# NERSC/swin_v2_weather

Hardware: AMD Instinct MI355X
Metric: ERA5 samples/sec (73x721x1440) swin_73var depth12 (higher is better)
Workload: dtype bf16

## Files before the change

include/swv2.h:

```cpp
#ifndef SWV2_H
#define SWV2_H
#include <stddef.h>
#include <stdint.h>

#ifdef __cplusplus
extern "C" {
#endif

#define SWV2_VERSION 112

enum {
    SWV2_OK = 0,
    SWV2_ERR_INVALID = -1,
    SWV2_ERR_UNSUPPORTED = -2,
    SWV2_ERR_LAUNCH = -3
};

int swv2_version(void);
const char* swv2_last_error(void);

int swv2_attn_geometry(int L, int head_dim, int* Lp, int* DP);

int swv2_attn_fwd_regime(int L, int head_dim, int has_bias, int dbg);

// ... 155 lines not shown
    void* out;
    int out_f32;
} swv2_prep_item;
int swv2_prep_chunk(void);
int swv2_prep_item_chunks(int out_rows, int out_cols, int transpose);
int swv2_prep_multi(const swv2_prep_item* items_dev, const int* chunks_dev, int n_chunks, void* stream);

#define SWV2_LN_BWD_MAX_BLOCKS 512
typedef struct swv2_ln_args {
    const void* a;
    const float* res;
    const float* gamma;
    const float* beta;
    const float* scale;
    const int32_t* rowidx;
    float* y;
    float* mean;
    float* rstd;
    const float* dy;
    void* da;
    float* dgamma;
    float* dbeta;
    float* ws;
    int M, C, res_mod, rows_per_sample;
    float eps;
} swv2_ln_args;

int swv2_ln_residual_fwd(const swv2_ln_args* a, void* stream);
int swv2_ln_residual_bwd(const swv2_ln_args* a, void* stream);

int swv2_batch_sum(const float* in, float* out, int B, long n, int accumulate, void* stream);

int swv2_merge_stats(const float* x, float* mean, float* rstd, int B, int H, int W, int C, float eps, void* stream);
int swv2_merge_ln_bwd(const float* x, const void* dn_bf16, const float* gamma, const float* mean, const float* rstd,
                      float* dx, float* dgamma, float* dbeta, int B, int H, int W, int C, void* stream);

int swv2_loss_sums(const float* prd, const float* tar, const float* quad_w, float* sums, int BC, int H, int W, void* stream);
int swv2_loss_grad(const float* prd, const float* tar, const float* quad_w, const float* coef, float* dprd, int BC, int H,
                   int W, void* stream);
#define SWV2_LOSS_PART_SLICES 8
#define SWV2_LOSS_GROUP_ROWS 32
#define SWV2_LOSS_DUMP_BYTES 2048
#define SWV2_LOSS_RESID_PITCH(N) (((N) + 63) / 64 * 64)
int swv2_loss_part_reduce(const float* part, int M, int T, int B, int Cout, int Ct, int coff, float* sums, void* stream);
int swv2_loss_resid_to_image(const void* resid, const float* coef, const float* add, float* out, int B, int Cout, int H, int W, int Cs, int Cadd,
                             void* stream);
int swv2_loss_finalize(const float* sums, int layers, const float* chw, int BC, int C, int absolute, int squared, float* loss, float* coef,
                       void* stream);

int swv2_adam_step(float* p, const float* g, float* m, float* v, long n, float lr, float beta1, float beta2, float eps,
                   int step, float grad_inv_scale, void* stream);

typedef struct swv2_adam_item {
    float* p;
    const float* g;
    float* m;
    float* v;
    long n;
} swv2_adam_item;
int swv2_adam_chunk(void);
int swv2_adam_multi(const swv2_adam_item* items_dev, const int* chunks_dev, int n_chunks, float lr, float beta1, float beta2,
                    float eps, int step, float grad_inv_scale, void* stream);

typedef struct swv2_lamb_item {
    float* p;
    const float* g;
    float* m;
    float* v;
    long n;
    long chunk0;
} swv2_lamb_item;
#define SWV2_LAMB_SUM_DEPTH 64
#define SWV2_LAMB_ADAMW 1
#define SWV2_LAMB_BIAS_CORRECTION 2
#define SWV2_LAMB_GRAD_AVERAGING 4
#define SWV2_LAMB_NVLAMB 8
#define SWV2_LAMB_WS_GNORM2 0
#define SWV2_LAMB_WS_CLIP 1
#define SWV2_LAMB_WS_BC1 2
#define SWV2_LAMB_WS_BC2 3
#define SWV2_LAMB_WS_ITEM(i) (4 + 4 * (i))
int swv2_lamb_chunk(void);
size_t swv2_lamb_ws_bytes(int n_items, int n_chunks);
int swv2_lamb_grad_norm(const swv2_lamb_item* items_dev, const int* chunks_dev, int n_items, int n_chunks, float grad_inv_scale, void* ws,
                        size_t ws_bytes, void* stream);
int swv2_lamb_multi(const swv2_lamb_item* items_dev, const int* chunks_dev, int n_items, int n_chunks, int item_lo, int item_hi,
                    int chunk_lo, int chunk_hi, float lr, float beta1, float beta2, float eps, float weight_decay, float grad_inv_scale,
                    float max_grad_norm, int step, int flags, const float* extra_gnorm2, void* ws, size_t ws_bytes, void* stream);

int swv2_score_slices(int planes, int H, int W);
size_t swv2_score_ws_bytes(int planes, int H, int W);
int swv2_score_sums(const float* prd, long prd_bstride, const float* tar, long tar_bstride, const float* clim, const float* w, int B, int C,
                    int H, int W, void* ws, size_t ws_bytes, void* stream);
int swv2_score_finalize(const void* ws, size_t ws_bytes, int B, int C, int H, int W, const float* scale, float* sums, float* rmse, float* acc,
                        float* rmse_mean, float* acc_mean, void* stream);

int swv2_stats_slices(int C, int H, int W);
size_t swv2_stats_ws_bytes(int C, int H, int W);
int swv2_stats_accumulate(const float* slab, const float* prev, const double* pivot, double* tsum, void* part, size_t part_bytes, int C, int H,
                          int W, int first, void* stream);
int swv2_stats_finalize(const void* part, size_t part_bytes, const double* tsum, const double* pivot, int C, int H, int W, long T,
                        double* folded, float* time_means, void* stream);

size_t swv2_quantile_ws_bytes(int planes, int H, int W, int K);
int swv2_plane_order_stats(const float* x, long bstride, int B, int C, int H, int W, const int* ranks, int K, float* out, int* nan_count,
                           void* ws, size_t ws_bytes, void* stream);

size_t swv2_ens_ws_bytes(int planes, int H, int W, int M);
int swv2_ens_sums(const float* ens, long ens_mstride, long ens_bstride, const float* tar, long tar_bstride, const float* w, int M, int B, int C,
                  int H, int W, void* ws, size_t ws_bytes, void* stream);
int swv2_ens_finalize(const void* ws, size_t ws_bytes, int M, int B, int C, int H, int W, const float* scale, float* sums, int* hist,
                      float* ens_rmse, float* spread, float* crps, float* fair_crps, float* means, void* stream);

size_t swv2_l1_ws_bytes(int planes, int H, int W);
int swv2_l1_sums(const float* prd, long prd_bstride, const float* tar, long tar_bstride, const float* w, int B, int C, int H, int W, void* ws,
                 size_t ws_bytes, void* stream);
int swv2_l1_finalize(const void* ws, size_t ws_bytes, int B, int C, int H, int W, const float* chw, int absolute, float* sums, float* loss,
                     float* coef, void* stream);
int swv2_l1_grad(const float* prd, const float* tar, const float* quad_w, const float* coef, float* dprd, int BC, int H, int W, void* stream);

size_t swv2_sht_ws_bytes(int planes, int lmax, int mmax);
int swv2_sht_power(const float* table, const float* X, float* power, float* coeffs, int planes, int nlat, int lmax, int mmax, void* ws,
                   size_t ws_bytes, void* stream);
int swv2_sht_adjoint(const float* table, const float* coeffs, const float* gpower, float* dX, int planes, int nlat, int lmax, int mmax,
                     void* stream);
int swv2_sht_repack(const float* src, float* dst, int planes, int nlat, int mmax, float scale, int backward, void* stream);
int swv2_sht_synth(const float* table, const float* rweights, const float* coeffs, const float* response, int response_stride, float scale_m0,
                   float scale_m, float* S, int planes, int nlat, int lmax, int mmax, int nlon, void* stream);

int swv2_era5_select_normalize(const float* raw, float* out, const int* chan, const float* mean, const float* stdv, int B, int S,
                               int Csel, int Craw, int Hraw, int Wraw, int H, int W, int Cout_total, int coff, void* stream);
int swv2_era5_zenith(float* out, const float* sun, int B, int nz, int H, int W, int Cout_total, int coff, void* stream);
int swv2_era5_static(const float* stat, float* out, int B, int Cs, int H, int W, int Cout_total, int coff, void* stream);

int swv2_era5_select_normalize_i16(const int16_t* raw, float* out, const int* chan, const float* mean, const float* stdv, const float* offset,
                                   const float* scale, const int* slab_row, int B, int S, int Csel, int Craw, int Hraw, int Wraw, int H, int W,
                                   int Cout_total, int coff, void* stream);
int swv2_era5_unpack_i16(const int16_t* raw, float* out, const float* offset, const float* scale, int C, int H, int W, void* stream);
int swv2_era5_pack_i16(const float* slab, int16_t* out, const float* offset, const float* scale, int C, int H, int W, void* stream);
size_t swv2_pack_range_ws_bytes(int C, int H, int W);
int swv2_pack_range(const float* slab, int C, int H, int W, int first, float* range, int64_t* missing, void* ws, size_t ws_bytes, void* stream);

typedef struct {
    const void* oh;
    const void* wp;
    const float* bp;
    const float* gamma; const float* beta; const float* scale;
    const int32_t* rowidx;
    const float* x;
    void* a1; float* mean; float* rstd;
    float* y;
    int Bw, Lp, heads, C, rows_per_sample;
    float eps;
} swv2_proj_ln_args;
typedef struct {
    const float* dy;
    const void* a1; const float* mean; const float* rstd; const float* gamma; const float* scale;
    const int32_t* rowidx;
    const void* wpt;
    void* da1;
    void* doh;
    float* dgamma; float* dbeta; float* ws;
    int Bw, Lp, heads, C, rows_per_sample;
} swv2_proj_ln_bwd_args;
int swv2_proj_ln_supported(int C, int heads, int head_pad);
size_t swv2_proj_ln_bwd_ws_floats(int Mw, int C);
int swv2_proj_ln_fwd(const swv2_proj_ln_args* a, void* stream);
int swv2_proj_ln_bwd(const swv2_proj_ln_bwd_args* a, void* stream);

typedef struct {
    const float* x;
    const void* w1;
    const float* b1;
    const void* w2;
    const float* b2;
    const float* gamma;
    const float* beta;
    const float* scale;
    void* hpre;
    void* a2;
    float* mean;
    float* rstd;
    float* y;
    int M, C, hidden, rows_per_sample;
    float eps;
} swv2_mlp_args;
int swv2_mlp_supported(int C, int hidden);
int swv2_mlp_recompute_supported(int C, int hidden);
int swv2_mlp_fwd(const swv2_mlp_args* a, void* stream);

typedef struct {
    const float* dy;
    const void* a2;
    const float* mean;
    const float* rstd;
    const float* gamma;
    const float* scale;
    const void* hpre;
    const void* w2t;
    const void* w1t;
    void* da2;
    void* dh;
    float* dx;
    float* dgamma;
    float* dbeta;
    float* ws;
    int M, C, hidden, rows_per_sample;
    const float* x;
    const void* w1;
    const float* b1;
} swv2_mlp_bwd_args;
size_t swv2_mlp_bwd_ws_floats(int M, int C);
int swv2_mlp_bwd(const swv2_mlp_bwd_args* a, void* stream);

int swv2_cpb_fwd(const float* w1, const float* b1, const float* w2, const float* b2, const void* keep_bf16, float* bias,
                 int wh, int ww, int heads, int hidden, float drop_p, void* stream);
int swv2_cpb_bwd(const float* dbias, const float* w1, const float* b1, const float* w2, const void* keep_bf16, float* dw1,
                 float* db1, float* dw2, float* db2, int wh, int ww, int heads, int hidden, float drop_p, void* stream);
size_t swv2_cpb_bwd_ws_bytes(int wh, int ww, int heads, int hidden);
int swv2_cpb_bwd_ws(const float* dbias, const float* w1, const float* b1, const float* w2, const void* keep_bf16, float* dw1,
                    float* db1, float* dw2, float* db2, int wh, int ww, int heads, int hidden, float drop_p, void* ws,
                    size_t ws_bytes, void* stream);

int swv2_cpb_fwd_multi(const float* const* params_dev, int nblk, const uint32_t* keep_bits, float* bias, int wh, int ww, int heads,
                       int hidden, float drop_p, void* stream);
size_t swv2_cpb_bwd_multi_ws_bytes(int nblk, int wh, int ww, int heads, int hidden);
int swv2_cpb_bwd_multi(const float* dbias_tables, int nchunk, const float* const* params_dev, int nblk, const uint32_t* keep_bits,
                       float* grads, int wh, int ww, int heads, int hidden, float drop_p, void* ws, size_t ws_bytes, void* stream);

typedef struct swv2_block_desc {
    int B, T, C, heads, head_dim, hidden, L, Lp, DP, nwh, nww, mask_thr;
    const int32_t* rowidx;
    const int32_t* qkv_map;
    const int32_t* proj_map;
    const float *logit_scale, *qkv_b_pad, *proj_b, *n1_w, *n1_b, *fc1_b, *fc2_b, *n2_w, *n2_b;
    const void *w_qkv, *w_proj, *w_fc1, *w_fc2;
    const void *w_qkvt, *w_projt, *w_fc1t, *w_fc2t;
    const float* x;
    const float* bias;
    void* bias_pack;
    const float* dp1;
    const float* dp2;
    void* qkvh;  float* rnorm; void* oh; float* lse; void* a1; float* mean1; float* rstd1; float* x1;
    void* hpre;  void* hact;   void* a2; float* mean2; float* rstd2;
    float* x2;
    const float* dx2;
    void *da2, *dh, *da1, *doh, *dqkvh;
    float* dx1;
    float* ln_ws;
    float* dx;
    float *d_logit_scale, *d_bias, *d_qkv_w, *d_qkv_b, *d_proj_w, *d_proj_b, *d_n1_w, *d_n1_b, *d_fc1_w, *d_fc1_b,
          *d_fc2_w, *d_fc2_b, *d_n2_w, *d_n2_b;
    int wgrad_splits;
    int ev_kernel;
    void* ev_start;
    void* ev_stop;
    int fuse_proj_ln;
    int fuse_mlp;
    void* wgrad_ws;
    size_t wgrad_ws_bytes;
    int wgrad_group;
    void* grad_zero;
    size_t grad_zero_bytes;
    size_t ln_ws_floats;
    int bias_prepacked;
    float* dbias_part;
    size_t dbias_part_bytes;
} swv2_block_desc;

enum swv2_block_step {
    SWV2_STEP_RNORM_ZERO = 1,
    SWV2_STEP_QKV,
    SWV2_STEP_QK_NORMALIZE,
    SWV2_STEP_PACK_BIAS,
    SWV2_STEP_ATTN_FWD,
    SWV2_STEP_PROJ, SWV2_STEP_LN1_FWD,
    SWV2_STEP_PROJ_LN_FWD,
    SWV2_STEP_FC1, SWV2_STEP_FC2, SWV2_STEP_LN2_FWD,
    SWV2_STEP_MLP_FWD,
    SWV2_STEP_LN2_BWD, SWV2_STEP_WGRAD_FC2, SWV2_STEP_DH, SWV2_STEP_WGRAD_FC1, SWV2_STEP_DX1,
    SWV2_STEP_MLP_BWD,
    SWV2_STEP_LN1_BWD,
    SWV2_STEP_PROJ_LN_BWD,
    SWV2_STEP_WGRAD_PROJ, SWV2_STEP_DOH, SWV2_STEP_ATTN_BWD, SWV2_STEP_WGRAD_QKV, SWV2_STEP_DX,
    SWV2_STEP_LN_FOLD,
    SWV2_STEP_WGRAD_GROUP,
    SWV2_STEP_COUNT
};
#define SWV2_BLOCK_MAX_STEPS 12
enum { SWV2_DBIAS_NONE = 0,
       SWV2_DBIAS_ATOMICS = 1,
       SWV2_DBIAS_WGRAD_WS = 2,
       SWV2_DBIAS_PART = 3 };
typedef struct swv2_block_plan_t {
    int mlp_fused;
    int proj_ln_fused;
    int ln_deferred;
    int wgrad_grouped;
    int wgrad_kernel;
    int grad_zero_in_kernel;
    int attn_fwd_chunks, attn_bwd_chunks;
    int dbias_dest;
    size_t need_hact_bytes;
    size_t need_ln_ws_floats;
    size_t need_wgrad_ws_bytes;
    int n_fwd, n_bwd;
    int fwd[SWV2_BLOCK_MAX_STEPS], bwd[SWV2_BLOCK_MAX_STEPS];
} swv2_block_plan_t;
int swv2_block_plan(const swv2_block_desc* d, swv2_block_plan_t* out);
int swv2_block_step_id(int step);
const char* swv2_block_step_name(int step);

int swv2_block_fwd(const swv2_block_desc* d, void* stream);
int swv2_block_bwd(const swv2_block_desc* d, void* stream);

#ifdef __cplusplus
}
#endif
#endif
```

swin_v2_weather_amd/_lib.py:

```python
from __future__ import annotations

import ctypes as C
import os
import subprocess
import threading

HERE = os.path.dirname(os.path.abspath(__file__))
CSRC = os.path.join(HERE, "csrc")
LIB_PATH = os.environ.get("SWV2_LIB") or os.path.join(HERE, "libswv2.so")
SOURCES = ["capi.hip", "attn.hip", "attn2.hip", "attn_bwd_stream.hip", "attn_wide.hip", "attn_d256.hip", "gemm.hip", "gemm_tn.hip", "gemm_tn_slab.hip", "rowops.hip", "lamb.hip", "block.hip", "cpb.hip", "mlp.hip", "proj_ln.hip", "dataio.hip", "packed.hip", "score.hip", "stats.hip", "quantile.hip", "ensemble.hip", "loss_l1.hip", "sht.hip"]

ABI_VERSION = 112

_lib = None
_lock = threading.Lock()


class Swv2Error(RuntimeError):
    pass


def build_library(force: bool = False, verbose: bool = False) -> str:
    import glob
    srcs = [os.path.join(CSRC, s) for s in SOURCES]
    deps = srcs + glob.glob(os.path.join(CSRC, "*.h")) + [os.path.join(HERE, "..", "include", "swv2.h")]
    if not force and os.path.exists(LIB_PATH) and all(os.path.getmtime(LIB_PATH) >= os.path.getmtime(d) for d in deps):
        return LIB_PATH
    hipcc = os.environ.get("HIPCC", "/opt/rocm/bin/hipcc")
    objs, procs = [], []
    os.makedirs(os.path.join(HERE, "build"), exist_ok=True)
    for s in srcs:
        o = os.path.join(HERE, "build", os.path.basename(s) + ".o")
        objs.append(o)
        cmd = [hipcc, "--offload-arch=gfx950", "-O3", "-std=c++17", "-fPIC", "-c", s, "-o", o]
        procs.append((cmd, subprocess.Popen(cmd, stdout=subprocess.PIPE, stderr=subprocess.STDOUT)))
    for cmd, p in procs:
        out, _ = p.communicate()
        if p.returncode != 0:
            raise Swv2Error("hipcc failed: %s\n%s" % (" ".join(cmd), out.decode()))
        if verbose and out:
            print(out.decode())
    cmd = [hipcc, "--offload-arch=gfx950", "-shared", "-fPIC", "-o", LIB_PATH] + objs
    r = subprocess.run(cmd, stdout=subprocess.PIPE, stderr=subprocess.STDOUT)
    if r.returncode != 0:
        raise Swv2Error("link failed: %s\n%s" % (" ".join(cmd), r.stdout.decode()))
    return LIB_PATH


def source_hash() -> str:
    import glob
    import hashlib
    h = hashlib.sha256()
    files = sorted(glob.glob(os.path.join(CSRC, "*"))) + [os.path.join(HERE, "..", "include", "swv2.h")]
    for f in files:
        if os.path.isfile(f):
            h.update(os.path.basename(f).encode())
            h.update(open(f, "rb").read())
    return h.hexdigest()[:16]


class AttnArgs(C.Structure):
    _fields_ = [("qkvh", C.c_void_p), ("logit_scale", C.c_void_p), ("bias", C.c_void_p), ("bias_pack", C.c_void_p), ("oh", C.c_void_p),
                ("lse", C.c_void_p), ("doh", C.c_void_p), ("rnorm", C.c_void_p), ("dqkvh", C.c_void_p),
                ("dlogit_scale", C.c_void_p), ("dbias", C.c_void_p),
                ("Bw", C.c_int), ("heads", C.c_int), ("L", C.c_int), ("head_dim", C.c_int),
                ("nwh", C.c_int), ("nww", C.c_int), ("mask_thr", C.c_int), ("max_chunks", C.c_int), ("dbg", C.c_int),
                ("dbias_ws", C.c_void_p), ("dbias_ws_bytes", C.c_size_t), ("dbias_partials", C.c_int)]


class AttnKernelInfo(C.Structure):
    _fields_ = [(n, C.c_int) for n in ("family", "Lp", "DP", "LT", "DK", "LFIX", "regime", "aug", "bias_lds", "qg")]


ATTN_K_D256, ATTN_K_FWD3, ATTN_K_FWD3W, ATTN_K_FWD3B, ATTN_K_WIDE, ATTN_K_STREAM, ATTN_K_FIRST_GEN = range(7)
ATTN_K_NAMES = ("D256", "FWD3", "FWD3W", "FWD3B", "WIDE", "STREAM", "FIRST_GEN")


class Operand(C.Structure):
    _fields_ = [("kind", C.c_int), ("ptr", C.c_void_p), ("rowidx", C.c_void_p), ("aux0", C.c_void_p),
                ("aux1", C.c_void_p), ("aux2", C.c_void_p), ("aux3", C.c_void_p), ("ld", C.c_long),
                ("rows", C.c_int), ("cols", C.c_int), ("p", C.c_int * 4)]


class PrepItem(C.Structure):
    _fields_ = [("w", C.c_void_p), ("rows", C.c_int), ("cols", C.c_int), ("transpose", C.c_int), ("row_map", C.c_void_p),
                ("out_rows", C.c_int), ("col_map", C.c_void_p), ("out_cols", C.c_int), ("out", C.c_void_p), ("out_f32", C.c_int)]


class AdamItem(C.Structure):
    _fields_ = [("p", C.c_void_p), ("g", C.c_void_p), ("m", C.c_void_p), ("v", C.c_void_p), ("n", C.c_long)]


class LambItem(C.Structure):
    _fields_ = [("p", C.c_void_p), ("g", C.c_void_p), ("m", C.c_void_p), ("v", C.c_void_p), ("n", C.c_long), ("chunk0", C.c_long)]


class WgradItem(C.Structure):
    _fields_ = [("dy", Operand), ("x", Operand), ("dW", C.c_void_p), ("db", C.c_void_p), ("nmap", C.c_void_p),
                ("kmap", C.c_void_p), ("ldw", C.c_int)]


class Epilogue(C.Structure):
    _fields_ = [("kind", C.c_int), ("out", C.c_void_p), ("bias", C.c_void_p), ("aux", C.c_void_p),
                ("aux_out", C.c_void_p), ("rowidx", C.c_void_p), ("ld", C.c_long), ("p", C.c_int * 5),
                ("loss_tar", C.c_void_p), ("loss_qw", C.c_void_p), ("loss_part", C.c_void_p),
                ("loss_resid", C.c_void_p),
                ("q", C.c_int * 3)]


class ProjLnArgs(C.Structure):
    _fields_ = [(n, C.c_void_p) for n in ("oh", "wp", "bp", "gamma", "beta", "scale", "rowidx", "x", "a1", "mean", "rstd", "y")] + \
               [(n, C.c_int) for n in ("Bw", "Lp", "heads", "C", "rows_per_sample")] + [("eps", C.c_float)]


class ProjLnBwdArgs(C.Structure):
    _fields_ = [(n, C.c_void_p) for n in ("dy", "a1", "mean", "rstd", "gamma", "scale", "rowidx", "wpt", "da1", "doh", "dgamma", "dbeta",
                                           "ws")] + [(n, C.c_int) for n in ("Bw", "Lp", "heads", "C", "rows_per_sample")]


class MlpArgs(C.Structure):
    _fields_ = [(n, C.c_void_p) for n in ("x", "w1", "b1", "w2", "b2", "gamma", "beta", "scale", "hpre", "a2", "mean", "rstd", "y")] + \
               [(n, C.c_int) for n in ("M", "C", "hidden", "rows_per_sample")] + [("eps", C.c_float)]


class MlpBwdArgs(C.Structure):
    _fields_ = [(n, C.c_void_p) for n in ("dy", "a2", "mean", "rstd", "gamma", "scale", "hpre", "w2t", "w1t", "da2", "dh", "dx",
                                           "dgamma", "dbeta", "ws")] + [(n, C.c_int) for n in ("M", "C", "hidden", "rows_per_sample")] + \
               [(n, C.c_void_p) for n in ("x", "w1", "b1")]


class LnArgs(C.Structure):
    _fields_ = [("a", C.c_void_p), ("res", C.c_void_p), ("gamma", C.c_void_p), ("beta", C.c_void_p),
                ("scale", C.c_void_p), ("rowidx", C.c_void_p), ("y", C.c_void_p), ("mean", C.c_void_p),
                ("rstd", C.c_void_p), ("dy", C.c_void_p), ("da", C.c_void_p), ("dgamma", C.c_void_p),
                ("dbeta", C.c_void_p), ("ws", C.c_void_p), ("M", C.c_int), ("C", C.c_int), ("res_mod", C.c_int),
                ("rows_per_sample", C.c_int), ("eps", C.c_float)]


LN_BWD_MAX_BLOCKS = 512
ATTN_FIRST_GEN, ATTN_PLAIN_STATS, ATTN_BWD_TWO_PHASE = 16, 8192, 32
LOSS_PART_SLICES = 8
LOSS_GROUP_ROWS = 32
LOSS_DUMP_BYTES = 2048
SHT_MRUN = 8


def loss_resid_pitch(n: int) -> int:
    return (n + 63) // 64 * 64
class BlockDesc(C.Structure):
    _fields_ = ([(n, C.c_int) for n in ("B", "T", "C", "heads", "head_dim", "hidden", "L", "Lp", "DP", "nwh", "nww", "mask_thr")] +
                [(n, C.c_void_p) for n in (
                    "rowidx", "qkv_map", "proj_map",
                    "logit_scale", "qkv_b_pad", "proj_b", "n1_w", "n1_b", "fc1_b", "fc2_b", "n2_w", "n2_b",
                    "w_qkv", "w_proj", "w_fc1", "w_fc2", "w_qkvt", "w_projt", "w_fc1t", "w_fc2t",
                    "x", "bias", "bias_pack", "dp1", "dp2",
                    "qkvh", "rnorm", "oh", "lse", "a1", "mean1", "rstd1", "x1", "hpre", "hact", "a2", "mean2", "rstd2", "x2",
                    "dx2", "da2", "dh", "da1", "doh", "dqkvh", "dx1", "ln_ws", "dx",
                    "d_logit_scale", "d_bias", "d_qkv_w", "d_qkv_b", "d_proj_w", "d_proj_b", "d_n1_w", "d_n1_b", "d_fc1_w",
                    "d_fc1_b", "d_fc2_w", "d_fc2_b", "d_n2_w", "d_n2_b")] +
                [("wgrad_splits", C.c_int), ("ev_kernel", C.c_int), ("ev_start", C.c_void_p), ("ev_stop", C.c_void_p),
                 ("fuse_proj_ln", C.c_int), ("fuse_mlp", C.c_int), ("wgrad_ws", C.c_void_p), ("wgrad_ws_bytes", C.c_size_t), ("wgrad_group", C.c_int), ("grad_zero", C.c_void_p),
                 ("grad_zero_bytes", C.c_size_t), ("ln_ws_floats", C.c_size_t),
                 ("bias_prepacked", C.c_int), ("dbias_part", C.c_void_p), ("dbias_part_bytes", C.c_size_t)])


LAMB_ADAMW, LAMB_BIAS_CORRECTION, LAMB_GRAD_AVERAGING, LAMB_NVLAMB = 1, 2, 4, 8
LAMB_SUM_DEPTH = 64
LAMB_WS_GNORM2, LAMB_WS_CLIP, LAMB_WS_BC1, LAMB_WS_BC2 = range(4)


def lamb_ws_item(i: int) -> int:
    return 4 + 4 * i


BLOCK_MAX_STEPS = 12
DBIAS_NONE, DBIAS_ATOMICS, DBIAS_WGRAD_WS, DBIAS_PART = range(4)


class BlockPlan(C.Structure):
    _fields_ = ([(n, C.c_int) for n in ("mlp_fused", "proj_ln_fused", "ln_deferred", "wgrad_grouped", "wgrad_kernel", "grad_zero_in_kernel",
                                        "attn_fwd_chunks", "attn_bwd_chunks", "dbias_dest")] +
                [(n, C.c_size_t) for n in ("need_hact_bytes", "need_ln_ws_floats", "need_wgrad_ws_bytes")] +
                [("n_fwd", C.c_int), ("n_bwd", C.c_int), ("fwd", C.c_int * BLOCK_MAX_STEPS), ("bwd", C.c_int * BLOCK_MAX_STEPS)])

    def steps(self, phase):
        lib = load()
        return [lib.swv2_block_step_name(s).decode() for s in getattr(self, phase)[:getattr(self, "n_" + phase)]]


def block_plan(desc: BlockDesc) -> BlockPlan:
    plan = BlockPlan()
    check(load().swv2_block_plan(C.byref(desc), C.byref(plan)), "swv2_block_plan")
    return plan


OP_F32, OP_BF16, OP_BF16_GELU, OP_HEADS, OP_PATCH, OP_MERGE_LN, OP_BF16_CSCALE = range(7)
EPI_BF16, EPI_F32, EPI_QKV_HEADS, EPI_GELU_GRAD, EPI_UNPATCH, EPI_HEADS, EPI_F32_ACC, EPI_BF16_GELU, EPI_UNPATCH_LOSS = range(9)
LINEAR_RESIDENT_QKV128, LINEAR_RESIDENT_QKV192X3, LINEAR_RESIDENT_DX128, LINEAR_WIDE_DMA, LINEAR_WIDE, LINEAR_TILE64, LINEAR_TILE128 = range(7)
LINEAR_WIDE_KERNELS, LINEAR_TILE_KERNELS = (LINEAR_WIDE_DMA, LINEAR_WIDE), (LINEAR_TILE64, LINEAR_TILE128)
WGRAD_WIDE, WGRAD_TILE = range(2)
BLOCK_WGRAD_SLAB, BLOCK_WGRAD_GROUPED = range(2)

_P, _I, _L, _F = C.c_void_p, C.c_int, C.c_long, C.c_float
SYMBOLS = {
    "swv2_version": (_I, []),
    "swv2_last_error": (C.c_char_p, []),
    "swv2_attn_geometry": (_I, [_I, _I, C.POINTER(_I), C.POINTER(_I)]),
    "swv2_attn_fwd_regime": (_I, [_I, _I, _I, _I]),
    "swv2_attn_fwd_kernel": (_I, [C.POINTER(AttnArgs), C.POINTER(AttnKernelInfo)]),
    "swv2_attn_bwd_kernel": (_I, [C.POINTER(AttnArgs), C.POINTER(AttnKernelInfo)]),
    "swv2_attn_pack_bias_bytes": (C.c_size_t, [_I, _I]),
    "swv2_attn_dbias_ws_bytes": (C.c_size_t, [_I, _I, _I]),
    "swv2_attn_pack_bias": (_I, [_P, _I, _I, _P, _P]),
    "swv2_attn_pack_bias_multi": (_I, [_P, _I, _I, _I, _P, _P]),
    "swv2_attn_bias_chunks": (_I, [_I]),
    "swv2_attn_fwd": (_I, [C.POINTER(AttnArgs), _P]),
    "swv2_attn_bwd": (_I, [C.POINTER(AttnArgs), _P]),
    "swv2_linear": (_I, [C.POINTER(Operand), _P, C.POINTER(Epilogue), _I, _P]),
    "swv2_linear_kernel": (_I, [C.POINTER(Operand), C.POINTER(Epilogue), _I]),
    "swv2_linear_wgrad_kernel": (_I, [C.POINTER(Operand), C.POINTER(Operand), _I, C.c_size_t]),
    "swv2_block_wgrad_kernel": (_I, [C.POINTER(WgradItem), _I, C.c_size_t]),
    "swv2_linear_wgrad": (_I, [C.POINTER(Operand), C.POINTER(Operand), _P, _P, _P, _P, _I, _I, _P]),
    "swv2_linear_wgrad_ws_bytes": (C.c_size_t, [_I, _I, _I, _I]),
    "swv2_qk_normalize": (_I, [_P, _P, _I, _I, _I, _I, _I, _P]),
    "swv2_block_wgrad_ws_bytes": (C.c_size_t, [_I, _I, _I, _I]),
    "swv2_block_wgrad": (_I, [C.POINTER(WgradItem), _I, _P, C.c_size_t, _P]),
    "swv2_linear_wgrad_ws": (_I, [C.POINTER(Operand), C.POINTER(Operand), _P, _P, _P, _P, _I, _I, _P, C.c_size_t, _P]),
    "swv2_prep_weight": (_I, [_P, _I, _I, _I, _P, _I, _P, _I, _P, _P]),
    "swv2_ln_residual_fwd": (_I, [C.POINTER(LnArgs), _P]),
    "swv2_ln_residual_bwd": (_I, [C.POINTER(LnArgs), _P]),
    "swv2_batch_sum": (_I, [_P, _P, _I, _L, _I, _P]),
    "swv2_merge_stats": (_I, [_P, _P, _P, _I, _I, _I, _I, _F, _P]),
    "swv2_merge_ln_bwd": (_I, [_P, _P, _P, _P, _P, _P, _P, _P, _I, _I, _I, _I, _P]),
    "swv2_loss_sums": (_I, [_P, _P, _P, _P, _I, _I, _I, _P]),
    "swv2_loss_grad": (_I, [_P, _P, _P, _P, _P, _I, _I, _I, _P]),
    "swv2_loss_part_reduce": (_I, [_P, _I, _I, _I, _I, _I, _I, _P, _P]),
    "swv2_loss_resid_to_image": (_I, [_P, _P, _P, _P, _I, _I, _I, _I, _I, _I, _P]),
    "swv2_loss_finalize": (_I, [_P, _I, _P, _I, _I, _I, _I, _P, _P, _P]),
    "swv2_prep_chunk": (_I, []),
    "swv2_prep_item_chunks": (_I, [_I, _I, _I]),
    "swv2_prep_multi": (_I, [_P, _P, _I, _P]),
    "swv2_adam_chunk": (_I, []),
    "swv2_adam_multi": (_I, [_P, _P, _I, _F, _F, _F, _F, _I, _F, _P]),
    "swv2_adam_step": (_I, [_P, _P, _P, _P, _L, _F, _F, _F, _F, _I, _F, _P]),
    "swv2_lamb_chunk": (_I, []),
    "swv2_lamb_ws_bytes": (C.c_size_t, [_I, _I]),
    "swv2_lamb_grad_norm": (_I, [_P, _P, _I, _I, _F, _P, C.c_size_t, _P]),
    "swv2_lamb_multi": (_I, [_P, _P, _I, _I, _I, _I, _I, _I, _F, _F, _F, _F, _F, _F, _F, _I, _I, _P, _P, C.c_size_t, _P]),
    "swv2_score_slices": (_I, [_I, _I, _I]),
    "swv2_score_ws_bytes": (C.c_size_t, [_I, _I, _I]),
    "swv2_score_sums": (_I, [_P, _L, _P, _L, _P, _P, _I, _I, _I, _I, _P, C.c_size_t, _P]),
    "swv2_score_finalize": (_I, [_P, C.c_size_t, _I, _I, _I, _I, _P, _P, _P, _P, _P, _P, _P]),
    "swv2_stats_slices": (_I, [_I, _I, _I]),
    "swv2_stats_ws_bytes": (C.c_size_t, [_I, _I, _I]),
    "swv2_stats_accumulate": (_I, [_P, _P, _P, _P, _P, C.c_size_t, _I, _I, _I, _I, _P]),
    "swv2_stats_finalize": (_I, [_P, C.c_size_t, _P, _P, _I, _I, _I, _L, _P, _P, _P]),
    "swv2_quantile_ws_bytes": (C.c_size_t, [_I, _I, _I, _I]),
    "swv2_plane_order_stats": (_I, [_P, _L, _I, _I, _I, _I, _P, _I, _P, _P, _P, C.c_size_t, _P]),
    "swv2_ens_ws_bytes": (C.c_size_t, [_I, _I, _I, _I]),
    "swv2_ens_sums": (_I, [_P, _L, _L, _P, _L, _P, _I, _I, _I, _I, _I, _P, C.c_size_t, _P]),
    "swv2_ens_finalize": (_I, [_P, C.c_size_t, _I, _I, _I, _I, _I, _P, _P, _P, _P, _P, _P, _P, _P, _P]),
    "swv2_l1_ws_bytes": (C.c_size_t, [_I, _I, _I]),
    "swv2_l1_sums": (_I, [_P, _L, _P, _L, _P, _I, _I, _I, _I, _P, C.c_size_t, _P]),
    "swv2_l1_finalize": (_I, [_P, C.c_size_t, _I, _I, _I, _I, _P, _I, _P, _P, _P, _P]),
    "swv2_l1_grad": (_I, [_P, _P, _P, _P, _P, _I, _I, _I, _P]),
    "swv2_sht_ws_bytes": (C.c_size_t, [_I, _I, _I]),
    "swv2_sht_power": (_I, [_P, _P, _P, _P, _I, _I, _I, _I, _P, C.c_size_t, _P]),
    "swv2_sht_adjoint": (_I, [_P, _P, _P, _P, _I, _I, _I, _I, _P]),
    "swv2_sht_repack": (_I, [_P, _P, _I, _I, _I, _F, _I, _P]),
    "swv2_sht_synth": (_I, [_P, _P, _P, _P, _I, _F, _F, _P, _I, _I, _I, _I, _I, _P]),
    "swv2_era5_select_normalize": (_I, [_P, _P, _P, _P, _P] + [_I] * 10 + [_P]),
    "swv2_era5_zenith": (_I, [_P, _P, _I, _I, _I, _I, _I, _I, _P]),
    "swv2_era5_static": (_I, [_P, _P, _I, _I, _I, _I, _I, _I, _P]),
    "swv2_era5_select_normalize_i16": (_I, [_P] * 8 + [_I] * 10 + [_P]),
    "swv2_era5_unpack_i16": (_I, [_P, _P, _P, _P, _I, _I, _I, _P]),
    "swv2_era5_pack_i16": (_I, [_P, _P, _P, _P, _I, _I, _I, _P]),
    "swv2_pack_range_ws_bytes": (C.c_size_t, [_I, _I, _I]),
    "swv2_pack_range": (_I, [_P, _I, _I, _I, _I, _P, _P, _P, C.c_size_t, _P]),
    "swv2_proj_ln_supported": (_I, [_I, _I, _I]),
    "swv2_proj_ln_bwd_ws_floats": (C.c_size_t, [_I, _I]),
    "swv2_proj_ln_fwd": (_I, [C.POINTER(ProjLnArgs), _P]),
    "swv2_proj_ln_bwd": (_I, [C.POINTER(ProjLnBwdArgs), _P]),
    "swv2_mlp_supported": (_I, [_I, _I]),
    "swv2_mlp_recompute_supported": (_I, [_I, _I]),
    "swv2_mlp_fwd": (_I, [C.POINTER(MlpArgs), _P]),
    "swv2_mlp_bwd_ws_floats": (C.c_size_t, [_I, _I]),
    "swv2_mlp_bwd": (_I, [C.POINTER(MlpBwdArgs), _P]),
    "swv2_cpb_fwd": (_I, [_P, _P, _P, _P, _P, _P, _I, _I, _I, _I, _F, _P]),
    "swv2_cpb_bwd": (_I, [_P, _P, _P, _P, _P, _P, _P, _P, _P, _I, _I, _I, _I, _F, _P]),
    "swv2_cpb_bwd_ws": (_I, [_P, _P, _P, _P, _P, _P, _P, _P, _P, _I, _I, _I, _I, _F, _P, C.c_size_t, _P]),
    "swv2_cpb_bwd_ws_bytes": (C.c_size_t, [_I, _I, _I, _I]),
    "swv2_cpb_fwd_multi": (_I, [_P, _I, _P, _P, _I, _I, _I, _I, _F, _P]),
    "swv2_cpb_bwd_multi_ws_bytes": (C.c_size_t, [_I, _I, _I, _I, _I]),
    "swv2_cpb_bwd_multi": (_I, [_P, _I, _P, _I, _P, _P, _I, _I, _I, _I, _F, _P, C.c_size_t, _P]),
    "swv2_block_plan": (_I, [C.POINTER(BlockDesc), C.POINTER(BlockPlan)]),
    "swv2_block_step_id": (_I, [_I]),
    "swv2_block_step_name": (C.c_char_p, [_I]),
    "swv2_block_fwd": (_I, [C.POINTER(BlockDesc), _P]),
    "swv2_block_bwd": (_I, [C.POINTER(BlockDesc), _P]),
}


def load() -> C.CDLL:
    global _lib
    if _lib is not None:
        return _lib
    with _lock:
        if _lib is None:
            if not os.path.exists(LIB_PATH):
                raise Swv2Error(f"{LIB_PATH} not found: run `python -c 'import __graft_entry__ as g; g.build()'` "
                                "(the HIP library is required; there is no fallback path)")
            import torch
            lib = C.CDLL(LIB_PATH)
            for name, (res, args) in SYMBOLS.items():
                fn = getattr(lib, name)
                fn.restype, fn.argtypes = res, args
            got = lib.swv2_version()
            if got != ABI_VERSION:
                raise Swv2Error(f"{LIB_PATH} reports ABI revision {got}, this binding mirrors revision {ABI_VERSION} of include/swv2.h: "
                                "rebuild the library (python -c 'import __graft_entry__ as g; g.build()')")
            _lib = lib
    return _lib


def check(rc: int, what: str = "") -> None:
    if rc != 0:
        msg = load().swv2_last_error()
        raise Swv2Error(f"{what} failed with code {rc}: {msg.decode() if msg else ''}")
```

swin_v2_weather_amd/csrc/block.hip:

```cpp
#include "common.h"

namespace {

swv2_operand op(int kind, const void* p, int rows, int cols, long ld, const int32_t* rowidx = nullptr) {
    swv2_operand o = {};
    o.kind = kind; o.ptr = p; o.rowidx = rowidx; o.ld = ld; o.rows = rows; o.cols = cols;
    return o;
}
swv2_operand op_heads(const void* p, int Bw, int heads, int parts, int Lp, int DP) {
    swv2_operand o = op(SWV2_OP_HEADS, p, Bw * Lp, parts * heads * DP, parts);
    o.p[0] = heads; o.p[2] = Lp; o.p[3] = DP;
    return o;
}
swv2_epilogue epi(int kind, void* out, long ld, const float* bias = nullptr, const void* aux = nullptr,
                  float* aux_out = nullptr, const int32_t* rowidx = nullptr) {
    swv2_epilogue e = {};
    e.kind = kind; e.out = out; e.ld = ld; e.bias = bias; e.aux = aux; e.aux_out = aux_out; e.rowidx = rowidx;
    return e;
}
swv2_attn_args attn(const swv2_block_desc* d, int max_chunks) {
    swv2_attn_args a = {};
    a.qkvh = d->qkvh; a.logit_scale = d->logit_scale; a.bias = d->bias; a.bias_pack = d->bias ? d->bias_pack : nullptr;
    a.oh = d->oh; a.lse = d->lse;
    a.Bw = d->B * d->nwh * d->nww; a.heads = d->heads; a.L = d->L; a.head_dim = d->head_dim; a.nwh = d->nwh; a.nww = d->nww;
    a.mask_thr = d->mask_thr; a.max_chunks = max_chunks;
    return a;
}
void wgrad_items(const swv2_block_desc* d, bool fused, swv2_wgrad_item it[4]) {
    const int BT = d->B * d->T, Bw = d->B * d->nwh * d->nww, Mw = Bw * d->Lp, C = d->C, h = d->heads, hid = d->hidden;
    it[0].dy = op(SWV2_OP_BF16, d->da2, BT, C, C);
    it[0].x = fused ? op(SWV2_OP_BF16_GELU, d->hpre, BT, hid, hid) : op(SWV2_OP_BF16, d->hact, BT, hid, hid);
    it[0].dW = d->d_fc2_w; it[0].db = d->d_fc2_b; it[0].ldw = hid;
    it[1].dy = op(SWV2_OP_BF16, d->dh, BT, hid, hid); it[1].x = op(SWV2_OP_F32, d->x1, BT, C, C);
    it[1].dW = d->d_fc1_w; it[1].db = d->d_fc1_b; it[1].ldw = C;
    it[2].dy = op(SWV2_OP_BF16, d->da1, Mw, C, C); it[2].x = op_heads(d->oh, Bw, h, 1, d->Lp, d->DP);
    it[2].dW = d->d_proj_w; it[2].db = d->d_proj_b; it[2].kmap = d->proj_map; it[2].ldw = C;
    it[3].dy = op_heads(d->dqkvh, Bw, h, 3, d->Lp, d->DP); it[3].x = op(SWV2_OP_F32, d->x, Mw, C, C, d->rowidx);
    it[3].dW = d->d_qkv_w; it[3].db = d->d_qkv_b; it[3].nmap = d->qkv_map; it[3].ldw = C;
}
#define TRY(x) do { int rc_ = (x); if (rc_) return rc_; } while (0)

const struct { int id; const char* name; } STEPS[SWV2_STEP_COUNT] = {
    {0, "end"},
    {0, "rnorm_zero"}, {1, "qkv"}, {0, "qk_normalize"}, {0, "pack_bias"}, {2, "attn_fwd"}, {3, "proj"}, {4, "ln1_fwd"}, {3, "proj_ln_fwd"},
    {5, "fc1"}, {6, "fc2"}, {7, "ln2_fwd"}, {5, "mlp_fwd"},
    {11, "ln2_bwd"}, {12, "wgrad_fc2"}, {13, "dh"}, {14, "wgrad_fc1"}, {15, "dx1"}, {13, "mlp_bwd"}, {16, "ln1_bwd"}, {16, "proj_ln_bwd"},
    {17, "wgrad_proj"}, {18, "doh"}, {19, "attn_bwd"}, {20, "wgrad_qkv"}, {21, "dx"}, {0, "ln_fold"}, {22, "wgrad_group"},
};
static_assert(SWV2_STEP_WGRAD_GROUP + 1 == SWV2_STEP_COUNT && SWV2_STEP_MLP_FWD == 12 && SWV2_STEP_LN2_BWD == 13, "STEPS follows enum swv2_block_step");

#define LAUNCH(step, x)                                                                                     \
    do {                                                                                                    \
        const bool t_ = d->ev_kernel == STEPS[step].id && d->ev_start && d->ev_stop;                         \
        if (t_) (void)hipEventRecord((hipEvent_t)d->ev_start, (hipStream_t)st);                             \
        TRY(x);                                                                                             \
        if (t_) (void)hipEventRecord((hipEvent_t)d->ev_stop, (hipStream_t)st);                              \
    } while (0)

int plan_block(const swv2_block_desc* d, swv2_block_plan_t* p) {
    SWV2_CHECK_ARG(d && p, "swv2_block_plan: null descriptor or plan");
    SWV2_CHECK_ARG(d->B > 0 && d->T > 0 && d->C > 0 && d->heads > 0 && d->hidden > 0 && d->Lp > 0 && d->DP > 0 && d->nwh > 0 && d->nww > 0,
                   "swv2_block_plan: non-positive geometry");
    *p = {};
    const int BT = d->B * d->T, Bw = d->B * d->nwh * d->nww, Mw = Bw * d->Lp, C = d->C, h = d->heads, hid = d->hidden;
    const int sp = d->wgrad_splits > 0 ? d->wgrad_splits : 64;
    const size_t ws_bytes = d->wgrad_ws ? d->wgrad_ws_bytes : 0;
    const size_t ln_pair = swv2_mlp_bwd_ws_floats(BT, C) + swv2_proj_ln_bwd_ws_floats(Mw, C);
    p->need_ln_ws_floats = std::max((size_t)SWV2_LN_BWD_MAX_BLOCKS * 2 * C, ln_pair);
    p->need_wgrad_ws_bytes = d->wgrad_group ? swv2_block_wgrad_ws_bytes(C, hid, h * d->DP, 0) : 0;
    const int prod[4][3] = {{BT, C, hid}, {BT, hid, C}, {Mw, C, h * d->DP}, {Mw, 3 * h * d->DP, C}};
    for (const auto& q : prod)
        p->need_wgrad_ws_bytes = std::max(p->need_wgrad_ws_bytes, swv2_linear_wgrad_ws_bytes(q[0], q[1], q[2], sp));

    p->mlp_fused = d->fuse_mlp && swv2_mlp_supported(C, hid);
    p->proj_ln_fused = d->fuse_proj_ln && swv2_proj_ln_supported(C, h, d->DP);
    p->need_hact_bytes = p->mlp_fused ? 0 : (size_t)BT * hid * 2;
    p->ln_deferred = p->mlp_fused && p->proj_ln_fused && d->ln_ws_floats >= ln_pair;
    p->wgrad_grouped = d->wgrad_group && p->mlp_fused && d->wgrad_ws && ws_bytes >= swv2_block_wgrad_ws_bytes(C, hid, h * d->DP, 0);
    p->wgrad_kernel = -1;
    p->grad_zero_in_kernel = p->mlp_fused && d->grad_zero != nullptr;
    p->attn_fwd_chunks = d->bias ? 32 : 64;
    p->attn_bwd_chunks = 64;
    if (d->bias) {
        p->attn_bwd_chunks = swv2_attn_bias_chunks(Bw);
        p->dbias_dest = d->dbias_part ? SWV2_DBIAS_PART : ws_bytes ? SWV2_DBIAS_WGRAD_WS : SWV2_DBIAS_ATOMICS;
    } else if (d->Lp == 176 && h <= 256) {
        p->attn_bwd_chunks = 256 / h;
    }

    auto fwd = [&](int s) { p->fwd[p->n_fwd++] = s; };
    auto bwd = [&](int s) { p->bwd[p->n_bwd++] = s; };
    const bool wide = d->DP > 64;
    if (wide) fwd(SWV2_STEP_RNORM_ZERO);
    fwd(SWV2_STEP_QKV);
    if (wide) fwd(SWV2_STEP_QK_NORMALIZE);
    if (d->bias && d->bias_pack && !d->bias_prepacked) fwd(SWV2_STEP_PACK_BIAS);
    fwd(SWV2_STEP_ATTN_FWD);
    if (p->proj_ln_fused) fwd(SWV2_STEP_PROJ_LN_FWD);
    else { fwd(SWV2_STEP_PROJ); fwd(SWV2_STEP_LN1_FWD); }
    if (p->mlp_fused) fwd(SWV2_STEP_MLP_FWD);
    else { fwd(SWV2_STEP_FC1); fwd(SWV2_STEP_FC2); fwd(SWV2_STEP_LN2_FWD); }

    const bool single = !p->wgrad_grouped;
    if (p->mlp_fused) {
        bwd(SWV2_STEP_MLP_BWD);
        if (single) { bwd(SWV2_STEP_WGRAD_FC2); bwd(SWV2_STEP_WGRAD_FC1); }
    } else {
        bwd(SWV2_STEP_LN2_BWD); bwd(SWV2_STEP_WGRAD_FC2); bwd(SWV2_STEP_DH); bwd(SWV2_STEP_WGRAD_FC1); bwd(SWV2_STEP_DX1);
    }
    bwd(p->proj_ln_fused ? SWV2_STEP_PROJ_LN_BWD : SWV2_STEP_LN1_BWD);
    if (single) bwd(SWV2_STEP_WGRAD_PROJ);
    if (!p->proj_ln_fused) bwd(SWV2_STEP_DOH);
    bwd(SWV2_STEP_ATTN_BWD);
    if (single) bwd(SWV2_STEP_WGRAD_QKV);
    bwd(SWV2_STEP_DX);
    if (p->ln_deferred && single) bwd(SWV2_STEP_LN_FOLD);
    if (p->wgrad_grouped) bwd(SWV2_STEP_WGRAD_GROUP);
    return SWV2_OK;
}

}

extern "C" int swv2_block_step_id(int step) { return step > 0 && step < SWV2_STEP_COUNT ? STEPS[step].id : -1; }
extern "C" const char* swv2_block_step_name(int step) { return step > 0 && step < SWV2_STEP_COUNT ? STEPS[step].name : nullptr; }

extern "C" int swv2_block_plan(const swv2_block_desc* d, swv2_block_plan_t* p) {
    TRY(plan_block(d, p));
    if (p->wgrad_grouped) {
        swv2_wgrad_item it[4] = {};
        wgrad_items(d, true, it);
        p->wgrad_kernel = swv2_block_wgrad_kernel(it, 0, d->wgrad_ws_bytes);
    }
    return SWV2_OK;
}

extern "C" int swv2_block_fwd(const swv2_block_desc* d, void* st) {
    SWV2_CHECK_ARG(d && d->x && d->x2 && d->qkvh && d->rowidx, "swv2_block_fwd: null descriptor field");
    swv2_block_plan_t p;
    TRY(plan_block(d, &p));
    SWV2_CHECK_ARG(d->hact || !p.need_hact_bytes, "swv2_block_fwd: the separate MLP kernels need hact (swv2_block_plan: need_hact_bytes)");
    const int BT = d->B * d->T, Bw = d->B * d->nwh * d->nww, Mw = Bw * d->Lp, C = d->C, h = d->heads, hid = d->hidden;
    for (int i = 0; i < p.n_fwd; ++i) switch (p.fwd[i]) {
    case SWV2_STEP_RNORM_ZERO:
        if (hipMemsetAsync(d->rnorm, 0, (size_t)Bw * h * 2 * d->Lp * sizeof(float), (hipStream_t)st) != hipSuccess) {
            swv2_set_error("swv2_block_fwd: hipMemsetAsync(rnorm) failed");
            return SWV2_ERR_LAUNCH;
        }
        break;
    case SWV2_STEP_QKV: {
        swv2_operand a = op(SWV2_OP_F32, d->x, Mw, C, C, d->rowidx);
        swv2_epilogue e = epi(SWV2_EPI_QKV_HEADS, d->qkvh, 0, d->qkv_b_pad, nullptr, d->rnorm);
        e.p[0] = h; e.p[2] = d->Lp; e.p[3] = d->DP; e.p[4] = d->L;
        LAUNCH(SWV2_STEP_QKV, swv2_linear(&a, d->w_qkv, &e, 3 * h * d->DP, st));
    } break;
    case SWV2_STEP_QK_NORMALIZE: TRY(swv2_qk_normalize(d->qkvh, (float*)d->rnorm, Bw, h, d->Lp, d->L, d->DP, st)); break;
    case SWV2_STEP_PACK_BIAS: TRY(swv2_attn_pack_bias(d->bias, h, d->L, d->bias_pack, st)); break;
    case SWV2_STEP_ATTN_FWD: {
        swv2_attn_args a = attn(d, p.attn_fwd_chunks);
        LAUNCH(SWV2_STEP_ATTN_FWD, swv2_attn_fwd(&a, st));
    } break;
    case SWV2_STEP_PROJ_LN_FWD: {
        swv2_proj_ln_args m = {};
        m.oh = d->oh; m.wp = d->w_proj; m.bp = d->proj_b; m.gamma = d->n1_w; m.beta = d->n1_b; m.scale = d->dp1; m.rowidx = d->rowidx;
        m.x = d->x; m.a1 = d->a1; m.mean = d->mean1; m.rstd = d->rstd1; m.y = d->x1; m.Bw = Bw; m.Lp = d->Lp; m.heads = h; m.C = C;
        m.rows_per_sample = d->T; m.eps = 1e-5f;
        LAUNCH(SWV2_STEP_PROJ_LN_FWD, swv2_proj_ln_fwd(&m, st));
    } break;
    case SWV2_STEP_PROJ: {
        swv2_operand a = op_heads(d->oh, Bw, h, 1, d->Lp, d->DP);
        swv2_epilogue e = epi(SWV2_EPI_BF16, d->a1, C, d->proj_b);
        LAUNCH(SWV2_STEP_PROJ, swv2_linear(&a, d->w_proj, &e, C, st));
    } break;
    case SWV2_STEP_LN1_FWD: {
        swv2_ln_args l = {};
        l.a = d->a1; l.res = d->x; l.gamma = d->n1_w; l.beta = d->n1_b; l.scale = d->dp1; l.rowidx = d->rowidx; l.y = d->x1;
        l.mean = d->mean1; l.rstd = d->rstd1; l.M = Mw; l.C = C; l.res_mod = 0; l.rows_per_sample = d->T; l.eps = 1e-5f;
        LAUNCH(SWV2_STEP_LN1_FWD, swv2_ln_residual_fwd(&l, st));
    } break;
    case SWV2_STEP_MLP_FWD: {
        swv2_mlp_args m = {};
        m.x = d->x1; m.w1 = d->w_fc1; m.b1 = d->fc1_b; m.w2 = d->w_fc2; m.b2 = d->fc2_b; m.gamma = d->n2_w; m.beta = d->n2_b;
        m.scale = d->dp2; m.hpre = d->hpre; m.a2 = d->a2; m.mean = d->mean2; m.rstd = d->rstd2; m.y = d->x2;
        m.M = BT; m.C = C; m.hidden = hid; m.rows_per_sample = d->T; m.eps = 1e-5f;
        LAUNCH(SWV2_STEP_MLP_FWD, swv2_mlp_fwd(&m, st));
    } break;
    case SWV2_STEP_FC1: {
        swv2_operand a = op(SWV2_OP_F32, d->x1, BT, C, C);
        swv2_epilogue e = epi(SWV2_EPI_BF16_GELU, d->hpre, hid, d->fc1_b, nullptr, (float*)d->hact);
        LAUNCH(SWV2_STEP_FC1, swv2_linear(&a, d->w_fc1, &e, hid, st));
    } break;
    case SWV2_STEP_FC2: {
        swv2_operand a = op(SWV2_OP_BF16, d->hact, BT, hid, hid);
        swv2_epilogue e = epi(SWV2_EPI_BF16, d->a2, C, d->fc2_b);
        LAUNCH(SWV2_STEP_FC2, swv2_linear(&a, d->w_fc2, &e, C, st));
    } break;
    case SWV2_STEP_LN2_FWD: {
        swv2_ln_args l = {};
        l.a = d->a2; l.res = d->x1; l.gamma = d->n2_w; l.beta = d->n2_b; l.scale = d->dp2; l.y = d->x2; l.mean = d->mean2;
        l.rstd = d->rstd2; l.M = BT; l.C = C; l.res_mod = 0; l.rows_per_sample = d->T; l.eps = 1e-5f;
        LAUNCH(SWV2_STEP_LN2_FWD, swv2_ln_residual_fwd(&l, st));
    } break;
    }
    return SWV2_OK;
}

extern "C" int swv2_block_bwd(const swv2_block_desc* d, void* st) {
    SWV2_CHECK_ARG(d && d->dx2 && d->dx && d->da2 && d->dh && d->dx1 && d->da1 && d->doh && d->dqkvh && d->ln_ws,
                   "swv2_block_bwd: null descriptor field");
    swv2_block_plan_t p;
    TRY(plan_block(d, &p));
    SWV2_CHECK_ARG(d->hact || !p.need_hact_bytes, "swv2_block_bwd: the separate MLP kernels need hact (swv2_block_plan: need_hact_bytes)");
    const int BT = d->B * d->T, Bw = d->B * d->nwh * d->nww, Mw = Bw * d->Lp, C = d->C, h = d->heads, hid = d->hidden;
    const int sp = d->wgrad_splits > 0 ? d->wgrad_splits : 64;
    swv2_wgrad_item it[4] = {};
    wgrad_items(d, p.mlp_fused, it);
    float* const ln1_ws = p.ln_deferred ? d->ln_ws + swv2_mlp_bwd_ws_floats(BT, C) : d->ln_ws;
    int n_ln1 = 0, n_ln2 = 0;
    for (int i = 0; i < p.n_bwd; ++i) switch (const int s = p.bwd[i]; s) {
    case SWV2_STEP_MLP_BWD: {
        swv2_mlp_bwd_args m = {};
        m.dy = d->dx2; m.a2 = d->a2; m.mean = d->mean2; m.rstd = d->rstd2; m.gamma = d->n2_w; m.scale = d->dp2; m.hpre = d->hpre;
        m.w2t = d->w_fc2t; m.w1t = d->w_fc1t; m.da2 = d->da2; m.dh = d->dh; m.dx = d->dx1; m.dgamma = d->d_n2_w;
        m.dbeta = d->d_n2_b; m.ws = d->ln_ws; m.M = BT; m.C = C; m.hidden = hid; m.rows_per_sample = d->T;
        LAUNCH(SWV2_STEP_MLP_BWD, swv2_mlp_bwd_impl(&m, st, p.ln_deferred ? &n_ln2 : nullptr, p.grad_zero_in_kernel ? (float*)d->grad_zero : nullptr,
                                                    (long)(d->grad_zero_bytes / 4)));
    } break;
    case SWV2_STEP_LN2_BWD: {
        swv2_ln_args l = {};
        l.a = d->a2; l.dy = d->dx2; l.gamma = d->n2_w; l.scale = d->dp2; l.mean = d->mean2; l.rstd = d->rstd2; l.da = d->da2;
        l.dgamma = d->d_n2_w; l.dbeta = d->d_n2_b; l.ws = d->ln_ws; l.M = BT; l.C = C; l.rows_per_sample = d->T;
        LAUNCH(SWV2_STEP_LN2_BWD, swv2_ln_residual_bwd(&l, st));
    } break;
    case SWV2_STEP_WGRAD_FC2: case SWV2_STEP_WGRAD_FC1: case SWV2_STEP_WGRAD_PROJ: case SWV2_STEP_WGRAD_QKV: {
        const swv2_wgrad_item& w = it[s == SWV2_STEP_WGRAD_FC2 ? 0 : s == SWV2_STEP_WGRAD_FC1 ? 1 : s == SWV2_STEP_WGRAD_PROJ ? 2 : 3];
        LAUNCH(s, swv2_linear_wgrad_ws(&w.dy, &w.x, w.dW, w.db, w.nmap, w.kmap, w.ldw, sp, d->wgrad_ws, d->wgrad_ws_bytes, st));
    } break;
    case SWV2_STEP_DH: {
        swv2_epilogue e = epi(SWV2_EPI_GELU_GRAD, d->dh, hid, nullptr, d->hpre);
        LAUNCH(SWV2_STEP_DH, swv2_linear(&it[0].dy, d->w_fc2t, &e, hid, st));
    } break;
    case SWV2_STEP_DX1: {
        swv2_epilogue e = epi(SWV2_EPI_F32, d->dx1, C, nullptr, d->dx2);
        LAUNCH(SWV2_STEP_DX1, swv2_linear(&it[1].dy, d->w_fc1t, &e, C, st));
    } break;
    case SWV2_STEP_PROJ_LN_BWD: {
        swv2_proj_ln_bwd_args m = {};
        m.dy = d->dx1; m.a1 = d->a1; m.mean = d->mean1; m.rstd = d->rstd1; m.gamma = d->n1_w; m.scale = d->dp1; m.rowidx = d->rowidx;
        m.wpt = d->w_projt; m.da1 = d->da1; m.doh = d->doh; m.dgamma = d->d_n1_w; m.dbeta = d->d_n1_b; m.ws = ln1_ws;
        m.Bw = Bw; m.Lp = d->Lp; m.heads = h; m.C = C; m.rows_per_sample = d->T;
        LAUNCH(SWV2_STEP_PROJ_LN_BWD, swv2_proj_ln_bwd_impl(&m, st, p.ln_deferred ? &n_ln1 : nullptr));
    } break;
    case SWV2_STEP_LN1_BWD: {
        swv2_ln_args l = {};
        l.a = d->a1; l.dy = d->dx1; l.gamma = d->n1_w; l.scale = d->dp1; l.rowidx = d->rowidx; l.mean = d->mean1; l.rstd = d->rstd1;
        l.da = d->da1; l.dgamma = d->d_n1_w; l.dbeta = d->d_n1_b; l.ws = d->ln_ws; l.M = Mw; l.C = C; l.rows_per_sample = d->T;
        LAUNCH(SWV2_STEP_LN1_BWD, swv2_ln_residual_bwd(&l, st));
    } break;
    case SWV2_STEP_DOH: {
        swv2_epilogue e = epi(SWV2_EPI_HEADS, d->doh, 0);
        e.p[0] = h; e.p[2] = d->Lp; e.p[3] = d->DP; e.p[4] = d->L;
        LAUNCH(SWV2_STEP_DOH, swv2_linear(&it[2].dy, d->w_projt, &e, h * d->DP, st));
    } break;
    case SWV2_STEP_ATTN_BWD: {
        swv2_attn_args a = attn(d, p.attn_bwd_chunks);
        a.doh = d->doh; a.rnorm = d->rnorm; a.dqkvh = d->dqkvh; a.dlogit_scale = d->d_logit_scale; a.dbias = d->d_bias;
        if (p.dbias_dest == SWV2_DBIAS_PART) { a.dbias_ws = d->dbias_part; a.dbias_ws_bytes = d->dbias_part_bytes; a.dbias_partials = 1; }
        if (p.dbias_dest == SWV2_DBIAS_WGRAD_WS) { a.dbias_ws = d->wgrad_ws; a.dbias_ws_bytes = d->wgrad_ws_bytes; }
        LAUNCH(SWV2_STEP_ATTN_BWD, swv2_attn_bwd(&a, st));
    } break;
    case SWV2_STEP_DX: {
        swv2_epilogue e = epi(SWV2_EPI_F32, d->dx, C, nullptr, d->dx1, nullptr, d->rowidx);
        LAUNCH(SWV2_STEP_DX, swv2_linear(&it[3].dy, d->w_qkvt, &e, C, st));
    } break;
    case SWV2_STEP_LN_FOLD:
        swv2_launch_ln_partials_reduce2(d->ln_ws, d->d_n2_w, d->d_n2_b, n_ln2, ln1_ws, d->d_n1_w, d->d_n1_b, n_ln1, C, (hipStream_t)st);
        break;
    case SWV2_STEP_WGRAD_GROUP: {
        swv2_ln_partials lnp = {{d->ln_ws, ln1_ws}, {d->d_n2_w, d->d_n1_w}, {d->d_n2_b, d->d_n1_b}, {n_ln2, n_ln1}, C};
        LAUNCH(SWV2_STEP_WGRAD_GROUP, swv2_block_wgrad_ln(it, 0, d->wgrad_ws, d->wgrad_ws_bytes, p.ln_deferred ? &lnp : nullptr, st));
    } break;
    }
    return SWV2_OK;
}
```

swin_v2_weather_amd/csrc/gemm_tn.hip:

```cpp
#include "gemm_common.h"
#ifdef SWV2_TN_STAMPS
#define SWV2_STAMPS
#endif
#include "stamps.h"

namespace {

constexpr int TM = 128;
constexpr int TP = 136;
constexpr int TCH = TM * 16 / NTHREADS;

struct TnOut {
    float* dW; float* db; const int32_t* nmap; const int32_t* kmap; int ldw, M, N, K, ntk, tiles; float* ws;
};
constexpr int TN_SMEM = 2 * TM * TP;

template <int YK, int XK, bool XG = false, bool HINC = false>
__device__ __forceinline__ void tn_tile(const ALoad<YK>& yl, const ALoad<XK>& xl_arg, const TnOut& o, int tile, int slice,
                                        int chunk_stride, uint16_t* smem, float* dbs, uint16_t* gtab) {
    float* __restrict__ dW = o.dW;
    float* __restrict__ db = o.db;
    const int32_t* __restrict__ nmap = o.nmap;
    const int32_t* __restrict__ kmap = o.kmap;
    const int ldw = o.ldw, M = o.M, N = o.N, K = o.K, ntk = o.ntk, tiles = o.tiles;
// ... 48 lines not shown
        for (int i = 0; i < TCH; ++i) {
            const int m0 = (slice + s * chunk_stride) * TM, my = m0 + yr_(i), mx = m0 + xr_(i);
            const bool iny = (s < steps) && (my < m_hi), inx = (s < steps) && (mx < m_hi);
            yrow[i] = iny ? my : -1;
            if constexpr (XG) {
                xrow[i] = xl.d.rowidx[min(mx, M - 1)];
                xin |= (uint32_t)inx << i;
            } else {
                xrow[i] = inx ? mx : -1;
            }
        }
    };
    auto issue = [&](int s) {
        okmask = 0;
#pragma unroll
        for (int i = 0; i < TCH; ++i) {
            const int yk = n_base + yc_(i) * 8, xk = k_base + xc_(i) * 8;
            const int xr = XG ? (((xin >> i) & 1) ? xrow[i] : -1) : xrow[i];
            const bool yok = yrow[i] >= 0 && yk < N, xok = xr >= 0 && xk < K;
            if constexpr (YLIN) ry[i] = yl.raw_lin(yrow[i] >= 0 ? yoff0 + i * ystep : ycol);
            else if constexpr (YHD) ry[i] = yl.raw_lin(yrow[i] >= 0 ? yl.step_off(yst, i) : 0u);
            else ry[i] = yl.raw_unc(max(yrow[i], 0), yk < N ? yk : 0);
            if constexpr (XLIN) rx[i] = xl.raw_lin(xr >= 0 ? xoff0 + i * xstep : xcol);
            else if constexpr (XHD) rx[i] = xl.raw_lin(xr >= 0 ? xl.step_off(xst, i) : 0u);
            else if constexpr (XG && XK == A_F32) rx[i] = xl.raw_lin((uint32_t)max(xr, 0) * (uint32_t)xl.d.ld + xcol);
            else rx[i] = xl.raw_unc(max(xr, 0), xk < K ? xk : 0);
            okmask |= ((uint32_t)yok << i) | ((uint32_t)xok << (16 + i));
        }
    };
    auto commit = [&]() {
        uint16_t* Ys = smem;
        uint16_t* Xs = smem + TM * TP;
        const uint4 zero4 = make_uint4(0, 0, 0, 0);
#pragma unroll
        for (int i = 0; i < TCH; ++i) {
            const uint4 yv = ((okmask >> i) & 1) ? yl.cvt(ry[i]) : zero4;
            *(uint4*)(Ys + yr_(i) * TP + yc_(i) * 8) = yv;
            *(uint4*)(Xs + xr_(i) * TP + xc_(i) * 8) = ((okmask >> (16 + i)) & 1) ? xl.cvt(rx[i]) : zero4;
            if (want_db && !YRF) {
                float v[8];
                unpack8(yv, v);
#pragma unroll
                for (int e = 0; e < 8; ++e) colsum[e] += v[e];
            }
        }
    };

    f32x4 acc[4][4];
#pragma unroll
    for (int i = 0; i < 4; ++i)
#pragma unroll
        for (int j = 0; j < 4; ++j) acc[i][j] = (f32x4){0.f, 0.f, 0.f, 0.f};

    STAMP_DECL(8)
    STAMP_START();
    resolve(0);
    issue(0);
    resolve(1);
    STAMP(7);
    for (int s = 0; s < steps; ++s) {
        STAMP_WAITV();
        STAMP(0);
        commit();
        STAMP(1);
        __syncthreads();
        STAMP(2);
        if (s + 1 < steps) { issue(s + 1); resolve(s + 2); }
        STAMP(3);
        const uint16_t* Ys = smem;
        const uint16_t* Xs = smem + TM * TP;
#pragma unroll
        for (int kk = 0; kk < TM / 32; ++kk) {
            bf16x8 af[4], bf[4];
            const int r0 = 32 * kk + 8 * g + (fr >> 2), cc = (fr & 3) * 4;
#pragma unroll
            for (int i = 0; i < 4; ++i) {
                const bf16x4 a0 = lds_tr_read(Ys + r0 * TP + wr * 64 + i * 16 + cc);
                const bf16x4 a1 = lds_tr_read(Ys + (r0 + 4) * TP + wr * 64 + i * 16 + cc);
                const bf16x4 b0 = lds_tr_read(Xs + r0 * TP + wc * 64 + i * 16 + cc);
                const bf16x4 b1 = lds_tr_read(Xs + (r0 + 4) * TP + wc * 64 + i * 16 + cc);
                af[i] = __builtin_shufflevector(a0, a1, 0, 1, 2, 3, 4, 5, 6, 7);
                bf[i] = __builtin_shufflevector(b0, b1, 0, 1, 2, 3, 4, 5, 6, 7);
            }
#pragma unroll
            for (int i = 0; i < 4; ++i)
#pragma unroll
                for (int j = 0; j < 4; ++j) acc[i][j] = mfma32(af[i], bf[j], acc[i][j]);
        }
        asm volatile("" :: "v"(acc[0][0][0]), "v"(acc[3][3][3]));
        STAMP(4);
        __syncthreads();
        STAMP(5);
    }
    if (ws) {
        float* pt = ws + ((size_t)slice * tiles + tile) * (BN * BN);
#pragma unroll
        for (int i = 0; i < 4; ++i)
#pragma unroll
            for (int j = 0; j < 4; ++j)
#pragma unroll
                for (int r = 0; r < 4; ++r)
                    pt[(wr * 64 + 16 * i + 4 * g + r) * BN + wc * 64 + 16 * j + fr] = acc[i][j][r];
#ifdef SWV2_TN_STAMPS
        STAMP_WAITV();
        STAMP(6);
        if (tid == 0) {
#pragma unroll
            for (int k = 0; k < 8; ++k) ((unsigned long long*)pt)[k] = st_acc[k];
        }
#endif
    } else
#pragma unroll
    for (int i = 0; i < 4; ++i)
#pragma unroll
        for (int j = 0; j < 4; ++j)
#pragma unroll
            for (int r = 0; r < 4; ++r) {
                int n = n_base + wr * 64 + 16 * i + 4 * g + r, k = k_base + wc * 64 + 16 * j + fr;
                if (n >= N || k >= K) continue;
                if (nmap) n = nmap[n];
                if (kmap) k = kmap[k];
                if (n >= 0 && k >= 0) atomicAdd(dW + (long)n * ldw + k, acc[i][j][r]);
            }
    if (want_db) {
#pragma unroll
        for (int e = 0; e < 8; ++e) atomicAdd(&dbs[scol * 8 + e], colsum[e]);
        __syncthreads();
        if (tid < BN && n_base + tid < N) {
            const int n = nmap ? nmap[n_base + tid] : n_base + tid;
            if (n >= 0) atomicAdd(db + n, dbs[tid]);
        }
    }
}

template <int YK, int XK, bool XG>
__global__ __launch_bounds__(NTHREADS, 2) void gemm_tn_kernel(ALoad<YK> yl, ALoad<XK> xl, TnOut o, int chunk_stride) {
    __shared__ __attribute__((aligned(16))) uint16_t smem[TN_SMEM];
    __shared__ float dbs[BN];
    __shared__ __attribute__((aligned(16))) uint16_t gtab[XK == A_BF16_GELU ? GT_N : 8];
    const int lin = blockIdx.x;
    const int x8 = lin & 7, rest = lin >> 3;
    const int tile = rest % o.tiles, slice = (rest / o.tiles) * 8 + x8;
    tn_tile<YK, XK, XG>(yl, xl, o, tile, slice, chunk_stride, smem, dbs, gtab);
}

struct TnGroup {
    ALoad<A_BF16> y0; ALoad<A_BF16_GELU> x0;
    ALoad<A_BF16> y1; ALoad<A_F32> x1;
    ALoad<A_BF16> y2; ALoad<A_HEADS> x2;
    ALoad<A_HEADS> y3; ALoad<A_F32> x3;
    TnOut o[4];
    int first[5];
    int slices;
};
__global__ __launch_bounds__(NTHREADS, 2) void gemm_tn_group_kernel(TnGroup a) {
    __shared__ __attribute__((aligned(16))) uint16_t smem[TN_SMEM];
    __shared__ float dbs[BN];
    __shared__ __attribute__((aligned(16))) uint16_t gtab[GT_N];
    const int lin = blockIdx.x, x8 = lin & 7, rest = lin >> 3, tt = a.first[4];
    const int t = rest % tt, slice = (rest / tt) * 8 + x8;
    if (t < a.first[1]) tn_tile<A_BF16, A_BF16_GELU>(a.y0, a.x0, a.o[0], t, slice, a.slices, smem, dbs, gtab);
    else if (t < a.first[2]) tn_tile<A_BF16, A_F32>(a.y1, a.x1, a.o[1], t - a.first[1], slice, a.slices, smem, dbs, gtab);
    else if (a.x2.d.p2 >= TM) {
        if (t < a.first[3]) tn_tile<A_BF16, A_HEADS, false, true>(a.y2, a.x2, a.o[2], t - a.first[2], slice, a.slices, smem, dbs, gtab);
        else tn_tile<A_HEADS, A_F32, true, true>(a.y3, a.x3, a.o[3], t - a.first[3], slice, a.slices, smem, dbs, gtab);
    } else {
        if (t < a.first[3]) tn_tile<A_BF16, A_HEADS>(a.y2, a.x2, a.o[2], t - a.first[2], slice, a.slices, smem, dbs, gtab);
        else tn_tile<A_HEADS, A_F32, true>(a.y3, a.x3, a.o[3], t - a.first[3], slice, a.slices, smem, dbs, gtab);
    }
}

struct TnReduce { TnOut o[4]; int first[5]; int slices; };
__global__ __launch_bounds__(256) void tn_reduce_kernel(TnReduce a) {
    __shared__ float part[4][64];
    const int e = blockIdx.x * 64 + (threadIdx.x & 63), sg = threadIdx.x >> 6, gt = blockIdx.y;
    const int pi = (gt >= a.first[1]) + (gt >= a.first[2]) + (gt >= a.first[3]);
    const TnOut& o = a.o[pi];
    const int tile = gt - a.first[pi], tiles = o.tiles, ntk = o.ntk;
    const int slices = min(a.slices, (o.M + TM - 1) / TM);
    const float* src = o.ws + (size_t)tile * (BN * BN) + e;
    const size_t stride = (size_t)tiles * (BN * BN);
    float s0 = 0.f, s1 = 0.f, s2 = 0.f, s3 = 0.f;
    int sl = sg;
    for (; sl + 12 < slices; sl += 16) {
        s0 += src[(size_t)sl * stride];
        s1 += src[(size_t)(sl + 4) * stride];
        s2 += src[(size_t)(sl + 8) * stride];
        s3 += src[(size_t)(sl + 12) * stride];
    }
    for (; sl < slices; sl += 4) s0 += src[(size_t)sl * stride];
    part[sg][threadIdx.x & 63] = (s0 + s1) + (s2 + s3);
    __syncthreads();
    if (sg == 0) {
        const int tn = tile / ntk, tk = tile - tn * ntk;
        int n = tn * BN + (e >> 7), k = tk * BN + (e & 127);
        if (n < o.N && k < o.K) {
            if (o.nmap) n = o.nmap[n];
            if (o.kmap) k = o.kmap[k];
            const int l = threadIdx.x;
            if (n >= 0 && k >= 0) o.dW[(long)n * o.ldw + k] += (part[0][l] + part[1][l]) + (part[2][l] + part[3][l]);
        }
    }
}

struct TnWidePlan { bool ok; int S; size_t part_bytes, db_bytes, cast_bytes, total; };
TnWidePlan tn_wide_plan(int M, int N, int K) {
    TnWidePlan p = {};
    p.ok = (N % 256 == 0) && (K % 256 == 0) && N >= 512 && K >= 512 && (M % 32 == 0) && M >= 8192 &&
           (double)M * (N > K ? N : K) * 2 < 4.29e9 && (double)N * K < 2.0e9;
    if (!p.ok) return p;
    const int tiles = (N / 256) * (K / 256);
    p.S = std::max(1, 256 / tiles);
    if (p.S > M / 32) p.S = M / 32;
    auto up = [](size_t b) { return (b + 255) / 256 * 256; };
    p.part_bytes = up((size_t)p.S * N * K * 4);
    p.db_bytes = up((size_t)p.S * (K / 256) * N * 4);
    p.cast_bytes = up((size_t)M * K * 2);
    p.total = p.part_bytes + p.db_bytes + p.cast_bytes;
    return p;
}
__global__ __launch_bounds__(256) void cast_rows_kernel(const float* __restrict__ src, const int32_t* __restrict__ rowidx, uint16_t* __restrict__ dst,
                                                        int M, int C, long ld) {
    const long i = (long)blockIdx.x * 256 + threadIdx.x, per_row = C / 8;
    if (i >= (long)M * per_row) return;
    const int m = (int)(i / per_row), c = (int)(i - (long)m * per_row) * 8;
    const int r = rowidx ? rowidx[m] : m;
    uint4 o = make_uint4(0, 0, 0, 0);
    if (r >= 0) {
        const float* p = src + (long)r * ld + c;
        RawF32 v = {*(const f32x4*)p, *(const f32x4*)(p + 4)};
        o = cvt_f32x8(v);
    }
    *(uint4*)(dst + (long)m * C + c) = o;
}
__global__ __launch_bounds__(256) void tn_wide_reduce_kernel(const float* __restrict__ part, const float* __restrict__ dbpart, float* __restrict__ dW,
                                                             float* __restrict__ db, const int32_t* __restrict__ nmap,
                                                             const int32_t* __restrict__ kmap, int ldw, int N, int K, int S) {
    const int i = (blockIdx.x * 256 + threadIdx.x) * 4, NK = N * K;
    if (i < NK) {
        f32x4 s0 = {0.f, 0.f, 0.f, 0.f}, s1 = s0;
        int sl = 0;
        for (; sl + 1 < S; sl += 2) { s0 += *(const f32x4*)(part + (size_t)sl * NK + i); s1 += *(const f32x4*)(part + (size_t)(sl + 1) * NK + i); }
        if (sl < S) s0 += *(const f32x4*)(part + (size_t)sl * NK + i);
        s0 += s1;
        int n = i / K;
        const int k = i - n * K;
        if (nmap) n = nmap[n];
        if (n >= 0) {
#pragma unroll
            for (int e = 0; e < 4; ++e) {
                const int kk = kmap ? kmap[k + e] : k + e;
                if (kk >= 0) dW[(long)n * ldw + kk] += s0[e];
            }
        }
    }
    const int n = blockIdx.x * 256 + threadIdx.x;
    if (db && dbpart && n < N) {
        const int rows = S * (K / 256);
        float a0 = 0.f, a1 = 0.f, a2 = 0.f, a3 = 0.f;
        int j = 0;
        for (; j + 3 < rows; j += 4) {
            a0 += dbpart[(size_t)j * N + n]; a1 += dbpart[(size_t)(j + 1) * N + n];
            a2 += dbpart[(size_t)(j + 2) * N + n]; a3 += dbpart[(size_t)(j + 3) * N + n];
        }
        for (; j < rows; ++j) a0 += dbpart[(size_t)j * N + n];
        const int nn = nmap ? nmap[n] : n;
        if (nn >= 0) db[nn] += (a0 + a1) + (a2 + a3);
    }
}

struct TnPlan { int ntn, ntk, tiles, real_slices, slices; size_t ws_bytes; };
TnPlan tn_plan(int M, int N, int K, int splits) {
    TnPlan p;
    p.ntn = cdiv(N, BN); p.ntk = cdiv(K, BN); p.tiles = p.ntn * p.ntk;
    int eff = (p.tiles >= 3) ? splits : splits * 2;
    eff = std::min(eff, std::max(8, (1024 / p.tiles) / 8 * 8));
    p.real_slices = std::min(eff, cdiv(M, TM));
    p.slices = cdiv(p.real_slices, 8) * 8;
    p.ws_bytes = (size_t)p.real_slices * p.tiles * BN * BN * sizeof(float);
    return p;
}
TnOut tn_out(float* dW, float* db, const int32_t* nmap, const int32_t* kmap, int ldw, int M, int N, int K, float* ws) {
    TnOut o;
    o.dW = dW; o.db = db; o.nmap = nmap; o.kmap = kmap; o.ldw = ldw; o.M = M; o.N = N; o.K = K;
    o.ntk = cdiv(K, BN); o.tiles = cdiv(N, BN) * o.ntk; o.ws = ws;
    return o;
}

enum class WgradKernel { WIDE = SWV2_WGRAD_WIDE, TILE = SWV2_WGRAD_TILE };

WgradKernel wgrad_kernel_for(const swv2_operand* y, const swv2_operand* x, size_t ws_bytes, int wide) {
    const int yk = y->kind, xk = x->kind;
    const bool kinds = (yk == A_BF16 || yk == A_HEADS) && (xk == A_BF16 || xk == A_HEADS || xk == A_F32) && !(yk == A_HEADS && xk == A_HEADS) &&
                       !y->rowidx && (xk == A_F32 || !x->rowidx);
    const TnWidePlan wp = tn_wide_plan(y->rows, y->cols, x->cols);
    return wide && wp.ok && kinds && ws_bytes >= wp.total ? WgradKernel::WIDE : WgradKernel::TILE;
}

int launch_tn_wide(const swv2_operand* y, const swv2_operand* x, float* dW, float* db, const int32_t* nmap, const int32_t* kmap, int ldw,
                   int M, int N, int K, float* ws, hipStream_t st) {
    const TnWidePlan wp = tn_wide_plan(M, N, K);
    float* part = ws;
    float* dbpart = db ? (float*)((char*)ws + wp.part_bytes) : nullptr;
    swv2_operand xb = *x;
    if (x->kind == SWV2_OP_F32) {
        uint16_t* cb = (uint16_t*)((char*)ws + wp.part_bytes + wp.db_bytes);
        const long chunks = (long)M * (K / 8);
        hipLaunchKernelGGL(cast_rows_kernel, dim3((unsigned)((chunks + 255) / 256)), dim3(256), 0, st, (const float*)x->ptr, x->rowidx, cb,
                           M, K, x->ld);
        xb.kind = SWV2_OP_BF16; xb.ptr = cb; xb.rowidx = nullptr; xb.ld = K;
    }
    int rc = swv2_tn_wide_launch(y, &xb, part, dbpart, M, N, K, wp.S, st);
    if (rc) return rc;
    const long quads = (long)N * K / 4;
    hipLaunchKernelGGL(tn_wide_reduce_kernel, dim3((unsigned)((quads + 255) / 256)), dim3(256), 0, st, (const float*)part,
// ... 4 lines not shown

template <int YK, int XK>
int launch_tn_tile(const swv2_operand* y, const swv2_operand* x, float* dW, float* db, const int32_t* nmap,
                   const int32_t* kmap, int ldw, int M, int N, int K, int splits, float* ws, size_t ws_bytes, hipStream_t st) {
    const TnPlan p = tn_plan(M, N, K, splits);
    if (ws && ws_bytes < p.ws_bytes) {
        swv2_set_error("swv2_linear_wgrad_ws: workspace of %zu bytes, %zu needed (swv2_linear_wgrad_ws_bytes)", ws_bytes, p.ws_bytes);
        return SWV2_ERR_INVALID;
    }
    const TnOut o = tn_out(dW, db, nmap, kmap, ldw, M, N, K, ws);
    if (y->rowidx || (x->rowidx && XK != A_F32)) {
        swv2_set_error("swv2_linear_wgrad: a row gather is supported for a fp32 X operand only (dY kind %d, X kind %d)", y->kind, x->kind);
        return SWV2_ERR_UNSUPPORTED;
    }
    if constexpr (XK == A_F32) {
        if (x->rowidx)
            hipLaunchKernelGGL((gemm_tn_kernel<YK, XK, true>), dim3(p.tiles * p.slices), dim3(NTHREADS), 0, st, make_loader<YK>(y),
                               make_loader<XK>(x), o, p.real_slices);
        else
            hipLaunchKernelGGL((gemm_tn_kernel<YK, XK, false>), dim3(p.tiles * p.slices), dim3(NTHREADS), 0, st, make_loader<YK>(y),
                               make_loader<XK>(x), o, p.real_slices);
    } else {
        hipLaunchKernelGGL((gemm_tn_kernel<YK, XK, false>), dim3(p.tiles * p.slices), dim3(NTHREADS), 0, st, make_loader<YK>(y),
                           make_loader<XK>(x), o, p.real_slices);
    }
    if (ws) {
        TnReduce r = {};
        r.o[0] = o; r.first[0] = 0; r.first[1] = r.first[2] = r.first[3] = r.first[4] = p.tiles; r.slices = p.real_slices;
        hipLaunchKernelGGL(tn_reduce_kernel, dim3(BN * BN / 64, p.tiles), dim3(256), 0, st, r);
    }
    SWV2_CHECK_LAUNCH("swv2_linear_wgrad");
    return SWV2_OK;
}

template <int YK, int XK>
int launch_tn2(const swv2_operand* y, const swv2_operand* x, float* dW, float* db, const int32_t* nmap,
               const int32_t* kmap, int ldw, int M, int N, int K, int splits, float* ws, size_t ws_bytes, hipStream_t st) {
    switch (wgrad_kernel_for(y, x, ws ? ws_bytes : 0, swv2_gemm_wide())) {
        case WgradKernel::WIDE: return launch_tn_wide(y, x, dW, db, nmap, kmap, ldw, M, N, K, ws, st);
        case WgradKernel::TILE: break;
    }
    return launch_tn_tile<YK, XK>(y, x, dW, db, nmap, kmap, ldw, M, N, K, splits, ws, ws_bytes, st);
}

template <int YK>
int launch_tn1(const swv2_operand* y, const swv2_operand* x, float* dW, float* db, const int32_t* nmap,
               const int32_t* kmap, int ldw, int M, int N, int K, int splits, float* ws, size_t wsb, hipStream_t st) {
    if (x->kind == SWV2_OP_F32) return launch_tn2<YK, A_F32>(y, x, dW, db, nmap, kmap, ldw, M, N, K, splits, ws, wsb, st);
    if constexpr (YK == A_BF16) {
        switch (x->kind) {
            case SWV2_OP_BF16: return launch_tn2<YK, A_BF16>(y, x, dW, db, nmap, kmap, ldw, M, N, K, splits, ws, wsb, st);
            case SWV2_OP_BF16_GELU: return launch_tn2<YK, A_BF16_GELU>(y, x, dW, db, nmap, kmap, ldw, M, N, K, splits, ws, wsb, st);
            case SWV2_OP_HEADS: return launch_tn2<YK, A_HEADS>(y, x, dW, db, nmap, kmap, ldw, M, N, K, splits, ws, wsb, st);
            case SWV2_OP_PATCH: return launch_tn2<YK, A_PATCH>(y, x, dW, db, nmap, kmap, ldw, M, N, K, splits, ws, wsb, st);
        }
    }
    if constexpr (YK == A_F32) {
        if (x->kind == SWV2_OP_MERGE_LN) return launch_tn2<YK, A_MERGE_LN>(y, x, dW, db, nmap, kmap, ldw, M, N, K, splits, ws, wsb, st);
    }
    swv2_set_error("swv2_linear_wgrad: operand pair (dY kind %d, X kind %d) is not instantiated", y->kind, x->kind);
    return SWV2_ERR_UNSUPPORTED;
}

}

extern "C" size_t swv2_linear_wgrad_ws_bytes(int M, int N, int K, int splits) {
    if (!(M > 0 && N > 0 && K > 0 && splits > 0)) return 0;
    const TnWidePlan w = tn_wide_plan(M, N, K);
    return std::max(tn_plan(M, N, K, splits).ws_bytes, w.ok ? w.total : (size_t)0);
}

extern "C" int swv2_linear_wgrad_ws(const swv2_operand* dy, const swv2_operand* x, float* dW, float* db, const int32_t* nmap,
                                    const int32_t* kmap, int ldw, int splits, void* ws, size_t ws_bytes, void* stream) {
    int rc = check_operand(dy, "swv2_linear_wgrad(dy)");
    if (rc) return rc;
    rc = check_operand(x, "swv2_linear_wgrad(x)");
    if (rc) return rc;
    SWV2_CHECK_ARG(dW && splits > 0 && ldw > 0, "swv2_linear_wgrad: null dW, non-positive splits or bad pitch");
    SWV2_CHECK_ARG(dy->rows == x->rows, "swv2_linear_wgrad: row counts differ (%d vs %d)", dy->rows, x->rows);
    SWV2_CHECK_ARG(!(db && dy->kind == SWV2_OP_PATCH), "swv2_linear_wgrad: no bias gradient with a patch-layout dY (row-fastest staging)");
    const int M = dy->rows, N = dy->cols, K = x->cols;
    hipStream_t st = (hipStream_t)stream;
    float* w = (float*)ws;
    switch (dy->kind) {
        case SWV2_OP_F32: return launch_tn1<A_F32>(dy, x, dW, db, nmap, kmap, ldw, M, N, K, splits, w, ws_bytes, st);
        case SWV2_OP_BF16: return launch_tn1<A_BF16>(dy, x, dW, db, nmap, kmap, ldw, M, N, K, splits, w, ws_bytes, st);
        case SWV2_OP_HEADS: return launch_tn1<A_HEADS>(dy, x, dW, db, nmap, kmap, ldw, M, N, K, splits, w, ws_bytes, st);
        case SWV2_OP_PATCH: return launch_tn1<A_PATCH>(dy, x, dW, db, nmap, kmap, ldw, M, N, K, splits, w, ws_bytes, st);
        case SWV2_OP_BF16_CSCALE: return launch_tn1<A_BF16_CS>(dy, x, dW, db, nmap, kmap, ldw, M, N, K, splits, w, ws_bytes, st);
    }
    swv2_set_error("swv2_linear_wgrad: unsupported dY operand kind %d", dy->kind);
    return SWV2_ERR_INVALID;
}

extern "C" int swv2_linear_wgrad(const swv2_operand* dy, const swv2_operand* x, float* dW, float* db, const int32_t* nmap,
                                 const int32_t* kmap, int ldw, int splits, void* stream) {
    return swv2_linear_wgrad_ws(dy, x, dW, db, nmap, kmap, ldw, splits, nullptr, 0, stream);
}

extern "C" int swv2_linear_wgrad_kernel(const swv2_operand* dy, const swv2_operand* x, int splits, size_t ws_bytes) {
    SWV2_CHECK_ARG(dy && x && splits > 0 && dy->rows > 0 && dy->rows == x->rows, "swv2_linear_wgrad_kernel: null operand, non-positive splits or row mismatch");
    return (int)wgrad_kernel_for(dy, x, ws_bytes, swv2_gemm_wide());
}

namespace {
int group_slices(int total_tiles, int requested) {
    if (requested > 0) return std::max(8, requested / 8 * 8);
    return std::max(8, (2 * 256 / total_tiles) / 8 * 8);
}
}

extern "C" size_t swv2_block_wgrad_ws_bytes(int C, int hidden, int heads_dp, int slices) {
    if (C <= 0 || hidden <= 0 || heads_dp <= 0) return 0;
    const int tt = 2 * cdiv(C, BN) * cdiv(hidden, BN) + cdiv(C, BN) * cdiv(heads_dp, BN) + cdiv(3 * heads_dp, BN) * cdiv(C, BN);
    return std::max((size_t)group_slices(tt, slices) * tt * BN * BN * sizeof(float), swv2_tn_slab_ws_bytes(C, hidden, heads_dp));
}

extern "C" int swv2_block_wgrad(const swv2_wgrad_item* it, int slices, void* ws, size_t ws_bytes, void* stream) {
    return swv2_block_wgrad_ln(it, slices, ws, ws_bytes, nullptr, stream);
}

namespace {
enum class BlockWgradKernel { SLAB = SWV2_BLOCK_WGRAD_SLAB, GROUPED = SWV2_BLOCK_WGRAD_GROUPED };

BlockWgradKernel block_wgrad_kernel_for(const swv2_wgrad_item* it, int slices, size_t ws_bytes) {
    return slices <= 0 && swv2_tn_slab_covers(it, ws_bytes) ? BlockWgradKernel::SLAB : BlockWgradKernel::GROUPED;
}

int launch_tn_group(const swv2_wgrad_item* it, int slices, void* ws, size_t ws_bytes, const swv2_ln_partials* ln, hipStream_t st) {
    TnGroup g = {};
    int tt = 0;
    for (int i = 0; i < 4; ++i) {
        g.first[i] = tt;
        tt += cdiv(it[i].dy.cols, BN) * cdiv(it[i].x.cols, BN);
    }
    g.first[4] = tt;
    const int S = group_slices(tt, slices);
    SWV2_CHECK_ARG(ws_bytes >= (size_t)S * tt * BN * BN * sizeof(float), "swv2_block_wgrad: workspace of %zu bytes, %zu needed",
                   ws_bytes, (size_t)S * tt * BN * BN * sizeof(float));
    if (ln && ln->C > 0)
        swv2_launch_ln_partials_reduce2(ln->ws[0], ln->dgamma[0], ln->dbeta[0], ln->n[0], ln->ws[1], ln->dgamma[1], ln->dbeta[1], ln->n[1], ln->C, st);
    TnReduce r = {};
    for (int i = 0; i < 4; ++i) {
        g.o[i] = tn_out(it[i].dW, it[i].db, it[i].nmap, it[i].kmap, it[i].ldw, it[i].dy.rows, it[i].dy.cols, it[i].x.cols,
                        (float*)ws + (size_t)g.first[i] * S * BN * BN);
        r.o[i] = g.o[i];
    }
    for (int i = 0; i < 5; ++i) r.first[i] = g.first[i];
    g.y0 = make_loader<A_BF16>(&it[0].dy); g.x0 = make_loader<A_BF16_GELU>(&it[0].x);
    g.y1 = make_loader<A_BF16>(&it[1].dy); g.x1 = make_loader<A_F32>(&it[1].x);
    g.y2 = make_loader<A_BF16>(&it[2].dy); g.x2 = make_loader<A_HEADS>(&it[2].x);
    g.y3 = make_loader<A_HEADS>(&it[3].dy); g.x3 = make_loader<A_F32>(&it[3].x);
    g.slices = r.slices = S;
    hipLaunchKernelGGL(gemm_tn_group_kernel, dim3(tt * S), dim3(NTHREADS), 0, st, g);
    hipLaunchKernelGGL(tn_reduce_kernel, dim3(BN * BN / 64, tt), dim3(256), 0, st, r);
    SWV2_CHECK_LAUNCH("swv2_block_wgrad");
    return SWV2_OK;
}
}

extern "C" int swv2_block_wgrad_kernel(const swv2_wgrad_item* it, int slices, size_t ws_bytes) {
    SWV2_CHECK_ARG(it, "swv2_block_wgrad_kernel: null items");
    return (int)block_wgrad_kernel_for(it, slices, ws_bytes);
}

int swv2_block_wgrad_ln(const swv2_wgrad_item* it, int slices, void* ws, size_t ws_bytes, const swv2_ln_partials* ln, void* stream) {
    SWV2_CHECK_ARG(it && ws, "swv2_block_wgrad: null items or workspace");
    static const int want[4][2] = {{SWV2_OP_BF16, SWV2_OP_BF16_GELU}, {SWV2_OP_BF16, SWV2_OP_F32}, {SWV2_OP_BF16, SWV2_OP_HEADS},
                                   {SWV2_OP_HEADS, SWV2_OP_F32}};
    for (int i = 0; i < 4; ++i) {
        int rc = check_operand(&it[i].dy, "swv2_block_wgrad(dy)");
        if (rc) return rc;
        rc = check_operand(&it[i].x, "swv2_block_wgrad(x)");
        if (rc) return rc;
        SWV2_CHECK_ARG(it[i].dy.kind == want[i][0] && it[i].x.kind == want[i][1],
                       "swv2_block_wgrad: item %d must be (dY kind %d, X kind %d)", i, want[i][0], want[i][1]);
        SWV2_CHECK_ARG(it[i].dW && it[i].ldw > 0 && it[i].dy.rows == it[i].x.rows, "swv2_block_wgrad: item %d: null dW or row mismatch", i);
        SWV2_CHECK_ARG(!it[i].dy.rowidx && (i == 3 ? it[i].x.rowidx != nullptr : it[i].x.rowidx == nullptr),
                       "swv2_block_wgrad: item %d: only the qkv product's X rows are gathered (and they must be)", i);
    }
    switch (block_wgrad_kernel_for(it, slices, ws_bytes)) {
        case BlockWgradKernel::SLAB: return swv2_tn_slab_launch(it, ws, ws_bytes, ln, (hipStream_t)stream);
        case BlockWgradKernel::GROUPED: break;
    }
    return launch_tn_group(it, slices, ws, ws_bytes, ln, (hipStream_t)stream);
}
```

swin_v2_weather_amd/csrc/gemm_tn_slab.hip:

```cpp
#include "gemm_common.h"
#pragma clang diagnostic ignored "-Wc++20-extensions"

namespace {

#ifdef SWV2_SLAB_PART_F32
typedef float sl_part_t;
#else
typedef uint16_t sl_part_t;
#endif
constexpr int SL_TH = 512;
constexpr int SL_SMEM = 160 * 1024;
constexpr int SL_IDX_CAP = 4096;
enum { F_ROW = 0, F_ROWG = 1, F_F32 = 2, F_F32G = 3, F_HEAD = 4 };

#ifdef SWV2_SLAB_STAMPS
#define SWV2_STAMPS
#endif
#include "stamps.h"

__device__ __forceinline__ uint4 sl_gelu8_tab(uint4 w, const unsigned char* tab0, bool& bad) {
    const uint32_t in[4] = {w.x, w.y, w.z, w.w};
    uint32_t out[4], off[4];
    u16x2_t mx = {0, 0};
    const u16x2_t lo = {(unsigned short)GT_LO, (unsigned short)GT_LO};
    typedef short s16x2_t __attribute__((ext_vector_type(2)));
#pragma unroll
    for (int i = 0; i < 4; ++i) {
        const u16x2_t idx = __builtin_bit_cast(u16x2_t, in[i] & 0x7fff7fffu) - lo;
        mx = __builtin_elementwise_max(mx, idx);
        const uint32_t sg = __builtin_bit_cast(uint32_t, __builtin_bit_cast(s16x2_t, in[i]) >> 15) & (uint32_t)(GT_HALF * 0x10001u);
        off[i] = __builtin_bit_cast(uint32_t, (idx + __builtin_bit_cast(u16x2_t, sg)) << 1);
    }
#pragma unroll
    for (int i = 0; i < 4; ++i)
        out[i] = (uint32_t)*(const uint16_t*)(tab0 + (off[i] & 0xffffu)) | ((uint32_t)*(const uint16_t*)(tab0 + (off[i] >> 16)) << 16);
    const u16x2_t top = {(unsigned short)(GT_HALF - 1), (unsigned short)(GT_HALF - 1)};
    bad = __builtin_bit_cast(uint32_t, __builtin_elementwise_min(mx, top)) != __builtin_bit_cast(uint32_t, mx);
    return make_uint4(out[0], out[1], out[2], out[3]);
}

struct SlOp {
    const void* ptr;
    const int32_t* rowidx;
    int ld;
    int heads, parts, Lp, DP;
    uint32_t mgLp, mgDP, mgH;
};
struct SlProd {
    SlOp y, x;
    sl_part_t* part;
    float* dbpart;
    int M, N, K;
    int first, wgs, ntile;
};
struct SlArgs { SlProd p[4]; unsigned long long* stamps; };

template <int W>
__device__ __forceinline__ int sl_swz(int r, int u) {
    if constexpr ((W * 2) % 256 == 0) return u ^ (r & 7);
    else { static_assert((W * 2) % 128 == 0, "slab width"); return u ^ ((r >> 1) & 3); }
}

template <int FY, int FX, int TN, int TK, int WGN, int WGK, int SR, int NS, bool INPLACE = false>
__device__ __forceinline__ void slab_job(const SlProd& P, const int j, unsigned char* __restrict__ smem, [[maybe_unused]] unsigned long long* stamps) {
    static_assert(WGN * WGK == 8, "8 waves");
    constexpr int IA = TN / (16 * WGN), JB = TK / (16 * WGK);
    static_assert(IA * 16 * WGN == TN && JB * 16 * WGK == TK, "wave tiles");
    constexpr bool XF32 = FX == F_F32 || FX == F_F32G;
    constexpr int YP = TN * 2, XP = TK * 2;
    constexpr int YB = SR * TN * 2, XB = SR * TK * (XF32 ? 4 : 2), STG = YB + XB;
    constexpr int NY = YB / 1024, NX = XB / 1024, NTOT = NY + NX;
    static_assert(YB % 1024 == 0 && XB % 1024 == 0, "whole DMA instructions");
    constexpr int NIW = (NTOT + 7) / 8, NREM = NTOT % 8, D = NS - 1;
    constexpr int OFF_TAB = 0, TABB = FX == F_ROWG ? (GT_N * 2 + 1023) / 1024 * 1024 : 0;
    constexpr int OFF_IDX = OFF_TAB + TABB, IDXB = FX == F_F32G ? SL_IDX_CAP * 4 : 0;
    constexpr int OFF_SLOT = OFF_IDX + IDXB;
    constexpr int OFF_XB = OFF_SLOT + NS * STG, XBB = (XF32 && !INPLACE) ? SR * TK * 2 : 0;
    static_assert(OFF_XB + XBB <= SL_SMEM, "LDS budget");
    static_assert(!INPLACE || XF32, "in-place conversion: fp32 operands only");
    constexpr int KS = SR / 32;

    const int tid = threadIdx.x, lane = tid & 63, wave = __builtin_amdgcn_readfirstlane(tid >> 6);
    const int fr = lane & 15, g = lane >> 4;
    const int wgn = wave / WGK, wgk = wave - wgn * WGK;
    const int n_w = wgn * (TN / WGN), k_w = wgk * (TK / WGK);
    const int ntile = P.ntile, ntk = P.K / TK;
    const int slice = j / ntile, tile = j - slice * ntile, S = P.wgs / ntile;
    const int n0 = (tile / ntk) * TN, k0 = (tile % ntk) * TK;
    const int M = P.M, T = (M + SR - 1) / SR;
    const int nst = slice < T ? (T - slice + S - 1) / S : 0;
    auto stage_of = [&](int i) { return slice + i * S; };
    const uint32_t lds0 = (uint32_t)(uintptr_t)smem + OFF_SLOT;
    uint16_t* const xbs = (uint16_t*)(smem + OFF_XB);
    uint16_t* const tab = (uint16_t*)(smem + OFF_TAB);
    int32_t* const idxs = (int32_t*)(smem + OFF_IDX);

    if constexpr (FX == F_ROWG) {
        for (int i = tid; i < GT_N; i += SL_TH) tab[i] = f2bf(gelu_f(bf2f(gelu_tab_arg(i))));
    }
    constexpr int HS = SL_IDX_CAP / 2 / SR, RING = 2 * HS;
    auto fill_idx = [&](int h0) {
        for (int i = tid; i < HS * SR; i += SL_TH) {
            const int ti = h0 + i / SR;
            const int m = stage_of(ti) * SR + (i % SR);
            idxs[(ti % RING) * SR + (i % SR)] = (ti < nst && m < M) ? P.x.rowidx[m] : -1;
        }
    };
    if constexpr (FX == F_F32G) { fill_idx(0); fill_idx(HS); }
    if constexpr (FX == F_ROWG || FX == F_F32G) __syncthreads();

    int orow[NIW];
    uint32_t ocol[NIW];
#pragma unroll
    for (int q = 0; q < NIW; ++q) {
        const int ii = 8 * q + wave;
        if (ii < NY) {
            const int o = ii * 1024 + lane * 16;
            if constexpr (FY == F_ROW) {
                const int row = o / YP, rem = o - row * YP, pu = rem >> 5, u = sl_swz<TN>(row, pu);
                orow[q] = row; ocol[q] = (uint32_t)(n0 + u * 16 + ((rem >> 4) & 1) * 8);
            } else {
                static_assert(FY == F_HEAD, "dY kinds");
                const int blk = o / (SR * 32), rem = o - blk * (SR * 32), row = rem >> 5, col = n0 + blk * 16 + ((rem >> 4) & 1) * 8;
                const int ph = fdiv(col, P.y.DP, P.y.mgDP), jj = col - ph * P.y.DP, part = fdiv(ph, P.y.heads, P.y.mgH), hd = ph - part * P.y.heads;
                orow[q] = row; ocol[q] = (uint32_t)(((hd * P.y.parts + part) * P.y.Lp) * P.y.DP + jj);
            }
        } else {
            const int o = (ii - NY) * 1024 + lane * 16;
            if constexpr (FX == F_ROW || FX == F_ROWG) {
                const int row = o / XP, rem = o - row * XP, pu = rem >> 5, u = sl_swz<TK>(row, pu);
                orow[q] = row; ocol[q] = (uint32_t)(k0 + u * 16 + ((rem >> 4) & 1) * 8);
            } else if constexpr (XF32) {
                const int row = o / (TK * 4), rem = o - row * (TK * 4);
                orow[q] = row; ocol[q] = (uint32_t)(k0 + (rem >> 2));
            } else {
                const int blk = o / (SR * 32), rem = o - blk * (SR * 32), row = rem >> 5, col = k0 + blk * 16 + ((rem >> 4) & 1) * 8;
                const int ph = fdiv(col, P.x.DP, P.x.mgDP), jj = col - ph * P.x.DP, part = fdiv(ph, P.x.heads, P.x.mgH), hd = ph - part * P.x.heads;
                orow[q] = row; ocol[q] = (uint32_t)(((hd * P.x.parts + part) * P.x.Lp) * P.x.DP + jj);
            }
        }
    }
    const uint32_t ywst = FY == F_HEAD ? (uint32_t)(P.y.heads * P.y.parts * P.y.Lp * P.y.DP) : 0u;
    const uint32_t xwst = FX == F_HEAD ? (uint32_t)(P.x.heads * P.x.parts * P.x.Lp * P.x.DP) : 0u;
    auto issue_q = [&](int ti, int slot, auto qtag) {
        constexpr int q = decltype(qtag)::value;
        const int ii = 8 * q + wave;
        if (NREM != 0 && q == NIW - 1 && ii >= NTOT) return;
        const int t = stage_of(ti);
        const uint32_t lslot = lds0 + (uint32_t)(slot * STG) + (uint32_t)(ii * 1024);
        if (ii < NY) {
            const int m = min(t * SR + orow[q], M - 1);
            uint32_t off;
            if constexpr (FY == F_ROW) off = 2u * ((uint32_t)m * (uint32_t)P.y.ld + ocol[q]);
            else {
                const int bw = fdiv(m, P.y.Lp, P.y.mgLp), tt = m - bw * P.y.Lp;
                off = 2u * ((uint32_t)bw * ywst + (uint32_t)(tt * P.y.DP) + ocol[q]);
            }
            dma_x4(P.y.ptr, off, lslot);
        } else {
            uint32_t off;
            if constexpr (FX == F_F32G) {
                const int r = max(idxs[(ti % RING) * SR + orow[q]], 0);
                off = 4u * ((uint32_t)r * (uint32_t)P.x.ld + ocol[q]);
            } else {
                const int m = min(t * SR + orow[q], M - 1);
                if constexpr (FX == F_ROW || FX == F_ROWG) off = 2u * ((uint32_t)m * (uint32_t)P.x.ld + ocol[q]);
                else if constexpr (FX == F_F32) off = 4u * ((uint32_t)m * (uint32_t)P.x.ld + ocol[q]);
                else {
                    const int bw = fdiv(m, P.x.Lp, P.x.mgLp), tt = m - bw * P.x.Lp;
                    off = 2u * ((uint32_t)bw * xwst + (uint32_t)(tt * P.x.DP) + ocol[q]);
                }
            }
            dma_x4(P.x.ptr, off, lslot);
        }
    };
    auto issue_range = [&](int ti, int slot, auto lo, auto hi) {
        constexpr int LO = decltype(lo)::value, HI = decltype(hi)::value;
        [&]<int... Q>(std::integer_sequence<int, Q...>) { (issue_q(ti, slot, std::integral_constant<int, LO + Q>{}), ...); }
        (std::make_integer_sequence<int, HI - LO>{});
    };
    auto issue = [&](int ti, int slot) { issue_range(ti, slot, std::integral_constant<int, 0>{}, std::integral_constant<int, NIW>{}); };
    constexpr int NP = 1 + JB * KS;
    auto issue_point = [&](int ti, int slot, auto ptag) {
        constexpr int p_ = decltype(ptag)::value;
        issue_range(ti, slot, std::integral_constant<int, p_ * NIW / NP>{}, std::integral_constant<int, (p_ + 1) * NIW / NP>{});
    };

    f32x4 acc[IA][JB];
#pragma unroll
    for (int i = 0; i < IA; ++i)
#pragma unroll
        for (int jj = 0; jj < JB; ++jj) acc[i][jj] = (f32x4){0.f, 0.f, 0.f, 0.f};
    constexpr int NDB = (IA + WGK - 1) / WGK;
    f32x4 accdb[NDB];
#pragma unroll
    for (int e = 0; e < NDB; ++e) accdb[e] = (f32x4){0.f, 0.f, 0.f, 0.f};
    const bool want_db = P.dbpart != nullptr && k0 == 0;
// ... 35 lines not shown
            const uint16_t* Xs = (const uint16_t*)(sb + YB);
            if ((stage_of(t) + 1) * SR > M) {
                for (int c = tid; c < YB / 16; c += SL_TH) {
                    const int row = FY == F_ROW ? (c * 16) / YP : ((c * 16) % (SR * 32)) >> 5;
                    if (stage_of(t) * SR + row >= M) *(uint4*)(sb + c * 16) = make_uint4(0, 0, 0, 0);
                }
                __syncthreads();
            }
            if constexpr (XF32) {
                constexpr int NCH = SR * TK / 8, NPASS = (NCH + SL_TH - 1) / SL_TH;
                uint16_t* const xdst = INPLACE ? (uint16_t*)(sb + YB) : xbs;
                uint4 cv[NPASS];
#pragma unroll
                for (int ps = 0; ps < NPASS; ++ps) {
                    const int c = min(tid + ps * SL_TH, NCH - 1), row = c / (TK / 8), ch = c - row * (TK / 8);
                    const float* src = (const float*)(sb + YB) + row * TK + ch * 8;
                    RawF32 v = {*(const f32x4*)src, *(const f32x4*)(src + 4)};
                    cv[ps] = cvt_f32x8(v);
                    if constexpr (FX == F_F32G) {
                        if (idxs[(t % RING) * SR + row] < 0) cv[ps] = make_uint4(0, 0, 0, 0);
                    }
                }
                if constexpr (INPLACE) __syncthreads();
#pragma unroll
                for (int ps = 0; ps < NPASS; ++ps) {
                    const int c = tid + ps * SL_TH, row = c / (TK / 8), ch = c - row * (TK / 8);
                    if (c < NCH) *(uint4*)(xdst + row * TK + (sl_swz<TK>(row, ch >> 1) << 4) + (ch & 1) * 8) = cv[ps];
                }
                __syncthreads();
                Xs = xdst;
            }
            STAMP_DRAINED(3);
#pragma unroll
            for (int kk = 0; kk < KS; ++kk) {
                auto read_a = [&](int i) -> bf16x8 {
                    bf16x4 a0, a1;
                    if constexpr (FY == F_ROW) {
                        a0 = tr_row(Ys, std::integral_constant<int, TN>{}, 32 * kk, n_w + 16 * i);
                        a1 = tr_row(Ys, std::integral_constant<int, TN>{}, 32 * kk + 16, n_w + 16 * i);
                    } else {
                        a0 = tr_head(Ys, 32 * kk, n_w + 16 * i);
                        a1 = tr_head(Ys, 32 * kk + 16, n_w + 16 * i);
                    }
                    return __builtin_shufflevector(a0, a1, 0, 1, 2, 3, 4, 5, 6, 7);
                };
                auto read_b = [&](auto jtag) -> bf16x8 {
                    constexpr int jj = decltype(jtag)::value;
                    bf16x4 b0, b1;
                    if constexpr (FX == F_HEAD) {
                        b0 = tr_head(Xs, 32 * kk, k_w + 16 * jj);
                        b1 = tr_head(Xs, 32 * kk + 16, k_w + 16 * jj);
                    } else {
                        b0 = tr_row(Xs, std::integral_constant<int, TK>{}, 32 * kk, k_w + 16 * jj);
                        b1 = tr_row(Xs, std::integral_constant<int, TK>{}, 32 * kk + 16, k_w + 16 * jj);
                    }
                    bf16x8 b = __builtin_shufflevector(b0, b1, 0, 1, 2, 3, 4, 5, 6, 7);
                    if constexpr (FX == F_ROWG) {
                        const uint4 raw = __builtin_bit_cast(uint4, b);
                        bool bad;
                        uint4 gv = sl_gelu8_tab(raw, smem + OFF_TAB, bad);
                        if (__builtin_expect(__any((int)bad), 0)) gv = glf.cvt(raw);
                        b = __builtin_bit_cast(bf16x8, gv);
                    }
                    [&]<int... KK>(std::integer_sequence<int, KK...>) {
                        ((kk == KK ? issue_point(ti_n, slot_n, std::integral_constant<int, 1 + KK * JB + jj>{}) : (void)0), ...);
                    }(std::make_integer_sequence<int, KS>{});
                    return b;
                };
                if (kk == 0) issue_point(ti_n, slot_n, std::integral_constant<int, 0>{});
                if constexpr (JB <= 4) {
                    bf16x8 bf[JB];
                    [&]<int... JJ>(std::integer_sequence<int, JJ...>) { ((bf[JJ] = read_b(std::integral_constant<int, JJ>{})), ...); }
                    (std::make_integer_sequence<int, JB>{});
                    STAMP_DRAINED(4);
#pragma unroll
                    for (int i0 = 0; i0 < IA; i0 += 4) {
                        bf16x8 af[4];
#pragma unroll
                        for (int i = i0; i < i0 + 4 && i < IA; ++i) af[i - i0] = read_a(i);
#pragma unroll
                        for (int i = i0; i < i0 + 4 && i < IA; ++i) {
#pragma unroll
                            for (int jj = 0; jj < JB; ++jj) acc[i][jj] = mfma32(af[i - i0], bf[jj], acc[i][jj]);
                            if (want_db && i % WGK == wgk) accdb[i / WGK] = mfma32(af[i - i0], ones, accdb[i / WGK]);
                        }
                    }
                } else {
                    static_assert(IA <= 4, "one side of the wave tile has at most four fragments");
                    bf16x8 af[IA];
#pragma unroll
                    for (int i = 0; i < IA; ++i) af[i] = read_a(i);
                    if (want_db) {
#pragma unroll
                        for (int i = 0; i < IA; ++i)
                            if (i % WGK == wgk) accdb[i / WGK] = mfma32(af[i], ones, accdb[i / WGK]);
                    }
                    [&]<int... J0>(std::integer_sequence<int, J0...>) { ([&] {
                        constexpr int j0 = 4 * J0;
                        bf16x8 bf[4];
                        [&]<int... JJ>(std::integer_sequence<int, JJ...>) {
                            (((j0 + JJ < JB) ? (void)(bf[JJ] = read_b(std::integral_constant<int, (j0 + JJ < JB ? j0 + JJ : 0)>{})) : (void)0), ...);
                        }(std::make_integer_sequence<int, 4>{});
#pragma unroll
                        for (int jj = j0; jj < j0 + 4 && jj < JB; ++jj)
#pragma unroll
                            for (int i = 0; i < IA; ++i) acc[i][jj] = mfma32(af[i], bf[jj - j0], acc[i][jj]);
                    }(), ...); }(std::make_integer_sequence<int, (JB + 3) / 4>{});
                    STAMP_DRAINED(4);
                }
#ifdef SWV2_SLAB_STAMPS
                asm volatile("" :: "v"(acc[0][0][0]), "v"(acc[IA - 1][JB - 1][3]));
#endif
                STAMP_DRAINED(5);
            }
        }
        asm volatile("s_waitcnt vmcnt(0)" ::: "memory");
    }
    {
        constexpr int CPT = 8 * IA * JB;
        sl_part_t* out = P.part + ((size_t)(tile * CPT + wave * IA * JB) * S + slice) * 256 + lane * 4;
#pragma unroll
        for (int i = 0; i < IA; ++i)
#pragma unroll
            for (int jj = 0; jj < JB; ++jj) {
#ifdef SWV2_SLAB_PART_F32
                *(f32x4*)(out + (size_t)(i * JB + jj) * S * 256) = acc[i][jj];
#else
                *(bf16x4*)(out + (size_t)(i * JB + jj) * S * 256) = f2bf4(acc[i][jj]);
#endif
            }
    }
#ifdef SWV2_SLAB_STAMPS
    asm volatile("s_waitcnt vmcnt(0)" ::: "memory");
    STAMP_DRAINED(6);
    if (tid == 0 && stamps) {
#pragma unroll
        for (int k = 0; k < 8; ++k) stamps[(size_t)blockIdx.x * 8 + k] = st_acc[k];
    }
#endif
    if (want_db && fr == 0) {
#pragma unroll
        for (int i = 0; i < IA; ++i)
            if (i % WGK == wgk) {
#pragma unroll
                for (int r = 0; r < 4; ++r) P.dbpart[(size_t)slice * P.N + n0 + n_w + 16 * i + 4 * g + r] = accdb[i / WGK][r];
            }
    }
}

__global__ __launch_bounds__(SL_TH) void gemm_tn_slab_c128_kernel(SlArgs a) {
    __shared__ __attribute__((aligned(1024))) unsigned char smem[SL_SMEM];
    const int b = blockIdx.x;
    if (b < a.p[1].first) slab_job<F_ROW, F_ROWG, 128, 512, 1, 8, 32, 3>(a.p[0], b - a.p[0].first, smem, a.stamps);
    else if (b < a.p[2].first) slab_job<F_ROW, F_F32, 512, 128, 8, 1, 32, 3>(a.p[1], b - a.p[1].first, smem, a.stamps);
    else if (b < a.p[3].first) slab_job<F_ROW, F_HEAD, 128, 128, 2, 4, 64, 4>(a.p[2], b - a.p[2].first, smem, a.stamps);
    else slab_job<F_HEAD, F_F32G, 384, 128, 8, 1, 32, 3>(a.p[3], b - a.p[3].first, smem, a.stamps);
}
__global__ __launch_bounds__(SL_TH) void gemm_tn_slab_c192_kernel(SlArgs a) {
    __shared__ __attribute__((aligned(1024))) unsigned char smem[SL_SMEM];
    const int b = blockIdx.x;
    if (b < a.p[1].first) slab_job<F_ROW, F_ROWG, 192, 384, 1, 8, 32, 3>(a.p[0], b - a.p[0].first, smem, a.stamps);
    else if (b < a.p[2].first) slab_job<F_ROW, F_F32, 384, 192, 8, 1, 32, 3>(a.p[1], b - a.p[1].first, smem, a.stamps);
    else if (b < a.p[3].first) slab_job<F_ROW, F_HEAD, 192, 256, 2, 4, 32, 4>(a.p[2], b - a.p[2].first, smem, a.stamps);
    else slab_job<F_HEAD, F_F32G, 384, 192, 8, 1, 32, 3, true>(a.p[3], b - a.p[3].first, smem, a.stamps);
}

struct SlLnRed { const float* ws[2]; float* dg[2]; float* db[2]; int n[2]; int C; };
struct SlRed { float* dW; float* db; const int32_t* nmap; const int32_t* kmap; const sl_part_t* part; const float* dbpart;
               int ldw, N, K, TN, TK, WGK, IA, JB, ntk, S, first, dbfirst; };
struct SlRedArgs { SlRed p[4]; int total, dbtotal; SlLnRed ln; int cpw; };
__global__ __launch_bounds__(512) void tn_slab_reduce_kernel(SlRedArgs a) {
    __shared__ f32x4 red[8][64];
    const int b = blockIdx.x;
    const int lane = threadIdx.x & 63, sg = threadIdx.x >> 6;
    if (b >= a.total + a.dbtotal) {
        const int bb = b - a.total - a.dbtotal, per_set = (2 * a.ln.C + 15) / 16;
        const int set = bb / per_set, col = threadIdx.x & 15, sl = threadIdx.x >> 4;
        const int jc = (bb - set * per_set) * 16 + col;
        float sum = 0.f;
        if (jc < 2 * a.ln.C) {
            const float* w = a.ln.ws[set];
#pragma unroll 4
            for (int r = sl; r < a.ln.n[set]; r += 32) sum += w[(size_t)r * 2 * a.ln.C + jc];
        }
        float* redf = (float*)red;
        redf[sl * 16 + col] = sum;
        __syncthreads();
        for (int hh = 16; hh > 0; hh >>= 1) {
            if (sl < hh) redf[sl * 16 + col] += redf[(sl + hh) * 16 + col];
            __syncthreads();
        }
        if (sl == 0 && jc < 2 * a.ln.C) {
            if (jc < a.ln.C) a.ln.dg[set][jc] += redf[col]; else a.ln.db[set][jc - a.ln.C] += redf[col];
        }
        return;
    }
    if (b >= a.total) {
        const int bb = b - a.total;
        const int pi = (bb >= a.p[1].dbfirst) + (bb >= a.p[2].dbfirst) + (bb >= a.p[3].dbfirst);
        const SlRed& p = a.p[pi];
        const int n = (bb - p.dbfirst) * 64 + lane;
        float a0 = 0.f, a1 = 0.f;
        if (p.db && p.dbpart && n < p.N) {
            int q = sg;
            for (; q + 8 < p.S; q += 16) { a0 += p.dbpart[(size_t)q * p.N + n]; a1 += p.dbpart[(size_t)(q + 8) * p.N + n]; }
            if (q < p.S) a0 += p.dbpart[(size_t)q * p.N + n];
        }
        float* redf = (float*)red;
        redf[sg * 64 + lane] = a0 + a1;
        __syncthreads();
        if (sg == 0 && p.db && p.dbpart && n < p.N) {
            const int nn = p.nmap ? p.nmap[n] : n;
            float t = 0.f;
#pragma unroll
            for (int e = 0; e < 8; ++e) t += redf[e * 64 + lane];
            if (nn >= 0) p.db[nn] += t;
        }
        return;
    }
    const int pi = (b >= a.p[1].first) + (b >= a.p[2].first) + (b >= a.p[3].first);
    const SlRed& p = a.p[pi];
    const int NG = 8 / a.cpw;
    const int cg = (b - p.first) * a.cpw + sg / NG, sl0 = sg % NG;
    int kk = -1, nn[4] = {-1, -1, -1, -1};
    float old[4] = {0.f, 0.f, 0.f, 0.f};
    if (sl0 == 0) {
        const int cpt = 8 * p.IA * p.JB, tile = cg / cpt, c = cg - tile * cpt;
        const int wave = c / (p.IA * p.JB), ij = c - wave * (p.IA * p.JB), i = ij / p.JB, jj = ij - i * p.JB;
        const int wgn = wave / p.WGK, wgk = wave - wgn * p.WGK, g = lane >> 4, fr = lane & 15;
        const int n0 = (tile / p.ntk) * p.TN + wgn * p.IA * 16 + 16 * i + 4 * g;
        const int k = (tile % p.ntk) * p.TK + wgk * p.JB * 16 + 16 * jj + fr;
        kk = p.kmap ? p.kmap[k] : k;
#pragma unroll
        for (int r = 0; r < 4; ++r) nn[r] = p.nmap ? p.nmap[n0 + r] : n0 + r;
#pragma unroll
        for (int r = 0; r < 4; ++r) old[r] = p.dW[(long)max(nn[r], 0) * p.ldw + max(kk, 0)];
    }
    const sl_part_t* src = p.part + (size_t)cg * p.S * 256 + lane * 4;
#ifdef SWV2_SLAB_PART_F32
    auto ld = [](const sl_part_t* q) -> f32x4 { return *(const f32x4*)q; };
#else
    auto ld = [](const sl_part_t* q) -> f32x4 {
        const bf16x4 v = *(const bf16x4*)q;
        return (f32x4){bf2f(v[0]), bf2f(v[1]), bf2f(v[2]), bf2f(v[3])};
    };
#endif
    f32x4 s0 = {0.f, 0.f, 0.f, 0.f}, s1 = s0, s2 = s0, s3 = s0;
    int s = sl0;
    for (; s + 3 * NG < p.S; s += 4 * NG) {
        s0 += ld(src + (size_t)s * 256);
        s1 += ld(src + (size_t)(s + NG) * 256);
        s2 += ld(src + (size_t)(s + 2 * NG) * 256);
        s3 += ld(src + (size_t)(s + 3 * NG) * 256);
    }
    for (; s < p.S; s += NG) s0 += ld(src + (size_t)s * 256);
    red[sg][lane] = (s0 + s1) + (s2 + s3);
    __syncthreads();
    if (sl0 == 0 && kk >= 0) {
        f32x4 t;
        if (a.cpw == 1) t = ((red[0][lane] + red[1][lane]) + (red[2][lane] + red[3][lane])) + ((red[4][lane] + red[5][lane]) + (red[6][lane] + red[7][lane]));
        else t = (red[sg][lane] + red[sg + 1][lane]) + (red[sg + 2][lane] + red[sg + 3][lane]);
#pragma unroll
        for (int r = 0; r < 4; ++r)
            if (nn[r] >= 0) p.dW[(long)nn[r] * p.ldw + kk] = old[r] + t[r];
    }
}

struct SlShape { int TN[4], TK[4], SR[4], WGN[4], WGK[4]; };
const SlShape SL_SETS[2] = {{{128, 512, 128, 384}, {512, 128, 128, 128}, {32, 32, 64, 32}, {1, 8, 2, 8}, {8, 1, 4, 1}},
                            {{192, 384, 192, 384}, {384, 192, 256, 192}, {32, 32, 32, 32}, {1, 8, 2, 8}, {8, 1, 4, 1}}};
const int SL_BLOCKS[2][4] = {{128, 512, 8, 16}, {192, 768, 8, 32}};
int sl_set(int C, int hidden, int heads_dp) {
    for (int i = 0; i < 2; ++i)
        if (C == SL_BLOCKS[i][0] && hidden == SL_BLOCKS[i][1] && heads_dp == SL_BLOCKS[i][2] * SL_BLOCKS[i][3]) return i;
    return -1;
}

constexpr int SL_CU_BOUND = 320;
int sl_cus() {
    static thread_local int cus[16] = {};
    int dev = 0;
    if (hipGetDevice(&dev) != hipSuccess || dev < 0 || dev >= 16) return 256;
    if (!cus[dev]) {
        int v = 0;
        if (hipDeviceGetAttribute(&v, hipDeviceAttributeMultiprocessorCount, dev) != hipSuccess || v <= 0) v = 256;
        cus[dev] = v < SL_CU_BOUND ? v : SL_CU_BOUND;
    }
    return cus[dev];
}

struct SlPlan { bool ok; int set; int wgs[4], ntile[4], S[4]; size_t part_off[4], db_off[4], total; };

SlPlan sl_plan(const swv2_wgrad_item* it, int cus) {
    SlPlan p = {};
    const int N[4] = {it[0].dy.cols, it[1].dy.cols, it[2].dy.cols, it[3].dy.cols};
    const int K[4] = {it[0].x.cols, it[1].x.cols, it[2].x.cols, it[3].x.cols};
    const int C = N[0], hid = K[0];
    p.set = sl_set(C, hid, K[2]);
    if (p.set < 0) return p;
    const SlShape& sh = SL_SETS[p.set];
    if (!(N[1] == hid && K[1] == C && N[2] == C && N[3] == 3 * K[2] && K[3] == C)) return p;
    if (!(it[2].x.p[3] == SL_BLOCKS[p.set][3] && it[3].dy.p[3] == SL_BLOCKS[p.set][3] && it[2].x.p[0] == SL_BLOCKS[p.set][2] &&
          it[3].dy.p[0] == SL_BLOCKS[p.set][2])) return p;
    if (!(it[0].dy.ld == C && it[0].x.ld == hid && it[1].dy.ld == hid && it[1].x.ld == C && it[2].dy.ld == C && it[3].x.ld == C)) return p;
    if (cus < 16 || cus > 1024) return p;
    double cost[4], tot = 0;
    const double wgt[4] = {1.55, 1.0, 1.0, 1.1};
    for (int i = 0; i < 4; ++i) {
        const double xb = it[i].x.kind == SWV2_OP_F32 ? 4.0 : 2.0;
        p.ntile[i] = (N[i] / sh.TN[i]) * (K[i] / sh.TK[i]);
        cost[i] = wgt[i] * (double)it[i].dy.rows * (2.0 * N[i] * (K[i] / sh.TK[i]) + xb * K[i] * (N[i] / sh.TN[i]));
        tot += cost[i];
    }
    int used = 0;
    for (int i = 0; i < 4; ++i) {
        const int T = cdiv(it[i].dy.rows, sh.SR[i]);
        int sl = (int)(cus * cost[i] / tot / p.ntile[i] + 0.5);
        sl = std::max(1, std::min(sl, T));
        p.S[i] = sl;
        p.wgs[i] = sl * p.ntile[i];
        used += p.wgs[i];
    }
    for (int guard = 0; used != cus && guard < 64; ++guard) {
        int best = -1;
        double br = 0;
        for (int i = 0; i < 4; ++i) {
            const int T = cdiv(it[i].dy.rows, sh.SR[i]);
            if (used < cus ? (p.S[i] >= T || used + p.ntile[i] > cus) : p.S[i] <= 1) continue;
            const double r = cost[i] / p.S[i];
            if (best < 0 || (used < cus ? r > br : r < br)) { best = i; br = r; }
        }
        if (best < 0) break;
        const int d = used < cus ? 1 : -1;
        p.S[best] += d; p.wgs[best] += d * p.ntile[best]; used += d * p.ntile[best];
    }
    size_t off = 0;
    for (int i = 0; i < 4; ++i) {
        const int T = cdiv(it[i].dy.rows, sh.SR[i]);
        if ((double)it[i].dy.rows * std::max(N[i], K[i]) * 4.0 >= 4.29e9) return p;
        p.part_off[i] = off;
        off += (size_t)p.wgs[i] * sh.TN[i] * sh.TK[i] * sizeof(float);
        p.db_off[i] = off;
        off += (size_t)p.S[i] * N[i] * sizeof(float);
        off = (off + 255) / 256 * 256;
    }
    p.total = off;
    p.ok = true;
    return p;
}

SlOp sl_op(const swv2_operand& o) {
    SlOp s = {};
    s.ptr = o.ptr; s.rowidx = o.rowidx; s.ld = (int)o.ld;
    if (o.kind == SWV2_OP_HEADS) {
        s.heads = o.p[0]; s.parts = (int)o.ld; s.Lp = o.p[2]; s.DP = o.p[3];
        s.mgLp = fdiv_magic(s.Lp); s.mgDP = fdiv_magic(s.DP); s.mgH = fdiv_magic(s.heads);
    }
    return s;
}

}

size_t swv2_tn_slab_ws_bytes(int C, int hidden, int heads_dp) {
    const int set = sl_set(C, hidden, heads_dp);
    if (set < 0) return 0;
    const int cus = SL_CU_BOUND;
    const SlShape& sh = SL_SETS[set];
    size_t tile = 0;
    for (int i = 0; i < 4; ++i) tile = std::max(tile, (size_t)sh.TN[i] * sh.TK[i] * 4);
    return (size_t)cus * tile + (size_t)cus * std::max(hidden, 3 * heads_dp) * 4 + 4 * 256;
}

bool swv2_tn_slab_covers(const swv2_wgrad_item* it, size_t ws_bytes) {
    const SlPlan pl = sl_plan(it, sl_cus());
    if (pl.ok && ws_bytes < pl.total) {
        static int once = 0;
        if (!once++) fprintf(stderr, "swv2: grouped weight gradient declined (workspace %zu bytes, %zu needed): size it with swv2_block_wgrad_ws_bytes; "
                                     "running the 128 x 128 tile kernels\n", ws_bytes, pl.total);
    }
    return pl.ok && ws_bytes >= pl.total;
}

int swv2_tn_slab_launch(const swv2_wgrad_item* it, void* ws, size_t ws_bytes, const swv2_ln_partials* ln, hipStream_t st) {
    const SlPlan pl = sl_plan(it, sl_cus());
    SWV2_CHECK_ARG(pl.ok && ws_bytes >= pl.total, "swv2_block_wgrad(slab): items or workspace not covered (swv2_tn_slab_covers)");
    const SlShape& sh = SL_SETS[pl.set];
    SlArgs a = {};
    SlRedArgs r = {};
    int first = 0, rfirst = 0, dbfirst = 0;
    int cpw = 2;
    for (int i = 0; i < 4; ++i)
        if (pl.S[i] > 40 || ((it[i].dy.cols * it[i].x.cols / 256) & 1)) cpw = 1;
    r.cpw = cpw;
    for (int i = 0; i < 4; ++i) {
        SlProd& p = a.p[i];
        p.y = sl_op(it[i].dy); p.x = sl_op(it[i].x);
        p.part = (sl_part_t*)((char*)ws + pl.part_off[i]);
        p.dbpart = it[i].db ? (float*)((char*)ws + pl.db_off[i]) : nullptr;
        p.M = it[i].dy.rows; p.N = it[i].dy.cols; p.K = it[i].x.cols;
        p.first = first; p.wgs = pl.wgs[i]; p.ntile = pl.ntile[i];
        first += pl.wgs[i];
        SlRed& q = r.p[i];
        q.dW = it[i].dW; q.db = it[i].db; q.nmap = it[i].nmap; q.kmap = it[i].kmap; q.part = p.part; q.dbpart = p.dbpart;
        q.ldw = it[i].ldw; q.N = p.N; q.K = p.K; q.TN = sh.TN[i]; q.TK = sh.TK[i]; q.WGK = sh.WGK[i];
        q.IA = sh.TN[i] / (16 * sh.WGN[i]); q.JB = sh.TK[i] / (16 * sh.WGK[i]); q.ntk = p.K / sh.TK[i]; q.S = pl.S[i]; q.first = rfirst;
        rfirst += p.N * p.K / 256 / cpw;
        q.dbfirst = dbfirst;
        dbfirst += cdiv(p.N, 64);
    }
    r.total = rfirst;
    r.dbtotal = dbfirst;
    int lnblocks = 0;
    if (ln && ln->C > 0) {
        for (int i = 0; i < 2; ++i) { r.ln.ws[i] = ln->ws[i]; r.ln.dg[i] = ln->dgamma[i]; r.ln.db[i] = ln->dbeta[i]; r.ln.n[i] = ln->n[i]; }
        r.ln.C = ln->C;
        lnblocks = 2 * cdiv(2 * ln->C, 16);
    }
#ifdef SWV2_SLAB_STAMPS
    if (ws_bytes >= pl.total + (size_t)first * 64) a.stamps = (unsigned long long*)((char*)ws + ws_bytes - (size_t)first * 64);
    { static int once = 0; if (!once++) fprintf(stderr, "slab plan: workgroups %d %d %d %d\n", pl.wgs[0], pl.wgs[1], pl.wgs[2], pl.wgs[3]); }
#endif
    if (pl.set == 0) hipLaunchKernelGGL(gemm_tn_slab_c128_kernel, dim3(first), dim3(SL_TH), 0, st, a);
    else hipLaunchKernelGGL(gemm_tn_slab_c192_kernel, dim3(first), dim3(SL_TH), 0, st, a);
    hipLaunchKernelGGL(tn_slab_reduce_kernel, dim3(rfirst + dbfirst + lnblocks), dim3(512), 0, st, r);
    SWV2_CHECK_LAUNCH("swv2_block_wgrad(slab)");
    return 0;
}
```

swin_v2_weather_amd/csrc/proj_ln.hip:

```cpp
#include <cstdlib>
#include "gemm_common.h"
#include "ln_common.h"

namespace {

constexpr int PL_MAX_HDP = 128;

template <int ROWS, int COLS, int PITCH, int NT>
__device__ __forceinline__ void stage_weight(uint16_t* dst, const uint16_t* __restrict__ src, int rows, int cols, int tid) {
    typedef uint32_t u32x4 __attribute__((ext_vector_type(4)));
    constexpr int CPRW = COLS / 8, CHUNKS = ROWS * CPRW, PER = (CHUNKS + NT - 1) / NT, B = PER < 6 ? PER : 6;
#pragma unroll
    for (int j0 = 0; j0 < PER; j0 += B) {
        u32x4 v[B];
#pragma unroll
        for (int u = 0; u < B; ++u) {
            const int i = tid + (j0 + u) * NT, r = i / CPRW, c8 = i % CPRW;
            v[u] = *(const u32x4*)(src + (size_t)min(r, rows - 1) * cols + min(8 * c8, cols - 8));
        }
#pragma unroll
        for (int u = 0; u < B; ++u) {
            const int i = tid + (j0 + u) * NT, r = i / CPRW, c8 = i % CPRW;
            if (j0 + u < PER && r < rows && 8 * c8 < cols) *(u32x4*)(dst + r * PITCH + 8 * c8) = v[u];
        }
    }
}

struct ProjLnFwd {
    const uint16_t* oh; const uint16_t* wp; const float* bp; const float* gamma; const float* beta; const float* scale;
    const int32_t* rowidx; const float* x; uint16_t* a1; float* mean; float* rstd; float* y;
    int Mw, Lp, h, rows_per_sample; float eps;
};

template <int C, int MT, int HS = 16, int NW = 4>
__global__ __launch_bounds__(64 * NW, NW == 4 ? 2 : 1) void proj_ln_fwd_kernel(const ProjLnFwd a) {
    constexpr int NTC = C / 16, NT = 64 * NW;
    constexpr int HDPM = 8 * HS;
    constexpr int PWP = HDPM + 8, PA = C + 8;
    constexpr int EWAVE = 16 * PA * 2 + 16 * 2 * 4;
    constexpr int KSM = HDPM / 32;
    static_assert(C * PWP * 2 + NW * EWAVE + 3 * C * 4 <= 160 * 1024, "LDS budget");
    __shared__ __attribute__((aligned(16))) uint16_t Wps[C * PWP];
    __shared__ __attribute__((aligned(16))) unsigned char epi[NW * EWAVE];
    __shared__ __attribute__((aligned(16))) float cs[3 * C];
    typedef uint32_t u32x4 __attribute__((ext_vector_type(4)));

    const int tid = threadIdx.x, lane = tid & 63, wave = tid >> 6, fr = lane & 15, g = lane >> 4;
    const int hdp = a.h * HS, ksn = hdp / 32;
    const int row0 = blockIdx.x * (16 * NW * MT) + wave * (16 * MT);

    constexpr int UNITS = 16 * (C / 8), NP = (UNITS + 63) / 64;
    int dstv[MT][NP];
    f32x4 xr[MT][NP][2];
    float scv[MT][NP];
#pragma unroll
    for (int mt = 0; mt < MT; ++mt)
#pragma unroll
        for (int p = 0; p < NP; ++p) {
            const int u = min(lane + 64 * p, UNITS - 1), row = u / (C / 8);
            const int m = min(row0 + 16 * mt + row, a.Mw - 1);
            dstv[mt][p] = a.rowidx ? a.rowidx[m] : m;
        }
    bf16x8 xf[MT][KSM];
#pragma unroll
    for (int mt = 0; mt < MT; ++mt) {
        const int m = min(row0 + 16 * mt + fr, a.Mw - 1), w = m / a.Lp, t = m - w * a.Lp;
#pragma unroll
        for (int ks = 0; ks < KSM; ++ks) {
            const int k0 = 32 * ks + 8 * g, kc = min(k0, hdp - 8);
            xf[mt][ks] = *(const bf16x8*)(a.oh + (((size_t)w * a.h + kc / HS) * a.Lp + t) * HS + (kc & (HS - 1)));
        }
    }
    stage_weight<C, HDPM, PWP, NT>(Wps, a.wp, C, hdp, tid);
    for (int i = tid; i < C; i += NT) { cs[i] = a.bp[i]; cs[C + i] = a.gamma[i]; cs[2 * C + i] = a.beta[i]; }
#pragma unroll
    for (int mt = 0; mt < MT; ++mt)
#pragma unroll
        for (int p = 0; p < NP; ++p) {
            const int u = min(lane + 64 * p, UNITS - 1), c8 = u % (C / 8);
            const size_t off = (size_t)max(dstv[mt][p], 0) * C + 8 * c8;
            xr[mt][p][0] = *(const f32x4*)(a.x + off);
            xr[mt][p][1] = *(const f32x4*)(a.x + off + 4);
            scv[mt][p] = (a.scale ? a.scale : a.gamma)[a.scale ? max(dstv[mt][p], 0) / a.rows_per_sample : 0];
        }
    __syncthreads();

    f32x4 yacc[MT][NTC];
#pragma unroll
    for (int mt = 0; mt < MT; ++mt)
#pragma unroll
        for (int tn = 0; tn < NTC; ++tn) yacc[mt][tn] = (f32x4){0.f, 0.f, 0.f, 0.f};
#pragma unroll
    for (int ks = 0; ks < KSM; ++ks) {
        if (ks < ksn) {
#pragma unroll
            for (int tn = 0; tn < NTC; ++tn) {
                const bf16x8 wf = *(const bf16x8*)(Wps + (16 * tn + fr) * PWP + 32 * ks + 8 * g);
#pragma unroll
                for (int mt = 0; mt < MT; ++mt) yacc[mt][tn] = mfma32(wf, xf[mt][ks], yacc[mt][tn]);
            }
        }
    }

    uint16_t* As = (uint16_t*)(epi + wave * EWAVE);
    float* St = (float*)(As + 16 * PA);
#pragma unroll
    for (int mt = 0; mt < MT; ++mt) {
        float s = 0.f;
#pragma unroll
        for (int tn = 0; tn < NTC; ++tn) {
            const f32x4 bv = *(const f32x4*)(cs + 16 * tn + 4 * g);
            const bf16x4 ar = f2bf4(yacc[mt][tn] + bv);
            *(bf16x4*)(As + fr * PA + 16 * tn + 4 * g) = ar;
#pragma unroll
            for (int e = 0; e < 4; ++e) { yacc[mt][tn][e] = bf2f(ar[e]); s += yacc[mt][tn][e]; }
        }
        s = xor32_allsum(xor16_allsum(s));
        const float mu = s * (1.f / C);
        float q = 0.f;
#pragma unroll
        for (int tn = 0; tn < NTC; ++tn)
#pragma unroll
            for (int e = 0; e < 4; ++e) { const float d = yacc[mt][tn][e] - mu; q = fmaf(d, d, q); }
        q = xor32_allsum(xor16_allsum(q));
        const float rs = rsqrtf(q * (1.f / C) + a.eps);
        if (g == 0) {
            const int m = min(row0 + 16 * mt + fr, a.Mw - 1);
            a.mean[m] = mu;
            a.rstd[m] = rs;
            St[2 * fr] = mu;
            St[2 * fr + 1] = rs;
        }
        __syncthreads();
#pragma unroll
        for (int p = 0; p < NP; ++p) {
            const int u = lane + 64 * p, row = u / (C / 8), c8 = u % (C / 8);
            if (UNITS % 64 == 0 || u < UNITS) {
                const int m = min(row0 + 16 * mt + row, a.Mw - 1);
                const u32x4 av = *(const u32x4*)(As + row * PA + 8 * c8);
                *(u32x4*)(a.a1 + (size_t)m * C + 8 * c8) = av;
                const int dst = dstv[mt][p];
                if (dst >= 0) {
                    const float mu_r = St[2 * row], rs_r = St[2 * row + 1];
                    const float sc = a.scale ? scv[mt][p] : 1.f;
                    const size_t off = (size_t)dst * C + 8 * c8;
                    float v[8];
                    unpack8(__builtin_bit_cast(uint4, av), v);
#pragma unroll
                    for (int hlf = 0; hlf < 2; ++hlf) {
                        const f32x4 gm = *(const f32x4*)(cs + C + 8 * c8 + 4 * hlf), bt = *(const f32x4*)(cs + 2 * C + 8 * c8 + 4 * hlf);
                        f32x4 o = xr[mt][p][hlf];
#pragma unroll
                        for (int e = 0; e < 4; ++e) o[e] += sc * ((v[4 * hlf + e] - mu_r) * rs_r * gm[e] + bt[e]);
                        *(f32x4*)(a.y + off + 4 * hlf) = o;
                    }
                }
            }
        }
        if (mt + 1 < MT) __syncthreads();
    }
}

struct ProjLnBwd {
    const float* dy; const uint16_t* a1; const float* mean; const float* rstd; const float* gamma; const float* scale;
    const int32_t* rowidx; const uint16_t* wpt; uint16_t* da1; uint16_t* doh; float* ws;
    int Mw, Lp, h, rows_per_sample;
};

template <int C, int MT, int HS = 16, int NW = 4>
__global__ __launch_bounds__(64 * NW, NW == 4 ? 2 : 1) void proj_ln_bwd_kernel(const ProjLnBwd a) {
    constexpr int KS = C / 32, NT = 64 * NW, HDPM = 8 * HS;
    constexpr int ROWS = 16 * NW * MT, PX = C + 8, PW = C + 8;
    typedef LnBwdShape<C, NT, ROWS> Sh;
    constexpr int LPR = Sh::LPR, RPP = Sh::RPP, NPASS = Sh::NPASS, BATCH = Sh::BATCH;
    constexpr bool TWO_ROUNDS = NW == 8;
    constexpr int GROWS = TWO_ROUNDS ? RPP / 2 : RPP;
    static_assert(HDPM * PW * 2 + ROWS * PX * 2 + GROWS * 2 * C * 4 <= 160 * 1024, "LDS budget");
    __shared__ __attribute__((aligned(16))) uint16_t Wts[HDPM * PW];
    __shared__ __attribute__((aligned(16))) uint16_t Xs[ROWS * PX];
    __shared__ __attribute__((aligned(16))) float gs[GROWS * 2 * C];
    typedef uint32_t u32x4 __attribute__((ext_vector_type(4)));
    typedef uint32_t u32x2 __attribute__((ext_vector_type(2)));

    const int tid = threadIdx.x, lane = tid & 63, wave = tid >> 6, fr = lane & 15, g = lane >> 4;
    const int hdp = a.h * HS;
    const int wg_row0 = blockIdx.x * ROWS;

    stage_weight<HDPM, C, PW, NT>(Wts, a.wpt, hdp, C, tid);
    {
        const int lr = tid % LPR, rg = tid / LPR;
        const bool act = 4 * lr < C;
        const int c0 = act ? 4 * lr : 0;
        const f32x4 gm = *(const f32x4*)(a.gamma + c0);
        f32x4 dgm = {0.f, 0.f, 0.f, 0.f}, dbt = {0.f, 0.f, 0.f, 0.f};
        int srcv[NPASS];
#pragma unroll
        for (int i = 0; i < NPASS; ++i) {
            const int m = min(wg_row0 + i * RPP + rg, a.Mw - 1);
            srcv[i] = a.rowidx ? a.rowidx[m] : m;
        }
        f32x4 d4s[2][BATCH];
        u32x2 a4s[2][BATCH];
        float mus[2][BATCH], rss[2][BATCH], scs[2][BATCH];
        int oks[2][BATCH];
        const float* scp = a.scale ? a.scale : a.gamma;
        auto load_batch = [&](int pb, auto set_c) {
            constexpr int S = decltype(set_c)::value;
#pragma unroll
            for (int i = 0; i < BATCH; ++i) {
                const int m = min(wg_row0 + (pb + i) * RPP + rg, a.Mw - 1);
                const int src = srcv[(pb + i) % NPASS];
                oks[S][i] = src >= 0;
                const int sr = max(src, 0);
                d4s[S][i] = *(const f32x4*)(a.dy + (size_t)sr * C + c0);
                a4s[S][i] = *(const u32x2*)(a.a1 + (size_t)m * C + c0);
                mus[S][i] = a.mean[m];
                rss[S][i] = a.rstd[m];
                scs[S][i] = scp[a.scale ? sr / a.rows_per_sample : 0];
            }
        };
        load_batch(0, std::integral_constant<int, 0>{});
#pragma unroll
        for (int pb = 0; pb < NPASS; pb += BATCH) {
            constexpr int dummy = 0; (void)dummy;
            const int cur = (pb / BATCH) & 1;
            if (pb + BATCH < NPASS) {
                if (cur == 0) load_batch(pb + BATCH, std::integral_constant<int, 1>{});
                else load_batch(pb + BATCH, std::integral_constant<int, 0>{});
            }
            f32x4 d4[BATCH];
            u32x2 a4[BATCH];
            float mu[BATCH], rs[BATCH], sc[BATCH];
            int ok[BATCH];
#pragma unroll
            for (int i = 0; i < BATCH; ++i) {
                d4[i] = d4s[cur][i]; a4[i] = a4s[cur][i]; mu[i] = mus[cur][i]; rs[i] = rss[cur][i];
                sc[i] = a.scale ? scs[cur][i] : 1.f; ok[i] = oks[cur][i];
            }
#pragma unroll
            for (int i = 0; i < BATCH; ++i) {
                const int row = (pb + i) * RPP + rg;
                const bool live = act && ok[i];
                const float once = (live && wg_row0 + row < a.Mw) ? 1.f : 0.f;
                const float av[4] = {__uint_as_float(a4[i][0] << 16), __uint_as_float(a4[i][0] & 0xffff0000u),
                                     __uint_as_float(a4[i][1] << 16), __uint_as_float(a4[i][1] & 0xffff0000u)};
                float gg[4], xh[4], t1 = 0.f, t2 = 0.f;
#pragma unroll
                for (int e = 0; e < 4; ++e) {
                    const float d = live ? sc[i] * d4[i][e] : 0.f;
                    xh[e] = (av[e] - mu[i]) * rs[i];
                    gg[e] = d * gm[e];
                    dgm[e] = fmaf(once * d, xh[e], dgm[e]);
                    dbt[e] = fmaf(once, d, dbt[e]);
                    t1 += gg[e];
                    t2 = fmaf(gg[e], xh[e], t2);
                }
                t1 = group_allsum<LPR>(t1); t2 = group_allsum<LPR>(t2);
                t1 *= (1.f / C); t2 *= (1.f / C);
                f32x4 o4;
#pragma unroll
                for (int e = 0; e < 4; ++e) o4[e] = ok[i] ? rs[i] * (gg[e] - t1 - xh[e] * t2) : 0.f;
                const bf16x4 ob = f2bf4(o4);
                if (act) {
                    *(bf16x4*)(a.da1 + (size_t)min(wg_row0 + row, a.Mw - 1) * C + c0) = ob;
                    *(bf16x4*)(Xs + row * PX + c0) = ob;
                }
            }
        }
        if constexpr (TWO_ROUNDS) {
            if (act && rg >= GROWS) {
                *(f32x4*)(gs + ((rg - GROWS) * 2 + 0) * C + c0) = dgm;
                *(f32x4*)(gs + ((rg - GROWS) * 2 + 1) * C + c0) = dbt;
            }
            __syncthreads();
            if (act && rg < GROWS) {
                dgm += *(const f32x4*)(gs + (rg * 2 + 0) * C + c0);
                dbt += *(const f32x4*)(gs + (rg * 2 + 1) * C + c0);
            }
            __syncthreads();
        }
        if (act && rg < GROWS) {
            *(f32x4*)(gs + (rg * 2 + 0) * C + c0) = dgm;
            *(f32x4*)(gs + (rg * 2 + 1) * C + c0) = dbt;
        }
        __syncthreads();
        for (int i = tid; i < 2 * C; i += NT) {
            float t = 0.f;
#pragma unroll
            for (int r = 0; r < GROWS; ++r) t += gs[r * 2 * C + i];
            a.ws[(size_t)blockIdx.x * 2 * C + i] = t;
        }
    }
#pragma unroll
    for (int mt = 0; mt < MT; ++mt) {
        bf16x8 xf[KS];
#pragma unroll
        for (int ks = 0; ks < KS; ++ks) xf[ks] = *(const bf16x8*)(Xs + (wave * 16 * MT + 16 * mt + fr) * PX + 32 * ks + 8 * g);
        const int m = min(wg_row0 + wave * 16 * MT + 16 * mt + fr, a.Mw - 1), w = m / a.Lp, t = m - w * a.Lp;
        for (int kt = 0; kt < a.h * (HS / 16); ++kt) {
            f32x4 acc = {0.f, 0.f, 0.f, 0.f};
#pragma unroll
            for (int ks = 0; ks < KS; ++ks) {
                const bf16x8 wf = *(const bf16x8*)(Wts + (16 * kt + fr) * PW + 32 * ks + 8 * g);
                acc = mfma32(wf, xf[ks], acc);
            }
            *(bf16x4*)(a.doh + (((size_t)w * a.h + kt / (HS / 16)) * a.Lp + t) * HS + 16 * (kt % (HS / 16)) + 4 * g) = f2bf4(acc);
        }
    }
}

}

extern "C" int swv2_proj_ln_supported(int C, int heads, int head_pad) {
    if (C == 192) return head_pad == 32 && heads >= 1 && heads <= 8;
    return (C == 32 || C == 64 || C == 96 || C == 128) && head_pad == 16 && heads >= 2 && heads % 2 == 0 && heads * 16 <= PL_MAX_HDP;
}

extern "C" size_t swv2_proj_ln_bwd_ws_floats(int Mw, int C) { return (Mw > 0 && C > 0) ? (size_t)cdiv(Mw, 64) * 2 * C : 0; }

extern "C" int swv2_proj_ln_fwd(const swv2_proj_ln_args* a, void* stream) {
    SWV2_CHECK_ARG(a && a->oh && a->wp && a->bp && a->gamma && a->beta && a->x && a->a1 && a->mean && a->rstd && a->y,
                   "swv2_proj_ln_fwd: null pointer");
    SWV2_CHECK_ARG(a->Bw > 0 && a->Lp > 0 && a->Lp % 16 == 0 && a->rows_per_sample > 0, "swv2_proj_ln_fwd: bad geometry");
    if (!swv2_proj_ln_supported(a->C, a->heads, a->C == 192 ? 32 : 16)) {
        swv2_set_error("swv2_proj_ln_fwd: C=%d heads=%d not instantiated; use swv2_linear + swv2_ln_residual_fwd", a->C, a->heads);
        return SWV2_ERR_UNSUPPORTED;
    }
    const int Mw = a->Bw * a->Lp;
    ProjLnFwd k = {(const uint16_t*)a->oh, (const uint16_t*)a->wp, a->bp, a->gamma, a->beta, a->scale, a->rowidx, a->x,
                   (uint16_t*)a->a1, a->mean, a->rstd, a->y, Mw, a->Lp, a->heads, a->rows_per_sample, a->eps};
    hipStream_t st = (hipStream_t)stream;
    const bool mt2 = Mw >= 128 * 256;
#define PL_CASE(CC)                                                                                                  \
    case CC:                                                                                                         \
        if (mt2) hipLaunchKernelGGL((proj_ln_fwd_kernel<CC, 2>), dim3(cdiv(Mw, 128)), dim3(256), 0, st, k);          \
        else hipLaunchKernelGGL((proj_ln_fwd_kernel<CC, 1>), dim3(cdiv(Mw, 64)), dim3(256), 0, st, k);               \
        break;
    switch (a->C) {
        PL_CASE(32) PL_CASE(64) PL_CASE(96) PL_CASE(128)
        case 192: hipLaunchKernelGGL((proj_ln_fwd_kernel<192, 1, 32, 8>), dim3(cdiv(Mw, 128)), dim3(512), 0, st, k); break;
    }
#undef PL_CASE
    SWV2_CHECK_LAUNCH("swv2_proj_ln_fwd");
    return SWV2_OK;
}

extern "C" int swv2_proj_ln_bwd(const swv2_proj_ln_bwd_args* a, void* stream) { return swv2_proj_ln_bwd_impl(a, stream, nullptr); }

int swv2_proj_ln_bwd_impl(const swv2_proj_ln_bwd_args* a, void* stream, int* deferred) {
    SWV2_CHECK_ARG(a && a->dy && a->a1 && a->mean && a->rstd && a->gamma && a->wpt && a->da1 && a->doh && a->dgamma && a->dbeta &&
                       a->ws, "swv2_proj_ln_bwd: null pointer");
    SWV2_CHECK_ARG(a->Bw > 0 && a->Lp > 0 && a->Lp % 16 == 0 && a->rows_per_sample > 0, "swv2_proj_ln_bwd: bad geometry");
    if (!swv2_proj_ln_supported(a->C, a->heads, a->C == 192 ? 32 : 16)) {
        swv2_set_error("swv2_proj_ln_bwd: C=%d heads=%d not instantiated; use swv2_ln_residual_bwd + swv2_linear", a->C, a->heads);
        return SWV2_ERR_UNSUPPORTED;
    }
    const int Mw = a->Bw * a->Lp;
    ProjLnBwd k = {a->dy, (const uint16_t*)a->a1, a->mean, a->rstd, a->gamma, a->scale, a->rowidx, (const uint16_t*)a->wpt,
                   (uint16_t*)a->da1, (uint16_t*)a->doh, a->ws, Mw, a->Lp, a->heads, a->rows_per_sample};
    hipStream_t st = (hipStream_t)stream;
    const bool mt2 = Mw >= 128 * 256;
#define PL_CASE(CC)                                                                                                  \
    case CC:                                                                                                         \
        if (mt2) hipLaunchKernelGGL((proj_ln_bwd_kernel<CC, 2>), dim3(cdiv(Mw, 128)), dim3(256), 0, st, k);          \
        else hipLaunchKernelGGL((proj_ln_bwd_kernel<CC, 1>), dim3(cdiv(Mw, 64)), dim3(256), 0, st, k);               \
        break;
    int nblk = cdiv(Mw, mt2 ? 128 : 64);
    switch (a->C) {
        PL_CASE(32) PL_CASE(64) PL_CASE(96) PL_CASE(128)
        case 192: nblk = cdiv(Mw, 128); hipLaunchKernelGGL((proj_ln_bwd_kernel<192, 1, 32, 8>), dim3(nblk), dim3(512), 0, st, k); break;
    }
#undef PL_CASE
    if (deferred) *deferred = nblk;
    else swv2_launch_ln_partials_reduce(a->ws, a->dgamma, a->dbeta, nblk, a->C, st);
    SWV2_CHECK_LAUNCH("swv2_proj_ln_bwd");
    return SWV2_OK;
}
```

swin_v2_weather_amd/networks/swinv2_global.py:

```python
from __future__ import annotations

import math
import os
from types import SimpleNamespace
from typing import Any, List, Optional, Tuple, Type, Union

import torch
import torch.nn as nn
import torch.nn.functional as F
from torch.utils.checkpoint import checkpoint

from .. import _lib as L
from .. import ops

BF16 = torch.bfloat16


def to_2tuple(x):
    return tuple(x) if isinstance(x, (tuple, list)) else (x, x)


def bchw_to_bhwc(x: torch.Tensor) -> torch.Tensor:
    return x.permute(0, 2, 3, 1)


def bhwc_to_bchw(x: torch.Tensor) -> torch.Tensor:
    return x.permute(0, 3, 1, 2)


def _need_gpu(x: torch.Tensor, who: str):
    if not x.is_cuda:
        raise L.Swv2Error(f"{who}: the swv2 hot path runs on an MI355X only (got a {x.device} tensor); there is no "
                          "CPU fallback")


def _zeros_like_shapes(device, *shapes):
    sizes = [((int(torch.Size(s).numel()) + 3) // 4) * 4 for s in shapes]
    flat = torch.zeros(sum(sizes), dtype=torch.float32, device=device)
    out, off = [], 0
    for s, n in zip(shapes, sizes):
        out.append(flat[off:off + int(torch.Size(s).numel())].view(*s))
        off += n
    return out


_OPT_EPOCH = [0]


def _bump_opt_epoch(*_a, **_k):
    _OPT_EPOCH[0] += 1


from torch.optim.optimizer import register_optimizer_step_post_hook as _reg_opt_hook

_reg_opt_hook(_bump_opt_epoch)


class _WeightCache:

    def __init__(self):
        self._c = {}

    @staticmethod
    def _ver(params):
        return tuple((p.data_ptr(), p._version, _OPT_EPOCH[0]) for p in params)

    def get(self, key, params, builder):
        ver = self._ver(params)
        hit = self._c.get(key)
        if hit is not None and hit[0] == ver:
            return hit[1]
        with torch.no_grad():
            val = builder()
        self._c[key] = (ver, val)
        return val

    def prep(self, key, w, batch, **spec):
        ver = self._ver((w,))
        hit = self._c.get(key)
        if hit is not None and hit[0] == ver:
            return hit[1]
        val = batch.add(w, out=None if hit is None else hit[1], **spec)
        self._c[key] = (None, val)
        batch.on_launched(lambda c=self._c, k=key, v=(ver, val): c.__setitem__(k, v))
        return val


def window_partition(x, window_size: Tuple[int, int]):
    B, H, W, C = x.shape
    x = x.view(B, H // window_size[0], window_size[0], W // window_size[1], window_size[1], C)
    return x.permute(0, 1, 3, 2, 4, 5).contiguous().view(-1, window_size[0], window_size[1], C)


def window_reverse(windows, window_size: Tuple[int, int], img_size: Tuple[int, int]):
    H, W = img_size
    C = windows.shape[-1]
    x = windows.view(-1, H // window_size[0], W // window_size[1], window_size[0], window_size[1], C)
    return x.permute(0, 1, 3, 2, 4, 5).contiguous().view(-1, H, W, C)


def _carve(sizes, align=256):
    offs, off = [], 0
    for s in sizes:
        offs.append(off)
        off += (s + align - 1) // align * align
    return offs, off


class _BlockRunner:

    ACTS = ("qkvh", "rnorm", "oh", "lse", "a1", "mean1", "rstd1", "x1", "hpre", "hact", "a2", "mean2", "rstd2", "bias_pack")
    SCRATCH = ("da2", "dh", "da1", "doh", "dqkvh", "dx1", "ln_ws", "wgrad_ws")

    def __init__(self, blk, plan, Cc, hid, device):
        self.plan, self.C, self.hid, self.device = plan, Cc, hid, device
        h, Lp, DP, Bw, B, T, Lw = plan.heads, plan.Lp, plan.DP, plan.Bw, plan.B, plan.T, plan.L
        BT, Mw = B * T, Bw * Lp
        d = L.BlockDesc()
        d.B, d.T, d.C, d.heads, d.head_dim, d.hidden = B, T, Cc, h, plan.d, hid
        d.L, d.Lp, d.DP, d.nwh, d.nww, d.mask_thr = Lw, Lp, DP, plan.nwh, plan.nww, plan.mask_thr
        d.rowidx, d.qkv_map, d.proj_map = plan.rowidx.data_ptr(), plan.qkv_map.data_ptr(), plan.proj_map.data_ptr()
        d.wgrad_splits = int(os.environ.get("SWV2_WGRAD_SPLITS", "128"))
        d.wgrad_group = int(os.environ.get("SWV2_WGRAD_GROUP", "1"))
        d.fuse_mlp = int(os.environ.get("SWV2_FUSE_MLP", "1"))
        d.fuse_proj_ln = int(os.environ.get("SWV2_FUSE_PROJ_LN", "1"))
        d.wgrad_ws = d.grad_zero = 1
        d.ln_ws_floats = d.wgrad_ws_bytes = 1 << 62
        full = L.block_plan(d)
        d.ln_ws_floats, d.wgrad_ws_bytes = full.need_ln_ws_floats, full.need_wgrad_ws_bytes
        self.launch_plan = lp = L.block_plan(d)
        if any(getattr(lp, n) != getattr(full, n) for n in ("mlp_fused", "proj_ln_fused", "ln_deferred", "wgrad_grouped", "wgrad_kernel")):
            raise L.Swv2Error("swv2_block_plan: the reported workspace needs do not cover the full plan")
        d.wgrad_ws = d.grad_zero = None
        self.desc = d
        act_sizes = [Bw * h * 3 * Lp * DP * 2, Bw * h * 2 * Lp * 4, Bw * h * Lp * DP * 2, Bw * h * Lp * 4, Mw * Cc * 2, Mw * 4,
                     Mw * 4, BT * Cc * 4, BT * hid * 2, lp.need_hact_bytes, BT * Cc * 2, BT * 4, BT * 4,
                     L.load().swv2_attn_pack_bias_bytes(h, Lw)]
        self.act_off, self.act_bytes = _carve(act_sizes)
        scr_sizes = [BT * Cc * 2, BT * hid * 2, Mw * Cc * 2, Bw * h * Lp * DP * 2, Bw * h * 3 * Lp * DP * 2, BT * Cc * 4,
                     d.ln_ws_floats * 4, d.wgrad_ws_bytes]
        self.scr_off, self.scr_bytes = _carve(scr_sizes)
        self.grad_shapes = [(h,), (3 * Cc, Cc), (3 * Cc,), (Cc, Cc), (Cc,), (Cc,), (Cc,), (hid, Cc), (hid,), (Cc, hid), (Cc,),
                            (Cc,), (Cc,)]
        self.grad_names = ["d_logit_scale", "d_qkv_w", "d_qkv_b", "d_proj_w", "d_proj_b", "d_n1_w", "d_n1_b", "d_fc1_w",
                           "d_fc1_b", "d_fc2_w", "d_fc2_b", "d_n2_w", "d_n2_b"]
        gs = [int(torch.Size(s).numel()) * 4 for s in self.grad_shapes]
        self.grad_off, self.grad_bytes = _carve(gs, 64)
        self.bias_elems = h * Lw * Lw

    def set_params(self, wc, logit_scale, qkv_w, qkv_b, proj_w, proj_b, n1_w, n1_b, fc1_w, fc1_b, fc2_w, fc2_b, n2_w, n2_b,
                   backward, batch=None):
        plan, d = self.plan, self.desc
        h, DP = plan.heads, plan.DP
        own = batch is None
        if own:
            batch = ops.PrepBatch()
        keep = [wc.prep("qkv", qkv_w, batch, row_map=plan.qkv_map, out_rows=3 * h * DP),
                wc.prep("qkv_b", qkv_b, batch, row_map=plan.qkv_map, out_rows=3 * h * DP, f32=True),
                wc.prep("proj", proj_w, batch, col_map=plan.proj_map, out_cols=h * DP),
                wc.prep("fc1", fc1_w, batch),
                wc.prep("fc2", fc2_w, batch)]
        d.w_qkv, d.qkv_b_pad, d.w_proj, d.w_fc1, d.w_fc2 = (t.data_ptr() for t in keep)
        if backward:
            kb = [wc.prep("qkvt", qkv_w, batch, transpose=True, col_map=plan.qkv_map, out_cols=3 * h * DP),
                  wc.prep("projt", proj_w, batch, transpose=True, row_map=plan.proj_map, out_rows=h * DP),
                  wc.prep("fc1t", fc1_w, batch, transpose=True),
                  wc.prep("fc2t", fc2_w, batch, transpose=True)]
            d.w_qkvt, d.w_projt, d.w_fc1t, d.w_fc2t = (t.data_ptr() for t in kb)
            keep += kb
        if own:
            batch.launch()
        d.logit_scale, d.proj_b, d.n1_w, d.n1_b = logit_scale.data_ptr(), proj_b.data_ptr(), n1_w.data_ptr(), n1_b.data_ptr()
        d.fc1_b, d.fc2_b, d.n2_w, d.n2_b = fc1_b.data_ptr(), fc2_b.data_ptr(), n2_w.data_ptr(), n2_b.data_ptr()
        return keep

    def set_acts(self, acts):
        base, d = acts.data_ptr(), self.desc
        for name, off in zip(self.ACTS, self.act_off):
            setattr(d, name, base + off)


class _BlockFn(torch.autograd.Function):
    @staticmethod
    def forward(ctx, x, bias, dp1, dp2, logit_scale, qkv_w, qkv_b, proj_w, proj_b, n1_w, n1_b, fc1_w, fc1_b, fc2_w,
                fc2_b, n2_w, n2_b, blk, ckpt=0, cpb=None):
        B, gh, gw, Cc = x.shape
        run = blk._runner(B, x.device)
        d = run.desc
        x = x.contiguous()
        keep = run.set_params(blk._wcache, logit_scale, qkv_w, qkv_b, proj_w, proj_b, n1_w, n1_b, fc1_w, fc1_b, fc2_w, fc2_b,
                              n2_w, n2_b, backward=False)
        bias_c = None if (bias is None or cpb is not None) else bias.detach().float().contiguous()
        acts = torch.empty(run.act_bytes, dtype=torch.uint8, device=x.device)
        x2 = torch.empty(B, gh, gw, Cc, dtype=torch.float32, device=x.device)
        run.set_acts(acts)
        d.x, d.x2 = x.data_ptr(), x2.data_ptr()
        d.bias = None if bias_c is None else bias_c.data_ptr()
        d.bias_prepacked, d.dbias_part, d.dbias_part_bytes = 0, None, 0
        if cpb is not None:
            cpb[0].point(d, cpb[1])
        d.dp1 = None if dp1 is None else dp1.data_ptr()
        d.dp2 = None if dp2 is None else dp2.data_ptr()
        ops.block_event_pair("fwd", d)
        L.check(ops._timed("block_fwd", L.load().swv2_block_fwd, run.desc, ops._stream()), "swv2_block_fwd")
        del keep
        ctx.blk, ctx.run, ctx.has_bias, ctx.ckpt, ctx.cpb = blk, run, bias is not None, int(ckpt), cpb
        e = x.new_empty(0)
        if ckpt:
            acts = e
            xs = x.to(BF16) if ckpt == 2 else x
        else:
            xs = x
        ctx.save_for_backward(xs, bias_c if bias_c is not None else e, dp1 if dp1 is not None else e, dp2 if dp2 is not None else e,
                              acts, logit_scale, qkv_w, qkv_b, proj_w, proj_b, n1_w, n1_b, fc1_w, fc1_b, fc2_w, fc2_b, n2_w, n2_b)
        return x2

    @staticmethod
    def backward(ctx, dx2):
        (x, bias_c, dp1, dp2, acts, logit_scale, qkv_w, qkv_b, proj_w, proj_b, n1_w, n1_b, fc1_w, fc1_b, fc2_w, fc2_b, n2_w,
         n2_b) = ctx.saved_tensors
        blk, run, cpb = ctx.blk, ctx.run, ctx.cpb
        d = run.desc
        dev = x.device
        keep = run.set_params(blk._wcache, logit_scale, qkv_w, qkv_b, proj_w, proj_b, n1_w, n1_b, fc1_w, fc1_b, fc2_w, fc2_b,
                              n2_w, n2_b, backward=True)
        dx2 = dx2.contiguous().float()
        own_bias = ctx.has_bias and cpb is None
        d.bias_prepacked, d.dbias_part, d.dbias_part_bytes = 0, None, 0
        if ctx.ckpt:
            x = x.float() if x.dtype != torch.float32 else x
            acts = torch.empty(run.act_bytes, dtype=torch.uint8, device=dev)
            x2_tmp = torch.empty_like(x)
            run.set_acts(acts)
            d.x, d.x2 = x.data_ptr(), x2_tmp.data_ptr()
            d.bias = bias_c.data_ptr() if own_bias else None
            if cpb is not None:
                cpb[0].point(d, cpb[1])
            d.dp1 = dp1.data_ptr() if dp1.numel() else None
            d.dp2 = dp2.data_ptr() if dp2.numel() else None
            d.ev_kernel = 0
            L.check(L.load().swv2_block_fwd(run.desc, ops._stream()), "swv2_block_fwd (recompute)")
            del x2_tmp
        run.set_acts(acts)
        scratch = torch.empty(run.scr_bytes, dtype=torch.uint8, device=dev)
        sb = scratch.data_ptr()
        for name, off in zip(run.SCRATCH, run.scr_off):
            setattr(d, name, sb + off)
        params = (logit_scale, qkv_w, qkv_b, proj_w, proj_b, n1_w, n1_b, fc1_w, fc1_b, fc2_w, fc2_b, n2_w, n2_b)
        wants_param_grads = any(ctx.needs_input_grad[4:17])
        reuse = blk._pass_grads_of(torch._C._current_graph_task_id()) \
            if (wants_param_grads and os.environ.get("SWV2_GRAD_ACC_INPLACE", "1") != "0") else None
        views = blk._bucket_views(params) if (reuse is None and blk._ddp_bucket_grads and not blk._bv_in_use) else None
        dbias_view = None
        if reuse is not None:
            for name, ptr in zip(run.grad_names, reuse):
                setattr(d, name, ptr)
            d.grad_zero, d.grad_zero_bytes = None, 0
            if ctx.has_bias and cpb is None:
                dbias_view = torch.zeros_like(bias_c)
        elif views is not None:
            blk._bv_in_use = True
            torch._foreach_zero_(views)
            for name, v in zip(run.grad_names, views):
                setattr(d, name, v.data_ptr())
            d.grad_zero, d.grad_zero_bytes = None, 0
        else:
            in_kernel = bool(run.launch_plan.grad_zero_in_kernel)
            nfl = (run.grad_bytes // 4 + 3) // 4 * 4
            nb = (bias_c.numel() + 3) // 4 * 4 if own_bias else 0
            grads = (torch.empty if in_kernel else torch.zeros)(nfl + nb, dtype=torch.float32, device=dev)
            gb = grads.data_ptr()
            d.grad_zero, d.grad_zero_bytes = (gb, (nfl + nb) * 4) if in_kernel else (None, 0)
            if nb:
                dbias_view = grads[nfl:nfl + bias_c.numel()].view_as(bias_c)
            for name, off in zip(run.grad_names, run.grad_off):
                setattr(d, name, gb + off)
        if blk._ddp_bucket_grads and reuse is None:
            blk._queue_view_refresh(params)
        dbias = (dbias_view if dbias_view is not None else torch.zeros_like(bias_c)) if own_bias else None
        dx = torch.empty_like(x)
        d.x, d.dx2, d.dx = x.data_ptr(), dx2.data_ptr(), dx.data_ptr()
        d.bias = bias_c.data_ptr() if own_bias else None
        d.d_bias = dbias.data_ptr() if own_bias else None
        if cpb is not None:
            cpb[0].point(d, cpb[1], backward=True)
        d.dp1 = dp1.data_ptr() if dp1.numel() else None
        d.dp2 = dp2.data_ptr() if dp2.numel() else None
        ops.block_event_pair("bwd", d)
        L.check(ops._timed("block_bwd", L.load().swv2_block_bwd, run.desc, ops._stream()), "swv2_block_bwd")
        del keep
        if reuse is not None:
            return (dx, dbias) + (None,) * 18
        if views is not None:
            g = [v.detach() for v in views]
        else:
            g = [grads[o // 4:o // 4 + int(torch.Size(s).numel())].view(*s) for o, s in zip(run.grad_off, run.grad_shapes)]
        if wants_param_grads:
            blk._remember_pass_grads(g, None if views is not None else grads, torch._C._current_graph_task_id())
        (dlogit, dqkvw, dqkvb, dprojw, dprojb, dn1w, dn1b, dfc1w, dfc1b, dfc2w, dfc2b, dn2w, dn2b) = g
        return (dx, dbias, None, None, dlogit, dqkvw, dqkvb, dprojw, dprojb, dn1w, dn1b, dfc1w, dfc1b, dfc2w, dfc2b, dn2w,
                dn2b, None, None, None)


class _CpbFn(torch.autograd.Function):

    @staticmethod
    def forward(ctx, w1, b1, w2, b2, keep, wh, ww, drop_p):
        heads, hidden = w2.shape
        Lw = wh * ww
        w1c, b1c, w2c, b2c = (t.detach().float().contiguous() for t in (w1, b1, w2, b2))
        bias = torch.empty(heads, Lw, Lw, dtype=torch.float32, device=w1.device)
        ops.cpb_fwd(w1c, b1c, w2c, b2c, keep, bias, wh, ww, heads, hidden, drop_p)
        ctx.geom = (wh, ww, heads, hidden, drop_p)
        ctx.save_for_backward(w1c, b1c, w2c, keep if keep is not None else w1c.new_empty(0))
        return bias

    @staticmethod
    def backward(ctx, dbias):
        w1c, b1c, w2c, keep = ctx.saved_tensors
        wh, ww, heads, hidden, drop_p = ctx.geom
        dev = w1c.device
        flat = torch.zeros(hidden * 2 + hidden + heads * hidden + heads, device=dev)
        dw1, db1, dw2, db2 = flat.split([hidden * 2, hidden, heads * hidden, heads])
        dw1, dw2 = dw1.view(hidden, 2), dw2.view(heads, hidden)
        ops.cpb_bwd(dbias.contiguous().float(), w1c, b1c, w2c, keep if keep.numel() else None, dw1, db1, dw2, db2, wh, ww, heads,
                    hidden, drop_p)
        return dw1, db1, dw2, db2, None, None, None, None


class _CpbStage:

    def __init__(self, blocks, device):
# ... 788 lines not shown
```

swin_v2_weather_amd/ops.py:

```python
from __future__ import annotations

import ctypes as C
import functools
from typing import Optional

import torch

from . import _lib as L

BF16 = torch.bfloat16


def _p(t: Optional[torch.Tensor]):
    return None if t is None else t.data_ptr()


def _stream():
    return torch.cuda.current_stream().cuda_stream


_TIMED = None


_EVERY = 1
# ... 568 lines not shown
    out = torch.empty(K, B, Cc, dtype=torch.float32, device=x.device)
    nan_count = torch.empty(B, Cc, dtype=torch.int32, device=x.device)
    L.check(L.load().swv2_plane_order_stats(_p(x), x.stride(0) if B > 1 else Cc * H * W, B, Cc, H, W, _p(ranks), K, _p(out), _p(nan_count),
                                            _p(ws), ws.numel() * 4, _stream()), "swv2_plane_order_stats")
    return out, nan_count


def stats_slices(Cc: int, H: int, W: int) -> int:
    return int(L.load().swv2_stats_slices(Cc, H, W))


def stats_workspace(Cc: int, H: int, W: int, device) -> torch.Tensor:
    return torch.empty(int(L.load().swv2_stats_ws_bytes(Cc, H, W)) // 8, dtype=torch.float64, device=device).view(Cc, -1, 6)


def stats_accumulate(slab, prev, pivot, tsum, part, first: bool, stream=None):
    _chk(slab, torch.float32, "stats slab"); _chk(pivot, torch.float64, "stats pivot")
    _chk(tsum, torch.float64, "stats tsum"); _chk(part, torch.float64, "stats workspace")
    if slab.dim() != 3 or tsum.shape != slab.shape or pivot.numel() != slab.shape[0]:
        raise L.Swv2Error(f"stats_accumulate: slab {tuple(slab.shape)}, tsum {tuple(tsum.shape)}, pivot {tuple(pivot.shape)}: expected "
                          "[C, H, W], [C, H, W], [C]")
    if prev is not None and _chk(prev, torch.float32, "stats prev").shape != slab.shape:
        raise L.Swv2Error(f"stats_accumulate: prev {tuple(prev.shape)}, slab {tuple(slab.shape)}")
    Cc, H, W = slab.shape
    L.check(L.load().swv2_stats_accumulate(_p(slab), _p(prev), _p(pivot), _p(tsum), _p(part), part.numel() * 8, Cc, H, W, int(bool(first)),
                                           stream if stream is not None else _stream()), "swv2_stats_accumulate")


def stats_finalize(part, tsum, pivot, T: int, stream=None):
    _chk(part, torch.float64, "stats workspace"); _chk(tsum, torch.float64, "stats tsum"); _chk(pivot, torch.float64, "stats pivot")
    if tsum.dim() != 3 or pivot.numel() != tsum.shape[0]:
        raise L.Swv2Error(f"stats_finalize: tsum {tuple(tsum.shape)}, pivot {tuple(pivot.shape)}: expected [C, H, W], [C]")
    Cc, H, W = tsum.shape
    folded = torch.empty(Cc, 6, dtype=torch.float64, device=tsum.device)
    time_means = torch.empty(Cc, H, W, dtype=torch.float32, device=tsum.device)
    L.check(L.load().swv2_stats_finalize(_p(part), part.numel() * 8, _p(tsum), _p(pivot), Cc, H, W, int(T), _p(folded), _p(time_means),
                                         stream if stream is not None else _stream()), "swv2_stats_finalize")
    return folded, time_means


def era5_select_normalize(raw, out, chan, mean, std, coff=0, stream=None):
    B, S, Craw, Hraw, Wraw = raw.shape
    _, Ct, H, W = out.shape
    _chk(raw, torch.float32, "era5 raw"); _chk(out, torch.float32, "era5 out")
    L.check(L.load().swv2_era5_select_normalize(_p(raw), _p(out), _p(chan), _p(mean), _p(std), B, S, chan.numel(), Craw, Hraw, Wraw,
                                                H, W, Ct, coff, stream if stream is not None else _stream()), "swv2_era5_select_normalize")


def era5_select_normalize_i16(raw, out, chan, mean, std, offset, scale, slab_row, coff=0, stream=None):
    B, S, Craw, Hraw, Wraw = raw.shape
    _, Ct, H, W = out.shape
    _chk(raw, torch.int16, "era5 packed raw"); _chk(out, torch.float32, "era5 out")
    _chk(offset, torch.float32, "era5 pack offset"); _chk(scale, torch.float32, "era5 pack scale"); _chk(slab_row, torch.int32, "era5 slab_row")
    if offset.dim() != 2 or offset.shape[1] != Craw or scale.shape != offset.shape or slab_row.numel() != B * S:
        raise L.Swv2Error(f"era5_select_normalize_i16: offset {tuple(offset.shape)}, scale {tuple(scale.shape)}, slab_row {tuple(slab_row.shape)}: "
                          f"expected [rows, {Craw}] twice and [{B}, {S}]")
    L.check(L.load().swv2_era5_select_normalize_i16(_p(raw), _p(out), _p(chan), _p(mean), _p(std), _p(offset), _p(scale), _p(slab_row), B, S,
                                                    chan.numel(), Craw, Hraw, Wraw, H, W, Ct, coff,
                                                    stream if stream is not None else _stream()), "swv2_era5_select_normalize_i16")


def _pack_slab_args(who, i16, f32, offset, scale):
    _chk(i16, torch.int16, who + " int16 slab"); _chk(f32, torch.float32, who + " fp32 slab")
    _chk(offset, torch.float32, who + " offset"); _chk(scale, torch.float32, who + " scale")
    if f32.dim() != 3 or i16.shape != f32.shape or offset.numel() != f32.shape[0] or scale.numel() != f32.shape[0]:
        raise L.Swv2Error(f"{who}: int16 {tuple(i16.shape)}, fp32 {tuple(f32.shape)}, offset {tuple(offset.shape)}, scale {tuple(scale.shape)}: "
                          "expected [C, H, W] twice and [C] twice")
    return f32.shape


def era5_unpack_i16(raw, out, offset, scale, stream=None):
    Cc, H, W = _pack_slab_args("era5_unpack_i16", raw, out, offset, scale)
    L.check(L.load().swv2_era5_unpack_i16(_p(raw), _p(out), _p(offset), _p(scale), Cc, H, W,
                                          stream if stream is not None else _stream()), "swv2_era5_unpack_i16")


def era5_pack_i16(slab, out, offset, scale, stream=None):
    Cc, H, W = _pack_slab_args("era5_pack_i16", out, slab, offset, scale)
    L.check(L.load().swv2_era5_pack_i16(_p(slab), _p(out), _p(offset), _p(scale), Cc, H, W,
                                        stream if stream is not None else _stream()), "swv2_era5_pack_i16")


def pack_range_workspace(Cc: int, H: int, W: int, device) -> torch.Tensor:
    return torch.empty(int(L.load().swv2_pack_range_ws_bytes(Cc, H, W)), dtype=torch.uint8, device=device)


def pack_range(slab, rng, missing, ws, first: bool, stream=None):
    _chk(slab, torch.float32, "pack_range slab"); _chk(rng, torch.float32, "pack_range range"); _chk(missing, torch.int64, "pack_range missing")
    _chk(ws, torch.uint8, "pack_range workspace")
    if slab.dim() != 3 or tuple(rng.shape) != (slab.shape[0], 2) or missing.numel() != slab.shape[0]:
        raise L.Swv2Error(f"pack_range: slab {tuple(slab.shape)}, range {tuple(rng.shape)}, missing {tuple(missing.shape)}: expected [C, H, W], "
                          "[C, 2], [C]")
    Cc, H, W = slab.shape
    L.check(L.load().swv2_pack_range(_p(slab), Cc, H, W, int(bool(first)), _p(rng), _p(missing), _p(ws), ws.numel(),
                                     stream if stream is not None else _stream()), "swv2_pack_range")


def era5_zenith(out, sun, coff, stream=None):
    B, Ct, H, W = out.shape
    _chk(sun, torch.float32, "era5_zenith sun")
    if sun.dim() != 3 or sun.shape[0] != B or sun.shape[2] != 3:
        raise L.Swv2Error(f"era5_zenith: sun must be [B, nz, 3], got {tuple(sun.shape)}")
    L.check(L.load().swv2_era5_zenith(_p(out), _p(sun), B, sun.shape[1], H, W, Ct, coff,
                                      stream if stream is not None else _stream()), "swv2_era5_zenith")


def era5_static(stat, out, coff, stream=None):
    B, Ct, H, W = out.shape
    L.check(L.load().swv2_era5_static(_p(stat), _p(out), B, stat.shape[0], H, W, Ct, coff,
                                      stream if stream is not None else _stream()), "swv2_era5_static")


def adam_step(p, g, m, v, lr, beta1, beta2, eps, step, grad_inv_scale=1.0):
    L.check(L.load().swv2_adam_step(_p(p), _p(g), _p(m), _p(v), p.numel(), lr, beta1, beta2, eps, step, grad_inv_scale,
                                    _stream()), "swv2_adam_step")


def mlp_fwd(x, w1, b1, w2, b2, gamma, beta, scale, rows_per_sample, eps=1e-5, keep_hpre=True, out=None):
    M, Cc = x.shape
    hid = w1.shape[0]
    _chk(x, torch.float32, "mlp x"); _chk(w1, BF16, "mlp w1"); _chk(w2, BF16, "mlp w2")
    dev = x.device
    if out is None:
        out = (torch.empty(M, Cc, dtype=torch.float32, device=dev), torch.empty(M, hid, dtype=BF16, device=dev) if keep_hpre else None,
               torch.empty(M, Cc, dtype=BF16, device=dev), torch.empty(M, device=dev), torch.empty(M, device=dev))
    y, hpre, a2, mean, rstd = out
    a = L.MlpArgs()
    a.x, a.w1, a.b1, a.w2, a.b2, a.gamma, a.beta, a.scale = (_p(t) for t in (x, w1, b1, w2, b2, gamma, beta, scale))
    a.hpre, a.a2, a.mean, a.rstd, a.y = (_p(t) for t in (hpre, a2, mean, rstd, y))
    a.M, a.C, a.hidden, a.rows_per_sample, a.eps = M, Cc, hid, rows_per_sample, eps
    L.check(_timed("mlp_fwd", L.load().swv2_mlp_fwd, C.byref(a), _stream()), "swv2_mlp_fwd")
    return y, hpre, a2, mean, rstd


def mlp_bwd(dy, a2, mean, rstd, gamma, scale, hpre, w2t, w1t, dgamma, dbeta, rows_per_sample, x=None, w1=None, b1=None, out=None, ws=None):
    M, Cc = dy.shape
    hid = w2t.shape[0]
    dev = dy.device
    if out is None:
        out = (torch.empty(M, Cc, dtype=torch.float32, device=dev), torch.empty(M, Cc, dtype=BF16, device=dev),
               torch.empty(M, hid, dtype=BF16, device=dev))
    if ws is None:
        ws = torch.empty(L.load().swv2_mlp_bwd_ws_floats(M, Cc), dtype=torch.float32, device=dev)
    dx, da2, dh = out
    a = L.MlpBwdArgs()
    a.dy, a.a2, a.mean, a.rstd, a.gamma, a.scale, a.hpre, a.w2t, a.w1t = (_p(t) for t in (dy, a2, mean, rstd, gamma, scale, hpre, w2t, w1t))
    a.da2, a.dh, a.dx, a.dgamma, a.dbeta, a.ws = (_p(t) for t in (da2, dh, dx, dgamma, dbeta, ws))
    a.M, a.C, a.hidden, a.rows_per_sample = M, Cc, hid, rows_per_sample
    a.x, a.w1, a.b1 = _p(x), _p(w1), _p(b1)
    L.check(_timed("mlp_bwd", L.load().swv2_mlp_bwd, C.byref(a), _stream()), "swv2_mlp_bwd")
    return dx, da2, dh


def proj_ln_fwd(oh, wp, bp, gamma, beta, scale, rowidx, x, Bw, Lp, heads, rows_per_sample, eps=1e-5, out=None):
    Cc, Mw = wp.shape[0], Bw * Lp
    _chk(oh, BF16, "proj_ln oh"); _chk(wp, BF16, "proj_ln wp"); _chk(x, torch.float32, "proj_ln x")
    dev = x.device
    if out is None:
        out = (torch.empty_like(x), torch.empty(Mw, Cc, dtype=BF16, device=dev), torch.empty(Mw, device=dev), torch.empty(Mw, device=dev))
    y, a1, mean, rstd = out
    a = L.ProjLnArgs()
    a.oh, a.wp, a.bp, a.gamma, a.beta, a.scale, a.rowidx, a.x = (_p(t) for t in (oh, wp, bp, gamma, beta, scale, rowidx, x))
    a.a1, a.mean, a.rstd, a.y = (_p(t) for t in (a1, mean, rstd, y))
    a.Bw, a.Lp, a.heads, a.C, a.rows_per_sample, a.eps = Bw, Lp, heads, Cc, rows_per_sample, eps
    L.check(_timed("proj_ln_fwd", L.load().swv2_proj_ln_fwd, C.byref(a), _stream()), "swv2_proj_ln_fwd")
    return y, a1, mean, rstd


def proj_ln_bwd(dy, a1, mean, rstd, gamma, scale, rowidx, wpt, dgamma, dbeta, Bw, Lp, heads, rows_per_sample, out=None, ws=None):
    Cc, Mw = wpt.shape[1], Bw * Lp
    _chk(dy, torch.float32, "proj_ln dy"); _chk(a1, BF16, "proj_ln a1"); _chk(wpt, BF16, "proj_ln wpt")
    dev = dy.device
    if out is None:
        out = (torch.empty(Mw, Cc, dtype=BF16, device=dev), torch.empty(Bw, heads, Lp, wpt.shape[0] // max(heads, 1), dtype=BF16, device=dev))
    if ws is None:
        ws = torch.empty(L.load().swv2_proj_ln_bwd_ws_floats(Mw, Cc), dtype=torch.float32, device=dev)
    da1, doh = out
    a = L.ProjLnBwdArgs()
    a.dy, a.a1, a.mean, a.rstd, a.gamma, a.scale, a.rowidx, a.wpt = (_p(t) for t in (dy, a1, mean, rstd, gamma, scale, rowidx, wpt))
    a.da1, a.doh, a.dgamma, a.dbeta, a.ws = (_p(t) for t in (da1, doh, dgamma, dbeta, ws))
    a.Bw, a.Lp, a.heads, a.C, a.rows_per_sample = Bw, Lp, heads, Cc, rows_per_sample
    L.check(_timed("proj_ln_bwd", L.load().swv2_proj_ln_bwd, C.byref(a), _stream()), "swv2_proj_ln_bwd")
    return da1, doh


def cpb_fwd(w1, b1, w2, b2, keep, bias, wh, ww, heads, hidden, drop_p):
    L.check(L.load().swv2_cpb_fwd(_p(w1), _p(b1), _p(w2), _p(b2), _p(keep), _p(bias), wh, ww, heads, hidden, drop_p, _stream()),
            "swv2_cpb_fwd")


_SCRATCH = {}


def _scratch(nbytes: int, device, tag: str) -> torch.Tensor:
    key = (device.index if device.index is not None else torch.cuda.current_device(), tag, _stream())
    t = _SCRATCH.get(key)
    if t is None or t.numel() < nbytes:
        t = _SCRATCH[key] = torch.empty(max(int(nbytes), 1), dtype=torch.uint8, device=device)
    return t


def cpb_bwd(dbias, w1, b1, w2, keep, dw1, db1, dw2, db2, wh, ww, heads, hidden, drop_p, atomics=False):
    lib = L.load()
    if atomics:
        L.check(lib.swv2_cpb_bwd(_p(dbias), _p(w1), _p(b1), _p(w2), _p(keep), _p(dw1), _p(db1), _p(dw2), _p(db2), wh, ww,
                                 heads, hidden, drop_p, _stream()), "swv2_cpb_bwd")
        return
    nb = lib.swv2_cpb_bwd_ws_bytes(wh, ww, heads, hidden)
    ws = _scratch(nb, dbias.device, "cpb_bwd")
    L.check(lib.swv2_cpb_bwd_ws(_p(dbias), _p(w1), _p(b1), _p(w2), _p(keep), _p(dw1), _p(db1), _p(dw2), _p(db2), wh, ww,
                                heads, hidden, drop_p, _p(ws), nb, _stream()), "swv2_cpb_bwd_ws")


def cpb_multi_supported(heads: int, hidden: int, drop_p: float) -> bool:
    return 0 < heads <= 16 and hidden in (64, 128, 256, 384, 512) and abs(drop_p - 0.125) < 1e-6


def cpb_fwd_multi(ptab, nblk, keep_bits, bias_all, wh, ww, heads, hidden, drop_p):
    _chk(bias_all, torch.float32, "cpb_fwd_multi bias")
    if keep_bits is not None:
        _chk(keep_bits, torch.int32, "cpb_fwd_multi keep_bits")
    L.check(L.load().swv2_cpb_fwd_multi(_p(ptab), nblk, _p(keep_bits), _p(bias_all), wh, ww, heads, hidden, drop_p, _stream()),
            "swv2_cpb_fwd_multi")


def cpb_bwd_multi(dtables, nchunk, ptab, nblk, keep_bits, grads, wh, ww, heads, hidden, drop_p):
    lib = L.load()
    _chk(dtables, torch.float32, "cpb_bwd_multi tables"); _chk(grads, torch.float32, "cpb_bwd_multi grads")
    nb = lib.swv2_cpb_bwd_multi_ws_bytes(nblk, wh, ww, heads, hidden)
    ws = _scratch(nb, grads.device, "cpb_bwd_multi")
    L.check(lib.swv2_cpb_bwd_multi(_p(dtables), nchunk, _p(ptab), nblk, _p(keep_bits), _p(grads), wh, ww, heads, hidden, drop_p,
                                   _p(ws), nb, _stream()), "swv2_cpb_bwd_multi")


def attn_pack_bias_multi(bias_all: torch.Tensor) -> torch.Tensor:
    _chk(bias_all, torch.float32, "attn_pack_bias_multi")
    ntab, heads, Lw = bias_all.shape[0], bias_all.shape[1], bias_all.shape[2]
    nb = L.load().swv2_attn_pack_bias_bytes(heads, Lw)
    out = torch.empty(ntab, nb, dtype=torch.uint8, device=bias_all.device)
    L.check(L.load().swv2_attn_pack_bias_multi(_p(bias_all), ntab, heads, Lw, _p(out), _stream()), "swv2_attn_pack_bias_multi")
    return out


class WindowPlan:

    def __init__(self, B, gh, gw, wh, ww, sh, sw, heads, head_dim, device):
        self.B, self.gh, self.gw, self.wh, self.ww, self.sh, self.sw = B, gh, gw, wh, ww, sh, sw
        self.heads, self.d = heads, head_dim
        self.L = wh * ww
        self.Lp, self.DP = attn_geometry(self.L, head_dim)
        self.nwh, self.nww = gh // wh, gw // ww
        self.nW = self.nwh * self.nww
        self.Bw = B * self.nW
        self.T = gh * gw
        if gh % wh or gw % ww:
            raise L.Swv2Error(f"window {wh}x{ww} does not divide the patch grid {gh}x{gw}")
        self.mask_thr = (wh - sh) * ww if sh > 0 else 0
        wi = torch.arange(self.nwh).view(-1, 1, 1, 1)
        wj = torch.arange(self.nww).view(1, -1, 1, 1)
        r = torch.arange(wh).view(1, 1, -1, 1)
        c = torch.arange(ww).view(1, 1, 1, -1)
        src = (((wi * wh + r + sh) % gh) * gw + (wj * ww + c + sw) % gw).reshape(self.nW, self.L)
        tab = torch.full((B, self.nW, self.Lp), -1, dtype=torch.int64)
        tab[:, :, :self.L] = src.unsqueeze(0) + (torch.arange(B) * self.T).view(B, 1, 1)
        self.rowidx = tab.reshape(-1).to(torch.int32).to(device)
        Cc = heads * head_dim
        j = torch.arange(self.DP)
        hd = torch.arange(heads).view(-1, 1)
        one = torch.where(j.view(1, -1) < head_dim, hd * head_dim + j.view(1, -1), torch.full((1, 1), -1)).reshape(-1)
        self.proj_map = one.to(torch.int32).to(device)
        three = torch.cat([torch.where(one >= 0, one + part * Cc, one) for part in range(3)])
        self.qkv_map = three.to(torch.int32).to(device)


@functools.lru_cache(maxsize=64)
def window_plan(B, gh, gw, wh, ww, sh, sw, heads, head_dim, device_index) -> WindowPlan:
    return WindowPlan(B, gh, gw, wh, ww, sh, sw, heads, head_dim, torch.device("cuda", device_index))
```

Measured before the change: 226.1.

## Write bf16 shadow of x1 in proj_ln fwd and use it for fc1 wgrad

The fused proj+LN forward kernel now also writes a bf16 copy of the residual output x1. The grouped weight-gradient kernels (both the tile and slab variants) read that bf16 copy instead of the fp32 x1 for the fc1 weight gradient, which halves the bytes loaded for that operand in backward. The cost is an extra bf16 activation buffer and an extra store in the forward pass. It also changes precision, since the fc1 gradient now uses bf16-rounded activations.

```diff
diff --git a/include/swv2.h b/include/swv2.h
--- a/include/swv2.h
+++ b/include/swv2.h
@@ -331,6 +331,7 @@
     float* y;
     int Bw, Lp, heads, C, rows_per_sample;
     float eps;
+    void* yb;
 } swv2_proj_ln_args;
 typedef struct {
     const float* dy;
@@ -445,6 +446,7 @@
     int bias_prepacked;
     float* dbias_part;
     size_t dbias_part_bytes;
+    void* x1b;
 } swv2_block_desc;
 
 enum swv2_block_step {
@@ -485,6 +487,7 @@
     size_t need_wgrad_ws_bytes;
     int n_fwd, n_bwd;
     int fwd[SWV2_BLOCK_MAX_STEPS], bwd[SWV2_BLOCK_MAX_STEPS];
+    int x1_shadow;
 } swv2_block_plan_t;
 int swv2_block_plan(const swv2_block_desc* d, swv2_block_plan_t* out);
 int swv2_block_step_id(int step);
diff --git a/swin_v2_weather_amd/_lib.py b/swin_v2_weather_amd/_lib.py
--- a/swin_v2_weather_amd/_lib.py
+++ b/swin_v2_weather_amd/_lib.py
@@ -110,7 +110,7 @@
 
 class ProjLnArgs(C.Structure):
     _fields_ = [(n, C.c_void_p) for n in ("oh", "wp", "bp", "gamma", "beta", "scale", "rowidx", "x", "a1", "mean", "rstd", "y")] + \
-               [(n, C.c_int) for n in ("Bw", "Lp", "heads", "C", "rows_per_sample")] + [("eps", C.c_float)]
+               [(n, C.c_int) for n in ("Bw", "Lp", "heads", "C", "rows_per_sample")] + [("eps", C.c_float), ("yb", C.c_void_p)]
 
 
 class ProjLnBwdArgs(C.Structure):
@@ -161,7 +161,7 @@
                 [("wgrad_splits", C.c_int), ("ev_kernel", C.c_int), ("ev_start", C.c_void_p), ("ev_stop", C.c_void_p),
                  ("fuse_proj_ln", C.c_int), ("fuse_mlp", C.c_int), ("wgrad_ws", C.c_void_p), ("wgrad_ws_bytes", C.c_size_t), ("wgrad_group", C.c_int), ("grad_zero", C.c_void_p),
                  ("grad_zero_bytes", C.c_size_t), ("ln_ws_floats", C.c_size_t),
-                 ("bias_prepacked", C.c_int), ("dbias_part", C.c_void_p), ("dbias_part_bytes", C.c_size_t)])
+                 ("bias_prepacked", C.c_int), ("dbias_part", C.c_void_p), ("dbias_part_bytes", C.c_size_t), ("x1b", C.c_void_p)])
 
 
 LAMB_ADAMW, LAMB_BIAS_CORRECTION, LAMB_GRAD_AVERAGING, LAMB_NVLAMB = 1, 2, 4, 8
@@ -181,7 +181,8 @@
     _fields_ = ([(n, C.c_int) for n in ("mlp_fused", "proj_ln_fused", "ln_deferred", "wgrad_grouped", "wgrad_kernel", "grad_zero_in_kernel",
                                         "attn_fwd_chunks", "attn_bwd_chunks", "dbias_dest")] +
                 [(n, C.c_size_t) for n in ("need_hact_bytes", "need_ln_ws_floats", "need_wgrad_ws_bytes")] +
-                [("n_fwd", C.c_int), ("n_bwd", C.c_int), ("fwd", C.c_int * BLOCK_MAX_STEPS), ("bwd", C.c_int * BLOCK_MAX_STEPS)])
+                [("n_fwd", C.c_int), ("n_bwd", C.c_int), ("fwd", C.c_int * BLOCK_MAX_STEPS), ("bwd", C.c_int * BLOCK_MAX_STEPS),
+                 ("x1_shadow", C.c_int)])
 
     def steps(self, phase):
         lib = load()
diff --git a/swin_v2_weather_amd/csrc/block.hip b/swin_v2_weather_amd/csrc/block.hip
--- a/swin_v2_weather_amd/csrc/block.hip
+++ b/swin_v2_weather_amd/csrc/block.hip
@@ -26,12 +26,12 @@
     a.mask_thr = d->mask_thr; a.max_chunks = max_chunks;
     return a;
 }
-void wgrad_items(const swv2_block_desc* d, bool fused, swv2_wgrad_item it[4]) {
+void wgrad_items(const swv2_block_desc* d, bool fused, bool x1_shadow, swv2_wgrad_item it[4]) {
     const int BT = d->B * d->T, Bw = d->B * d->nwh * d->nww, Mw = Bw * d->Lp, C = d->C, h = d->heads, hid = d->hidden;
     it[0].dy = op(SWV2_OP_BF16, d->da2, BT, C, C);
     it[0].x = fused ? op(SWV2_OP_BF16_GELU, d->hpre, BT, hid, hid) : op(SWV2_OP_BF16, d->hact, BT, hid, hid);
     it[0].dW = d->d_fc2_w; it[0].db = d->d_fc2_b; it[0].ldw = hid;
-    it[1].dy = op(SWV2_OP_BF16, d->dh, BT, hid, hid); it[1].x = op(SWV2_OP_F32, d->x1, BT, C, C);
+    it[1].dy = op(SWV2_OP_BF16, d->dh, BT, hid, hid); it[1].x = x1_shadow ? op(SWV2_OP_BF16, d->x1b, BT, C, C) : op(SWV2_OP_F32, d->x1, BT, C, C);
     it[1].dW = d->d_fc1_w; it[1].db = d->d_fc1_b; it[1].ldw = C;
     it[2].dy = op(SWV2_OP_BF16, d->da1, Mw, C, C); it[2].x = op_heads(d->oh, Bw, h, 1, d->Lp, d->DP);
     it[2].dW = d->d_proj_w; it[2].db = d->d_proj_b; it[2].kmap = d->proj_map; it[2].ldw = C;
@@ -75,6 +75,7 @@
     p->mlp_fused = d->fuse_mlp && swv2_mlp_supported(C, hid);
     p->proj_ln_fused = d->fuse_proj_ln && swv2_proj_ln_supported(C, h, d->DP);
     p->need_hact_bytes = p->mlp_fused ? 0 : (size_t)BT * hid * 2;
+    p->x1_shadow = d->x1b != nullptr && p->mlp_fused && p->proj_ln_fused;
     p->ln_deferred = p->mlp_fused && p->proj_ln_fused && d->ln_ws_floats >= ln_pair;
     p->wgrad_grouped = d->wgrad_group && p->mlp_fused && d->wgrad_ws && ws_bytes >= swv2_block_wgrad_ws_bytes(C, hid, h * d->DP, 0);
     p->wgrad_kernel = -1;
@@ -128,7 +129,7 @@
     TRY(plan_block(d, p));
     if (p->wgrad_grouped) {
         swv2_wgrad_item it[4] = {};
-        wgrad_items(d, true, it);
+        wgrad_items(d, true, p->x1_shadow, it);
         p->wgrad_kernel = swv2_block_wgrad_kernel(it, 0, d->wgrad_ws_bytes);
     }
     return SWV2_OK;
@@ -163,7 +164,7 @@
         swv2_proj_ln_args m = {};
         m.oh = d->oh; m.wp = d->w_proj; m.bp = d->proj_b; m.gamma = d->n1_w; m.beta = d->n1_b; m.scale = d->dp1; m.rowidx = d->rowidx;
         m.x = d->x; m.a1 = d->a1; m.mean = d->mean1; m.rstd = d->rstd1; m.y = d->x1; m.Bw = Bw; m.Lp = d->Lp; m.heads = h; m.C = C;
-        m.rows_per_sample = d->T; m.eps = 1e-5f;
+        m.rows_per_sample = d->T; m.eps = 1e-5f; m.yb = p.x1_shadow ? d->x1b : nullptr;
         LAUNCH(SWV2_STEP_PROJ_LN_FWD, swv2_proj_ln_fwd(&m, st));
     } break;
     case SWV2_STEP_PROJ: {
@@ -213,7 +214,7 @@
     const int BT = d->B * d->T, Bw = d->B * d->nwh * d->nww, Mw = Bw * d->Lp, C = d->C, h = d->heads, hid = d->hidden;
     const int sp = d->wgrad_splits > 0 ? d->wgrad_splits : 64;
     swv2_wgrad_item it[4] = {};
-    wgrad_items(d, p.mlp_fused, it);
+    wgrad_items(d, p.mlp_fused, p.x1_shadow, it);
     float* const ln1_ws = p.ln_deferred ? d->ln_ws + swv2_mlp_bwd_ws_floats(BT, C) : d->ln_ws;
     int n_ln1 = 0, n_ln2 = 0;
     for (int i = 0; i < p.n_bwd; ++i) switch (const int s = p.bwd[i]; s) {
diff --git a/swin_v2_weather_amd/csrc/gemm_tn.hip b/swin_v2_weather_amd/csrc/gemm_tn.hip
--- a/swin_v2_weather_amd/csrc/gemm_tn.hip
+++ b/swin_v2_weather_amd/csrc/gemm_tn.hip
@@ -224,6 +224,7 @@
     TnOut o[4];
     int first[5];
     int slices;
+    int x1_bf16;
 };
 __global__ __launch_bounds__(NTHREADS, 2) void gemm_tn_group_kernel(TnGroup a) {
     __shared__ __attribute__((aligned(16))) uint16_t smem[TN_SMEM];
@@ -232,7 +233,13 @@
     const int lin = blockIdx.x, x8 = lin & 7, rest = lin >> 3, tt = a.first[4];
     const int t = rest % tt, slice = (rest / tt) * 8 + x8;
     if (t < a.first[1]) tn_tile<A_BF16, A_BF16_GELU>(a.y0, a.x0, a.o[0], t, slice, a.slices, smem, dbs, gtab);
-    else if (t < a.first[2]) tn_tile<A_BF16, A_F32>(a.y1, a.x1, a.o[1], t - a.first[1], slice, a.slices, smem, dbs, gtab);
+    else if (t < a.first[2]) {
+        if (a.x1_bf16) {
+            ALoad<A_BF16> xb;
+            xb.d = a.x1.d;
+            tn_tile<A_BF16, A_BF16>(a.y1, xb, a.o[1], t - a.first[1], slice, a.slices, smem, dbs, gtab);
+        } else tn_tile<A_BF16, A_F32>(a.y1, a.x1, a.o[1], t - a.first[1], slice, a.slices, smem, dbs, gtab);
+    }
     else if (a.x2.d.p2 >= TM) {
         if (t < a.first[3]) tn_tile<A_BF16, A_HEADS, false, true>(a.y2, a.x2, a.o[2], t - a.first[2], slice, a.slices, smem, dbs, gtab);
         else tn_tile<A_HEADS, A_F32, true, true>(a.y3, a.x3, a.o[3], t - a.first[3], slice, a.slices, smem, dbs, gtab);
@@ -543,6 +550,7 @@
     g.y2 = make_loader<A_BF16>(&it[2].dy); g.x2 = make_loader<A_HEADS>(&it[2].x);
     g.y3 = make_loader<A_HEADS>(&it[3].dy); g.x3 = make_loader<A_F32>(&it[3].x);
     g.slices = r.slices = S;
+    g.x1_bf16 = it[1].x.kind == SWV2_OP_BF16;
     hipLaunchKernelGGL(gemm_tn_group_kernel, dim3(tt * S), dim3(NTHREADS), 0, st, g);
     hipLaunchKernelGGL(tn_reduce_kernel, dim3(BN * BN / 64, tt), dim3(256), 0, st, r);
     SWV2_CHECK_LAUNCH("swv2_block_wgrad");
@@ -564,7 +572,7 @@
         if (rc) return rc;
         rc = check_operand(&it[i].x, "swv2_block_wgrad(x)");
         if (rc) return rc;
-        SWV2_CHECK_ARG(it[i].dy.kind == want[i][0] && it[i].x.kind == want[i][1],
+        SWV2_CHECK_ARG(it[i].dy.kind == want[i][0] && (it[i].x.kind == want[i][1] || (i == 1 && it[i].x.kind == SWV2_OP_BF16)),
                        "swv2_block_wgrad: item %d must be (dY kind %d, X kind %d)", i, want[i][0], want[i][1]);
         SWV2_CHECK_ARG(it[i].dW && it[i].ldw > 0 && it[i].dy.rows == it[i].x.rows, "swv2_block_wgrad: item %d: null dW or row mismatch", i);
         SWV2_CHECK_ARG(!it[i].dy.rowidx && (i == 3 ? it[i].x.rowidx != nullptr : it[i].x.rowidx == nullptr),
diff --git a/swin_v2_weather_amd/csrc/gemm_tn_slab.hip b/swin_v2_weather_amd/csrc/gemm_tn_slab.hip
--- a/swin_v2_weather_amd/csrc/gemm_tn_slab.hip
+++ b/swin_v2_weather_amd/csrc/gemm_tn_slab.hip
@@ -43,6 +43,7 @@
     const void* ptr;
     const int32_t* rowidx;
     int ld;
+    int bf16;
     int heads, parts, Lp, DP;
     uint32_t mgLp, mgDP, mgH;
 };
@@ -384,7 +385,10 @@
     __shared__ __attribute__((aligned(1024))) unsigned char smem[SL_SMEM];
     const int b = blockIdx.x;
     if (b < a.p[1].first) slab_job<F_ROW, F_ROWG, 128, 512, 1, 8, 32, 3>(a.p[0], b - a.p[0].first, smem, a.stamps);
-    else if (b < a.p[2].first) slab_job<F_ROW, F_F32, 512, 128, 8, 1, 32, 3>(a.p[1], b - a.p[1].first, smem, a.stamps);
+    else if (b < a.p[2].first) {
+        if (a.p[1].x.bf16) slab_job<F_ROW, F_ROW, 512, 128, 8, 1, 32, 3>(a.p[1], b - a.p[1].first, smem, a.stamps);
+        else slab_job<F_ROW, F_F32, 512, 128, 8, 1, 32, 3>(a.p[1], b - a.p[1].first, smem, a.stamps);
+    }
     else if (b < a.p[3].first) slab_job<F_ROW, F_HEAD, 128, 128, 2, 4, 64, 4>(a.p[2], b - a.p[2].first, smem, a.stamps);
     else slab_job<F_HEAD, F_F32G, 384, 128, 8, 1, 32, 3>(a.p[3], b - a.p[3].first, smem, a.stamps);
 }
@@ -392,7 +396,10 @@
     __shared__ __attribute__((aligned(1024))) unsigned char smem[SL_SMEM];
     const int b = blockIdx.x;
     if (b < a.p[1].first) slab_job<F_ROW, F_ROWG, 192, 384, 1, 8, 32, 3>(a.p[0], b - a.p[0].first, smem, a.stamps);
-    else if (b < a.p[2].first) slab_job<F_ROW, F_F32, 384, 192, 8, 1, 32, 3>(a.p[1], b - a.p[1].first, smem, a.stamps);
+    else if (b < a.p[2].first) {
+        if (a.p[1].x.bf16) slab_job<F_ROW, F_ROW, 384, 192, 8, 1, 32, 3>(a.p[1], b - a.p[1].first, smem, a.stamps);
+        else slab_job<F_ROW, F_F32, 384, 192, 8, 1, 32, 3>(a.p[1], b - a.p[1].first, smem, a.stamps);
+    }
     else if (b < a.p[3].first) slab_job<F_ROW, F_HEAD, 192, 256, 2, 4, 32, 4>(a.p[2], b - a.p[2].first, smem, a.stamps);
     else slab_job<F_HEAD, F_F32G, 384, 192, 8, 1, 32, 3, true>(a.p[3], b - a.p[3].first, smem, a.stamps);
 }
@@ -583,7 +590,7 @@
 
 SlOp sl_op(const swv2_operand& o) {
     SlOp s = {};
-    s.ptr = o.ptr; s.rowidx = o.rowidx; s.ld = (int)o.ld;
+    s.ptr = o.ptr; s.rowidx = o.rowidx; s.ld = (int)o.ld; s.bf16 = o.kind == SWV2_OP_BF16;
     if (o.kind == SWV2_OP_HEADS) {
         s.heads = o.p[0]; s.parts = (int)o.ld; s.Lp = o.p[2]; s.DP = o.p[3];
         s.mgLp = fdiv_magic(s.Lp); s.mgDP = fdiv_magic(s.DP); s.mgH = fdiv_magic(s.heads);
diff --git a/swin_v2_weather_amd/csrc/proj_ln.hip b/swin_v2_weather_amd/csrc/proj_ln.hip
--- a/swin_v2_weather_amd/csrc/proj_ln.hip
+++ b/swin_v2_weather_amd/csrc/proj_ln.hip
@@ -30,6 +30,7 @@
     const uint16_t* oh; const uint16_t* wp; const float* bp; const float* gamma; const float* beta; const float* scale;
     const int32_t* rowidx; const float* x; uint16_t* a1; float* mean; float* rstd; float* y;
     int Mw, Lp, h, rows_per_sample; float eps;
+    uint16_t* yb;
 };
 
 template <int C, int MT, int HS = 16, int NW = 4>
@@ -153,7 +154,10 @@
 #pragma unroll
                         for (int e = 0; e < 4; ++e) o[e] += sc * ((v[4 * hlf + e] - mu_r) * rs_r * gm[e] + bt[e]);
                         *(f32x4*)(a.y + off + 4 * hlf) = o;
+#pragma unroll
+                        for (int e = 0; e < 4; ++e) v[4 * hlf + e] = o[e];
                     }
+                    if (a.yb) *(uint4*)(a.yb + off) = pack8(v);
                 }
             }
         }
@@ -328,7 +332,7 @@
     }
     const int Mw = a->Bw * a->Lp;
     ProjLnFwd k = {(const uint16_t*)a->oh, (const uint16_t*)a->wp, a->bp, a->gamma, a->beta, a->scale, a->rowidx, a->x,
-                   (uint16_t*)a->a1, a->mean, a->rstd, a->y, Mw, a->Lp, a->heads, a->rows_per_sample, a->eps};
+                   (uint16_t*)a->a1, a->mean, a->rstd, a->y, Mw, a->Lp, a->heads, a->rows_per_sample, a->eps, (uint16_t*)a->yb};
     hipStream_t st = (hipStream_t)stream;
     const bool mt2 = Mw >= 128 * 256;
 #define PL_CASE(CC)                                                                                                  \
diff --git a/swin_v2_weather_amd/networks/swinv2_global.py b/swin_v2_weather_amd/networks/swinv2_global.py
--- a/swin_v2_weather_amd/networks/swinv2_global.py
+++ b/swin_v2_weather_amd/networks/swinv2_global.py
@@ -109,7 +109,7 @@
 
 class _BlockRunner:
 
-    ACTS = ("qkvh", "rnorm", "oh", "lse", "a1", "mean1", "rstd1", "x1", "hpre", "hact", "a2", "mean2", "rstd2", "bias_pack")
+    ACTS = ("qkvh", "rnorm", "oh", "lse", "a1", "mean1", "rstd1", "x1", "hpre", "hact", "a2", "mean2", "rstd2", "bias_pack", "x1b")
     SCRATCH = ("da2", "dh", "da1", "doh", "dqkvh", "dx1", "ln_ws", "wgrad_ws")
 
     def __init__(self, blk, plan, Cc, hid, device):
@@ -124,18 +124,20 @@
         d.wgrad_group = int(os.environ.get("SWV2_WGRAD_GROUP", "1"))
         d.fuse_mlp = int(os.environ.get("SWV2_FUSE_MLP", "1"))
         d.fuse_proj_ln = int(os.environ.get("SWV2_FUSE_PROJ_LN", "1"))
-        d.wgrad_ws = d.grad_zero = 1
+        d.wgrad_ws = d.grad_zero = d.x1b = 1
         d.ln_ws_floats = d.wgrad_ws_bytes = 1 << 62
         full = L.block_plan(d)
         d.ln_ws_floats, d.wgrad_ws_bytes = full.need_ln_ws_floats, full.need_wgrad_ws_bytes
         self.launch_plan = lp = L.block_plan(d)
-        if any(getattr(lp, n) != getattr(full, n) for n in ("mlp_fused", "proj_ln_fused", "ln_deferred", "wgrad_grouped", "wgrad_kernel")):
+        if any(getattr(lp, n) != getattr(full, n) for n in ("mlp_fused", "proj_ln_fused", "ln_deferred", "wgrad_grouped", "wgrad_kernel",
+                                                            "x1_shadow")):
             raise L.Swv2Error("swv2_block_plan: the reported workspace needs do not cover the full plan")
-        d.wgrad_ws = d.grad_zero = None
+        d.wgrad_ws = d.grad_zero = d.x1b = None
         self.desc = d
         act_sizes = [Bw * h * 3 * Lp * DP * 2, Bw * h * 2 * Lp * 4, Bw * h * Lp * DP * 2, Bw * h * Lp * 4, Mw * Cc * 2, Mw * 4,
                      Mw * 4, BT * Cc * 4, BT * hid * 2, lp.need_hact_bytes, BT * Cc * 2, BT * 4, BT * 4,
-                     L.load().swv2_attn_pack_bias_bytes(h, Lw)]
+                     L.load().swv2_attn_pack_bias_bytes(h, Lw),
+                     BT * Cc * 2 if lp.x1_shadow else 0]
         self.act_off, self.act_bytes = _carve(act_sizes)
         scr_sizes = [BT * Cc * 2, BT * hid * 2, Mw * Cc * 2, Bw * h * Lp * DP * 2, Bw * h * 3 * Lp * DP * 2, BT * Cc * 4,
                      d.ln_ws_floats * 4, d.wgrad_ws_bytes]
@@ -178,6 +180,8 @@
         base, d = acts.data_ptr(), self.desc
         for name, off in zip(self.ACTS, self.act_off):
             setattr(d, name, base + off)
+        if not self.launch_plan.x1_shadow:
+            d.x1b = None
 
 
 class _BlockFn(torch.autograd.Function):
diff --git a/swin_v2_weather_amd/ops.py b/swin_v2_weather_amd/ops.py
--- a/swin_v2_weather_amd/ops.py
+++ b/swin_v2_weather_amd/ops.py
@@ -744,7 +744,7 @@
     return dx, da2, dh
 
 
-def proj_ln_fwd(oh, wp, bp, gamma, beta, scale, rowidx, x, Bw, Lp, heads, rows_per_sample, eps=1e-5, out=None):
+def proj_ln_fwd(oh, wp, bp, gamma, beta, scale, rowidx, x, Bw, Lp, heads, rows_per_sample, eps=1e-5, out=None, yb=None):
     Cc, Mw = wp.shape[0], Bw * Lp
     _chk(oh, BF16, "proj_ln oh"); _chk(wp, BF16, "proj_ln wp"); _chk(x, torch.float32, "proj_ln x")
     dev = x.device
@@ -755,6 +755,9 @@
     a.oh, a.wp, a.bp, a.gamma, a.beta, a.scale, a.rowidx, a.x = (_p(t) for t in (oh, wp, bp, gamma, beta, scale, rowidx, x))
     a.a1, a.mean, a.rstd, a.y = (_p(t) for t in (a1, mean, rstd, y))
     a.Bw, a.Lp, a.heads, a.C, a.rows_per_sample, a.eps = Bw, Lp, heads, Cc, rows_per_sample, eps
+    if yb is not None:
+        _chk(yb, BF16, "proj_ln yb")
+        a.yb = _p(yb)
     L.check(_timed("proj_ln_fwd", L.load().swv2_proj_ln_fwd, C.byref(a), _stream()), "swv2_proj_ln_fwd")
     return y, a1, mean, rstd
 
```

Result: no change. 226.2 (median of 2 runs) (+0.0%).
